# dongyangli-del/EEG_Image_decode

Measured on AMD Instinct MI355X. Metric: EEG-CLIP contrastive train samples/sec (global batch), higher is better.
Workload: dtype f32; 1 GPU; configs[1]: full ATM-S EEG encoder (63ch x 250t -> 1024-d) contrastive train step vs frozen 1024-d CLIP embeddings, 256 samples/GPU; global_batch=256, per_gpu_batch=256, parallelism=dp1, n_classes_for_accuracy=1654, optimizer=AdamW lr 3e-4 (fused)

## Files before the change

eeg_image_decode_amd/_abi.py:

```python
import ctypes as C

BIG = 1 << 62


class Dim(C.Structure):
    _fields_ = [("div", C.c_longlong), ("so", C.c_longlong), ("si", C.c_longlong)]


def dim(si, div=BIG, so=0):
    return Dim(int(div), int(so), int(si))


class GemmDesc(C.Structure):
    _fields_ = [
        ("M", C.c_int), ("N", C.c_int), ("K", C.c_int),
        ("A", C.c_void_p), ("Am", Dim), ("Ak", Dim),
        ("B", C.c_void_p), ("Bk", Dim), ("Bn", Dim),
        ("C", C.c_void_p), ("Cm", Dim), ("Cn", Dim),
        ("Cpre", C.c_void_p),
        ("bias_n", C.c_void_p), ("bias_m", C.c_void_p),
        ("R", C.c_void_p), ("Rm", Dim), ("Rn", Dim),
        ("alpha", C.c_float), ("accumulate", C.c_int), ("act", C.c_int),
        ("drop_p", C.c_float), ("seed", C.c_ulonglong), ("drop_site", C.c_uint),
        ("split_k", C.c_int),
        ("rowsum_a", C.c_void_p),
        ("precision", C.c_int),
        ("workspace", C.c_void_p), ("workspace_bytes", C.c_longlong),
    ]


class SplitItem(C.Structure):
    _fields_ = [("src", C.c_void_p), ("hi", C.c_void_p), ("lo", C.c_void_p), ("rows", C.c_int), ("cols", C.c_int), ("ld_src", C.c_longlong),
                ("ld_out", C.c_longlong), ("transpose", C.c_int), ("copy", C.c_void_p), ("ld_copy", C.c_longlong)]


class InfonceProblem(C.Structure):
    _fields_ = [("q_hi", C.c_void_p), ("q_lo", C.c_void_p), ("k_hi", C.c_void_p), ("k_lo", C.c_void_p), ("col0", C.c_int), ("weight", C.c_float),
                ("part", C.c_void_p), ("diag", C.c_void_p), ("lse", C.c_void_p), ("lse_k", C.c_void_p), ("G", C.c_void_p), ("ldg", C.c_longlong),
                ("part_k", C.c_void_p), ("diag_k", C.c_void_p), ("G_hi", C.c_void_p), ("G_lo", C.c_void_p)]


class TokenBlockDesc(C.Structure):
    _fields_ = ([("B", C.c_int), ("x", C.c_void_p), ("packed", C.c_void_p), ("bv", C.c_void_p), ("pe", C.c_void_p), ("tokens", C.c_void_p), ("ids", C.c_void_p)]
                + [(k, C.c_void_p) for k in ("bqkv", "bo", "ln1_g", "ln1_b", "b1", "b2", "ln2_g", "ln2_b", "ln3_g", "ln3_b")]
                + [(k, C.c_void_p) for k in ("h", "qkv", "r1", "mu1", "rs1", "f1", "r2", "n2", "mu2", "rs2", "n3", "mu3", "rs3")]
                + [(k, C.c_void_p) for k in ("xp", "hp", "ctxp", "n1p", "g1p")]
                + [("drop_p", C.c_float), ("eps", C.c_float), ("scale", C.c_float), ("seed", C.c_ulonglong)]
                + [(k, C.c_uint) for k in ("site_embed", "site_attn", "site_attn_out", "site_ffn_act", "site_ffn_out")]
                + [("packed_embed", C.c_void_p), ("embed_subject", C.c_void_p), ("bv_stride", C.c_longlong)]
                + [("cs_w25", C.c_void_p), ("cs_bias", C.c_void_p), ("cs_rows", C.c_void_p), ("cs_H", C.c_int)])


class TokenBlockBwdDesc(C.Structure):
    _fields_ = ([("B", C.c_int), ("packed", C.c_void_p)]
                + [(k, C.c_void_p) for k in ("dn3", "n2", "r2", "r1", "f1", "mu1", "rs1", "mu2", "rs2", "mu3", "rs3", "ln1_g", "ln2_g", "ln2_b", "ln3_g")]
                + [(k, C.c_void_p) for k in ("dr1", "dctx", "partials", "df2p", "dg1p", "da1p", "dr1p", "dqkvp")]
                + [(k, C.c_void_p) for k in ("dln3_g", "dln3_b", "dln2_g", "dln2_b", "dln1_g", "dln1_b")]
                + [("drop_p", C.c_float), ("seed", C.c_ulonglong)]
                + [(k, C.c_uint) for k in ("site_embed", "site_attn_out", "site_ffn_act", "site_ffn_out")])


class GemmPlanesDesc(C.Structure):
    _fields_ = [("a_hi", C.c_void_p), ("a_lo", C.c_void_p), ("b_hi", C.c_void_p), ("b_lo", C.c_void_p), ("lda", C.c_longlong), ("ldb", C.c_longlong),
                ("M", C.c_int), ("N", C.c_int), ("K", C.c_int), ("C", C.c_void_p), ("ldc", C.c_longlong), ("Cpre", C.c_void_p), ("ldcpre", C.c_longlong),
                ("bias", C.c_void_p), ("R", C.c_void_p), ("ldr", C.c_longlong), ("p_hi", C.c_void_p), ("p_lo", C.c_void_p), ("ldp", C.c_longlong),
                ("act", C.c_int), ("accumulate", C.c_int), ("planes_of", C.c_int)]


class HeadGemmDesc(C.Structure):
    _fields_ = [("a_hi", C.c_void_p), ("a_lo", C.c_void_p), ("b_hi", C.c_void_p), ("b_lo", C.c_void_p), ("lda", C.c_longlong), ("ldb", C.c_longlong),
                ("M", C.c_int), ("N", C.c_int), ("K", C.c_int), ("slices", C.c_int), ("slab_stride", C.c_longlong), ("bias", C.c_void_p),
                ("Cpre", C.c_void_p), ("ldcpre", C.c_longlong), ("act", C.c_int), ("aux", C.c_void_p), ("ldaux", C.c_longlong), ("R", C.c_void_p),
                ("ldr", C.c_longlong), ("C", C.c_void_p), ("ldc", C.c_longlong), ("p_hi", C.c_void_p), ("p_lo", C.c_void_p), ("ldp", C.c_longlong),
                ("b_kmajor", C.c_int)]


class Conv16Desc(C.Structure):
    _fields_ = [("in_", C.c_void_p), ("W", C.c_void_p), ("out", C.c_void_p), ("bias", C.c_void_p), ("residual", C.c_void_p),
                ("N", C.c_int), ("Hi", C.c_int), ("Wi", C.c_int), ("Cin", C.c_int), ("in_pad", C.c_int),
                ("Ho", C.c_int), ("Wo", C.c_int), ("Cout", C.c_int), ("out_pad", C.c_int),
                ("KS", C.c_int), ("stride", C.c_int), ("pad_top", C.c_int), ("pad_left", C.c_int), ("upsample", C.c_int), ("dtype", C.c_int),
                ("chan_bias", C.c_void_p)]


class WgradTokProblem(C.Structure):
    _fields_ = [("a", C.c_void_p), ("b", C.c_void_p), ("a_group_stride", C.c_longlong), ("m_groups", C.c_int), ("heads_m", C.c_int), ("heads_n", C.c_int),
                ("M", C.c_int), ("N", C.c_int), ("out", C.c_void_p), ("ldo", C.c_longlong), ("bias_out", C.c_void_p), ("bias_mfma", C.c_int),
                ("sample0", C.c_int), ("samples", C.c_int), ("sample_index", C.c_void_p)]


class CstackFwdDesc(C.Structure):
    _fields_ = [("B", C.c_int), ("H", C.c_int), ("x", C.c_void_p), ("xs_b", C.c_longlong), ("xs_h", C.c_longlong), ("w25", C.c_void_p), ("bias1", C.c_void_p),
                ("stat1", C.c_void_p), ("nstat1", C.c_int), ("count1", C.c_double), ("eps", C.c_float), ("momentum", C.c_float),
                ("gamma1", C.c_void_p), ("beta1", C.c_void_p), ("mean1", C.c_void_p), ("rstd1", C.c_void_p), ("run_mean1", C.c_void_p),
                ("run_var1", C.c_void_p), ("nbt1", C.c_void_p), ("packed", C.c_void_p), ("bias2", C.c_void_p), ("y2", C.c_void_p), ("stat2", C.c_void_p)]


class CstackBwdDesc(C.Structure):
    _fields_ = [("B", C.c_int), ("H", C.c_int), ("x", C.c_void_p), ("xs_b", C.c_longlong), ("xs_h", C.c_longlong), ("w25", C.c_void_p), ("bias1", C.c_void_p),
                ("mean1", C.c_void_p), ("rstd1", C.c_void_p), ("gamma1", C.c_void_p), ("beta1", C.c_void_p), ("packed_t", C.c_void_p), ("dy2", C.c_void_p),
                ("rows_out", C.c_void_p), ("stat", C.c_void_p), ("nstat", C.c_int), ("count", C.c_double), ("stat_local", C.c_void_p),
                ("nstat_local", C.c_int), ("dgamma", C.c_void_p), ("dbeta", C.c_void_p), ("dx", C.c_void_p), ("dw_partials", C.c_void_p), ("dw25", C.c_void_p)]


class WgradPlanesProblem(C.Structure):
    _fields_ = [("a_hi", C.c_void_p), ("a_lo", C.c_void_p), ("lda", C.c_longlong), ("b_hi", C.c_void_p), ("b_lo", C.c_void_p), ("ldb", C.c_longlong),
                ("rows", C.c_int), ("M", C.c_int), ("N", C.c_int), ("out", C.c_void_p), ("ldo", C.c_longlong), ("bias_out", C.c_void_p), ("slices", C.c_int)]


PLAN_MAX_ARGS = 28
PLAN_MEMSET, PLAN_JOIN, PLAN_SIDE, PLAN_SKIP, PLAN_SIDE2 = -2, -3, 1, 2, 4


class PlanArg(C.Union):
    _fields_ = [("p", C.c_void_p), ("i", C.c_longlong), ("u", C.c_ulonglong), ("d", C.c_double), ("f", C.c_float), ("i32", C.c_int), ("u32", C.c_uint)]


class PlanOp(C.Structure):
    _fields_ = [("fn", C.c_int), ("flags", C.c_int), ("a", PlanArg * PLAN_MAX_ARGS)]


ACT_NONE, ACT_GELU, ACT_SILU, ACT_GELU_GRAD = 0, 1, 2, 3
PREC_F32, PREC_BF16X3 = 0, 1
ABI_VERSION = 14
DT_BF16, DT_F16 = 0, 1
_P, _I, _F, _L, _U64, _U, _D = C.c_void_p, C.c_int, C.c_float, C.c_longlong, C.c_ulonglong, C.c_uint, C.c_double

PROTOTYPES = {
    "eegclip_abi_version": [],
    "eegclip_gemm_f32": [C.POINTER(GemmDesc), _P],
    "eegclip_gemm_workspace_bytes": [C.POINTER(GemmDesc)],
    "eegclip_split_rows": [C.POINTER(SplitItem), _I, _P],
    "eegclip_gemm_f32_grouped": [_P, _I, _P],
    "eegclip_layernorm_fwd": [_P, _P, _P, _P, _P, _P, _I, _I, _F, _P],
    "eegclip_residual_layernorm_fwd": [_P, _P, _P, _F, _U64, _U, _P, _P, _P, _P, _P, _P, _P, _P, _P, _P, _I, _I, _F, _P],
    "eegclip_residual_layernorm_fwd_planes": [_P, _P, _P, _F, _U64, _U, _P, _P, _P, _P, _P, _P, _P, _P, _P, _P, _I, _I, _F, _P, _P, _P],
    "eegclip_layernorm_bwd": [_P, _P, _P, _P, _P, _P, _P, _P, _I, _I, _I, _P, _F, _U64, _U, _P],
    "eegclip_layernorm_bwd_full_workspace_floats": [_I, _I],
    "eegclip_layernorm_bwd_full": [_P, _P, _P, _P, _P, _P, _P, _P, _I, _I, _I, _P, _F, _U64, _U, _P, _P],
    "eegclip_layernorm_bwd_params_workspace_floats": [_I, _I],
    "eegclip_layernorm_bwd_params": [_P, _P, _P, _P, _P, _P, _I, _I, _P, _P],
    "eegclip_layernorm_silu_fwd": [_P, _P, _P, _P, _P, _P, _P, _I, _I, _F, _F, _U64, _U, _P],
    "eegclip_silu_bwd": [_P, _P, _P, _L, _I, _F, _U64, _U, _P],
    "eegclip_timestep_embedding": [_P, _I, _I, _P, _P],
    "eegclip_ddpm_add_noise": [_P, _P, _P, _P, _P, _P, _I, _I, _P],
    "eegclip_ddpm_step": [_P, _P, _P, _F, _F, _F, _F, _F, _F, _P, _P, _P, _L, _P],
    "eegclip_prior_stage_infer": [_P, _P, _P, _P, _P, _P, _P, _I, _P, _I, _I, _F, _P],
    "eegclip_mse_loss_grad": [_P, _P, _L, _P, _P, _P],
    "eegclip_mse_loss_grad_scaled": [_P, _P, _L, _F, _P, _P, _P],
    "eegclip_bn_stats": [_P, _I, _I, _I, _P, _P],
    "eegclip_bn_finalize": [_P, _D, _F, _F, _I, _P, _P, _P, _P, _I, _P, _P],
    "eegclip_bn_finalize_rows": [_P, _I, _D, _F, _F, _I, _P, _P, _P, _P, _P, _P, _P],
    "eegclip_bn_elu_fwd": [_P, _P, _P, _P, _P, _P, _I, _I, _I, _F, _U64, _U, _P],
    "eegclip_bn_elu_bwd": [_P, _P, _P, _P, _P, _P, _P, _P, _P, _P, _I, _I, _I, _F, _U64, _U, _P],
    "eegclip_bn_elu_bwd_stats": [_P, _P, _P, _P, _P, _P, _P, _I, _I, _I, _F, _U64, _U, _P],
    "eegclip_bn_elu_bwd_apply": [_P, _P, _P, _P, _P, _P, _P, _P, _D, _P, _P, _P, _I, _I, _I, _F, _U64, _U, _P],
    "eegclip_embed_finish": [_P, _P, _P, _I, _I, _I, _F, _U64, _U, _P],
    "eegclip_embed_finish_bwd": [_P, _P, _P, _I, _I, _I, _F, _U64, _U, _P],
    "eegclip_dropout_scale": [_P, _L, _F, _U64, _U, _P],
    "eegclip_gelu_bwd": [_P, _P, _P, _L, _I, _F, _U64, _U, _P],
    "eegclip_bias_act": [_P, _P, _P, _P, _P, _I, _I, _I, _F, _U64, _U, _P],
    "eegclip_axpby": [_P, _P, _L, _F, _F, _P],
    "eegclip_reduce_mid": [_P, _I, _I, _I, _P, _P],
    "eegclip_colsum_blocks": [_P, _I, _I, _I, _I, _L, _P, _P],
    "eegclip_sumsq": [_P, _L, _P, _P],
    "eegclip_stage_eeg": [_P, _P, _L, _I, _I, _I, _P, _I, _I, _P],
    "eegclip_gather_rows": [_P, _L, _P, _L, _P, _I, _I, _I, _P],
    "eegclip_adamw_step": [_P, _P, _P, _P, _L, _F, _F, _F, _F, _F, _L, _F, _P, _P],
    "eegclip_adamw_step_zero_grad": [_P, _P, _P, _P, _L, _F, _F, _F, _F, _F, _L, _F, _P, _P],
    "eegclip_clip_scale": [_P, _F, _P, _P],
    "eegclip_attention_fwd": [_P, _P, _I, _I, _I, _I, _I, _F, _F, _U64, _U, _P],
    "eegclip_attention_bwd": [_P, _P, _P, _I, _I, _I, _I, _I, _F, _F, _U64, _U, _P],
    "eegclip_attention_bwd_x3": [_P, _P, _P, _I, _I, _I, _I, _I, _I, _F, _F, _U64, _U, _P],
    "eegclip_proj1x1_fwd": [_P, _P, _P, _P, _P, _P, _P, _P, _P, _I, _F, _U64, _U, _P],
    "eegclip_proj1x1_fwd_rows": [_P, _P, _I, _D, _F, _F, _P, _P, _P, _P, _P, _P, _P, _P, _P, _P, _P, _I, _F, _U64, _U, _P],
    "eegclip_proj1x1_bwd_workspace_floats": [_I],
    "eegclip_proj1x1_bwd": [_P, _P, _P, _P, _P, _P, _P, _P, _P, _P, _P, _P, _P, _I, _F, _U64, _U, _P],
    "eegclip_cast_bf16": [_P, _P, _L, _P],
    "eegclip_logits_bf16": [_P, _P, _P, _I, _I, _I, _L, _P, _P],
    "eegclip_tsconv_fwd_workspace_floats": [_I, _I],
    "eegclip_tsconv_fwd": [_P, _L, _L, _P, _P, _P, _I, _I, _I, _I, _P, _P, _P],
    "eegclip_tsconv_bwd_w": [_P, _L, _L, _P, _P, _P, _I, _I, _I, _I, _P],
    "eegclip_tsconv_bwd_w_workspace_floats": [_I, _I],
    "eegclip_tsconv_bwd_x": [_P, _P, _P, _L, _L, _I, _I, _I, _I, _P],
    "eegclip_cross_attn_fwd": [_P, _P, _P, _P, _P, _P, _I, _I, _I, _I, _I, _I, _F, _I, _P],
    "eegclip_self_attn_supported": [_I, _L, _L, _L, _L],
    "eegclip_self_attn_fwd": [_P, _L, _P, _L, _P, _L, _P, _L, _I, _I, _I, _I, _I, _F, _I, _P],
    "eegclip_self_attn_causal_fwd": [_P, _L, _P, _L, _P, _L, _P, _L, _I, _I, _I, _I, _I, _F, _I, _P],
    "eegclip_sconv_fwd": [_P, _P, _P, _P, _P, _P, _P, _P, _P, _I, _I, _I, _P, _P],
    "eegclip_sconv_fwd_workspace_floats": [_I],
    "eegclip_sconv_bwd_w_workspace_floats": [_I, _I],
    "eegclip_sconv_bwd_w": [_P, _P, _P, _P, _P, _P, _P, _P, _I, _I, _I, _P],
    "eegclip_sconv_bwd_x_stats_workspace_floats": [_I],
    "eegclip_sconv_bwd_x_stats": [_P, _P, _P, _P, _P, _P, _P, _P, _P, _P, _P, _I, _I, _P],
    "eegclip_sconv_bwd_x_apply": [_P, _P, _P, _P, _P, _P, _P, _P, _P, _P, _P, _D, _P, _P, _P, _I, _I, _P],
    "eegclip_lse_rows": [_P, _I, _I, _L, _P, _P, _P],
    "eegclip_lse_cols": [_P, _I, _I, _L, _P, _P, _P],
    "eegclip_infonce_grad": [_P, _I, _I, _L, _I, _I, _P, _P, _P, _F, _P, _P, _P],
    "eegclip_infonce_loss": [_P, _I, _L, _P, _P, _P, _F, _P, _P],
    "eegclip_gemm16": [_P, _L, _P, _L, _P, _L, _P, _P, _L, _I, _I, _I, _I, _I, _P],
    "eegclip_sampler_step": [_P, _P, _P, _P, _P, _P, _F, _F, _F, _F, _F, _L, _I, _P],
    "eegclip_split_bf16": [_P, _P, _P, _L, _P],
    "eegclip_infonce_fused_supported": [_I, _I, _I],
    "eegclip_infonce_fused_workspace_floats": [_I, _I],
    "eegclip_infonce_fused_fwd": [C.POINTER(InfonceProblem), _I, _I, _I, _I, _I, _I, _P, _P, _P],
    "eegclip_infonce_fused_grad": [C.POINTER(InfonceProblem), _I, _I, _I, _I, _I, _I, _P, _P, _P],
    "eegclip_infonce_fused_grad_finalize": [C.POINTER(InfonceProblem), _I, _I, _I, _I, _I, _I, _P, _P, _P, _P],
    "eegclip_token_block_packed_bytes": [],
    "eegclip_token_block_pack": [_P, _P, _P, _P, _P, _P, _P],
    "eegclip_weight_prep": [_P, _P, _P, _P, _P, _P, _P, _P, _P, _I, _P],
    "eegclip_token_block_packed_embed_bytes": [_I],
    "eegclip_token_block_pack_embed": [_P, _L, _I, _P, _P],
    "eegclip_token_block_fwd": [C.POINTER(TokenBlockDesc), _P],
    "eegclip_token_block_bwd_workspace_floats": [_I],
    "eegclip_token_block_bwd": [C.POINTER(TokenBlockBwdDesc), _I, _P],
    "eegclip_gemm_planes": [C.POINTER(GemmPlanesDesc), _P],
    "eegclip_split_transpose": [C.POINTER(SplitItem), _I, _P],
    "eegclip_infonce_small_supported": [_I, _I],
    "eegclip_infonce_small_workspace_floats": [_I, _I],
    "eegclip_infonce_small_fwd": [_P, _I, _L, _I, _I, _P, _P, _P],
    "eegclip_infonce_small_grad": [_I, _I, _P, _P, _F, _F, _F, _F, _P, _P, _L, _P, _P, _P],
    "eegclip_conv16": [C.POINTER(Conv16Desc), _P],
    "eegclip_groupnorm16": [_P, _I, _I, _I, _I, _I, _I, _P, _P, _F, _I, _P, _I, _P, _I, _P],
    "eegclip_softmax_rows16": [_P, _I, _I, _L, _F, _I, _P],
    "eegclip_vae_sample16": [_P, _P, _P, _L, _I, _I, _P],
    "eegclip_layernorm16": [_P, _L, _P, _P, _P, _L, _I, _I, _F, _I, _P],
    "eegclip_geglu16": [_P, _P, _I, _I, _I, _P],
    "eegclip_concat16": [_P, _P, _P, _I, _I, _I, _I, _I, _I, _I, _I, _P],
    "eegclip_gather_rows16": [_P, _L, _P, _I, _P, _I, _P, _I, _I, _I, _P],
    "eegclip_act16": [_P, _L, _P, _L, _I, _I, _I, _I, _P],
    "eegclip_head_gemm_slices": [_I, _I, _I],
    "eegclip_head_gemm": [C.POINTER(HeadGemmDesc), _P],
    "eegclip_head_act": [_P, _I, _L, _P, _P, _P, _P, _P, _I, _I, _P],
    "eegclip_head_act_bwd": [_P, _I, _L, _P, _P, _P, _P, _P, _L, _P],
    "eegclip_residual_layernorm_fwd_slabs": [_P, _P, _P, _F, _U64, _U, _P, _P, _P, _P, _P, _P, _P, _P, _P, _P, _I, _I, _F, _P, _P, _I, _L, _P, _P],
    "eegclip_layernorm_bwd_slabs": [_P, _I, _L, _P, _P, _P, _P, _P, _I, _I, _P, _P, _P, _P, _F, _U64, _U, _P],
    "eegclip_proj1x1_bwd_slabs": [_P, _I, _L, _P, _P, _P, _P, _P, _P, _P, _P, _P, _P, _P, _P, _I, _F, _U64, _U, _P],
    "eegclip_proj1x1_fwd_rows_planes": [_P, _P, _I, _D, _F, _F, _P, _P, _P, _P, _P, _P, _P, _P, _P, _P, _P, _I, _F, _U64, _U, _P, _P, C.POINTER(SplitItem), _I, _P],
    "eegclip_proj1x1_bwd_rows": [_P, _I, _L, _P, _P, _P, _P, _P, _P, _P, _P, _P, _P, _I, _F, _U64, _U, _P],
    "eegclip_proj1x1_bwd_reduce": [_P, _I, _P, _P, _P, _P],
    "eegclip_bn_elu_bwd_apply_rows": [_P, _P, _P, _P, _P, _P, _P, _I, _L, _I, _D, _P, _P, _P, _I, _I, _I, _F, _U64, _U, _P],
    "eegclip_prior_stage_fwd": [_P, _P, _P, _P, _P, _P, _P, _P, _P, _P, _I, _I, _F, _F, _U64, _U, _P],
    "eegclip_prior_stage_bwd": [_P, _P, _P, _P, _P, _P, _P, _P, _P, _P, _P, _I, _I, _F, _U64, _U, _P, _P],
    "eegclip_prior_stage_bwd_workspace_floats": [_I, _I],
    "eegclip_prior_stage_bwd_params": [_P, _I, _I, _P, _P, _P],
    "eegclip_silu_bwd_planes": [_P, _P, _P, _P, _L, _P],
    "eegclip_wgrad_tok_slices": [_I, _I],
    "eegclip_wgrad_tok_workspace_floats": [C.POINTER(WgradTokProblem), _I, _I, _I],
    "eegclip_wgrad_tok": [C.POINTER(WgradTokProblem), _I, _I, _I, _P, _I, _P],
    "eegclip_wgrad_tok_reduce": [C.POINTER(WgradTokProblem), _I, _I, _I, _P, _P],
    "eegclip_wgrad_tok_reduce_adamw": [C.POINTER(WgradTokProblem), _I, _I, _I, _P, _P, _P, _P, _P, _L, _F, _F, _F, _F, _F, _L, _P],
    "eegclip_wgrad_planes": [C.POINTER(WgradPlanesProblem), _I, _P],
    "eegclip_tok_planes_from_f32": [_P, _L, _I, _I, _I, _I, _P, _P],
    "eegclip_cstack_packed_bytes": [_I],
    "eegclip_cstack_pack": [_P, _P, _I, _P],
    "eegclip_cstack_stats1": [_P, _L, _L, _P, _P, _P, _I, _I, _P],
    "eegclip_cstack_fwd": [C.POINTER(CstackFwdDesc), _P],
    "eegclip_cstack_packed_t_bytes": [_I],
    "eegclip_cstack_pack_t": [_P, _P, _I, _P],
    "eegclip_cstack_pack_all": [_P, _P, _P, _I, _P],
    "eegclip_cstack_bwd_stats": [C.POINTER(CstackBwdDesc), _P],
    "eegclip_cstack_bwd_workspace_floats": [_I],
    "eegclip_cstack_bwd_apply": [C.POINTER(CstackBwdDesc), _P],
    "eegclip_cstack_bwd_taps_reduce": [_P, _I, _P, _P],
    "eegclip_cstack_bwd_w2_workspace_floats": [_I, _I],
    "eegclip_cstack_bwd_w2": [_P, _L, _L, _P, _P, _P, _P, _P, _P, _P, _P, _P, _I, _I, _P],
    "eegclip_plan_fn_id": [C.c_char_p],
    "eegclip_plan_events": [_I, C.POINTER(C.c_void_p)],
    "eegclip_plan_events_destroy": [_I, C.POINTER(C.c_void_p)],
    "eegclip_plan_run": [C.POINTER(PlanOp), _I, _I, _I, _P, _P, _P, C.POINTER(C.c_void_p), _P, _P, C.POINTER(C.c_int), C.POINTER(C.c_int)],
    "eegclip_topk_rows": [_P, _I, _I, _L, _I, _P, _P, _P],
    "eegclip_count_equal": [_P, _I, _P, _I, _P, _P],
    "eegclip_top1_count": [_P, _I, _I, _L, _P, _P, _P, _P],
    "eegclip_timing_event_create": [],
    "eegclip_timing_event_destroy": [_P],
    "eegclip_time_next_launch": [_P, _P],
    "eegclip_timing_elapsed_ms": [_P, _P],
# ... 20 lines not shown
```

eeg_image_decode_amd/atms.py:

```python
import os
import weakref
import ctypes
import math

import numpy as np
import torch
import torch.nn as nn

from . import _abi
from ._lib import EegclipError, current_stream, lib, raw_stream, require_cuda
from .loss import ClipLoss
from .plan import Plan

D = _abi.dim
ACT_GELU = _abi.ACT_GELU
ACT_GELU_GRAD = _abi.ACT_GELU_GRAD

N_CH, T_LEN, D_MODEL, N_HEADS, D_HEAD, D_FF = 63, 250, 250, 4, 62, 256
L_TOK = N_CH + 1
HE = N_HEADS * D_HEAD
C_TS, W_TS, F_TS, P_DIM = 40, 36, 1440, 1024
EPS = 1e-5
SITE_EMBED, SITE_ATTN, SITE_ATTN_OUT, SITE_FFN_ACT, SITE_FFN_OUT, SITE_CONV, SITE_PROJ = range(7)

# ... 677 lines not shown
                _p(self.buffers[_TS + "2.running_mean"]), _p(self.buffers[_TS + "2.running_var"]), int(train),
                _p(self.buffers[_TS + "2.num_batches_tracked"]))
        if "scf_ws" not in b:
            b["scf_ws"] = torch.empty(int(lib().eegclip_sconv_fwd_workspace_floats(B)), dtype=torch.float32, device=self.device)
        pl.call("eegclip_sconv_fwd", _p(b["y1"]), _p(bn[0]), _p(bn[1]), _p(P[_TS + "2.weight"]), _p(P[_TS + "2.bias"]), _p(P[_TS + "4.weight"]),
                _p(P[_TS + "4.bias"]), _p(b["y2"]), _p(sums[1]) if train else None, B, N_CH, 1, _p(b["scf_ws"]))
        if W > 1:
            pl.callback(lambda: self._allreduce(sums[1]), "allreduce_bn2")
        pl.call("eegclip_bn_finalize", _p(sums[1]), float(W * B * W_TS), EPS, 0.1, C_TS, _p(bn[2]), _p(bn[3]),
                _p(self.buffers[_TS + "5.running_mean"]), _p(self.buffers[_TS + "5.running_var"]), int(train),
                _p(self.buffers[_TS + "5.num_batches_tracked"]))

    def _build_bwd(self, B, shared, probs, want_dx, early_reduce=False, train=True):
        P, G, b = self.P, self.G, self.bufs[B]
        pe_, pc_, pp_ = probs
        pl = Plan(f"atms_bwd[B={B}]")
        R = B * L_TOK
        sums, bn = b["sums"], b["bn"]
        defer_small = os.environ.get("EEGCLIP_DEFER_SMALL", "1") != "0"
        pl.deferred = []
        wsk = int(os.environ.get("EEGCLIP_WGRAD_SK", "0"))
        attn_bwd = "eegclip_attention_bwd_x3" if pl.precision == _abi.PREC_BF16X3 else "eegclip_attention_bwd"
        sk = lambda k: (wsk if (wsk > 0 and k >= 4096) else max(1, min(64, k // 512)))

        head_side = os.environ.get("EEGCLIP_HEAD_WGRAD_SIDE", "1") != "0"

        def wgrad(name, dY, ldy, X, ldx, Nout, Nin, K, bias=None, side=head_side):
            return pl.gemm(Nout, Nin, K, dY, D(1), D(ldy), X, D(ldx), D(1), _p(G[name]), D(Nin), D(1), accumulate=1, split_k=sk(K),
                           rowsum_a=_p(G[bias]) if bias else None, side=side)

        ln_side = os.environ.get("EEGCLIP_LN_SIDE", "1") != "0"
        if "lnp_ws" not in b:
            b["lnp_ws"] = torch.empty(int(lib().eegclip_layernorm_bwd_params_workspace_floats(R, D_MODEL)), dtype=torch.float32, device=self.device)
        lnp_ws = _p(b["lnp_ws"])
        if "lnf_ws" not in b:
            b["lnf_ws"] = torch.empty(int(lib().eegclip_layernorm_bwd_full_workspace_floats(R, D_MODEL)), dtype=torch.float32, device=self.device)
        lnf_ws = _p(b["lnf_ws"])
        pl.dout_op = len(pl.ops)
        head_planes = self._head_planes_enabled(pl) and hasattr(self, "hw")
        pl.head_planes = head_planes
        dfeat_slabs = None
        if head_planes:
            if "dvp" not in b:
                b["dvp"] = torch.empty(2, B, P_DIM, dtype=torch.bfloat16, device=self.device)
                b["dup"] = torch.empty(2, B, P_DIM, dtype=torch.bfloat16, device=self.device)
                b["dout_sum"] = torch.empty(B, P_DIM, dtype=torch.float32, device=self.device)
            vp, up = (_p(b["dvp"][0]), _p(b["dvp"][1])), (_p(b["dup"][0]), _p(b["dup"][1]))
            pl.call("eegclip_layernorm_bwd_slabs", 0, 1, 0, _p(b["s"]), _p(P["proj_eeg.2.weight"]), _p(b["mu4"]), _p(b["rs4"]), _p(b["ds"]), B, P_DIM,
                    _p(b["dv"]), *vp, None, pp_, 0, SITE_PROJ, seed_at=15)
            one_fork = os.environ.get("EEGCLIP_HEAD_FORKS", "1") == "1"
            head_side_ops = []

            def later(fn):
                if one_fork:
                    head_side_ops.append(fn)
                else:
                    fn()

            def ln_params():
                pl.dout_par_op = len(pl.ops)
                pl.call("eegclip_layernorm_bwd", 0, _p(b["s"]), None, _p(b["mu4"]), _p(b["rs4"]), None,
                        _p(G["proj_eeg.2.weight"]), _p(G["proj_eeg.2.bias"]), B, P_DIM, 0, None, 0.0, 0, 0, side=ln_side)
            later(ln_params)
            wplanes = B % 32 == 0 and os.environ.get("EEGCLIP_HEAD_WGRAD_PLANES", "1") != "0"
            if not wplanes:
                later(lambda: wgrad("proj_eeg.1.fn.1.weight", _p(b["dv"]), P_DIM, _p(b["gu"]), P_DIM, P_DIM, P_DIM, B, bias="proj_eeg.1.fn.1.bias"))
            if os.environ.get("EEGCLIP_HEAD_FUSED_EPI", "0") == "1":
                pl.call_desc("eegclip_head_gemm", _abi.HeadGemmDesc(a_hi=vp[0], a_lo=vp[1], b_hi=self.hw["w2"][0], b_lo=self.hw["w2"][1], lda=P_DIM, ldb=P_DIM, M=B,
                                                                   N=P_DIM, K=P_DIM, slices=1, slab_stride=0, act=ACT_GELU_GRAD, aux=_p(b["u"]), ldaux=P_DIM,
                                                                   R=_p(b["ds"]), ldr=P_DIM, C=_p(b["ds"]), ldc=P_DIM, p_hi=up[0], p_lo=up[1], ldp=P_DIM, b_kmajor=1))
            else:
                sl = self._head_gemm(pl, b, "dgu_slabs", vp, P_DIM, self.hw["w2"], P_DIM, B, kmajor=True)
                pl.call("eegclip_head_act_bwd", *sl, _p(b["u"]), _p(b["ds"]), _p(b["ds"]), *up, B * P_DIM)
            if wplanes:
                gp_, fp_ = (_p(b["gup"][0]), _p(b["gup"][1])), (_p(b["featp"][0]), _p(b["featp"][1]))
                probs = (_abi.WgradPlanesProblem * 2)(
                    _abi.WgradPlanesProblem(a_hi=vp[0], a_lo=vp[1], lda=P_DIM, b_hi=gp_[0], b_lo=gp_[1], ldb=P_DIM, rows=B, M=P_DIM, N=P_DIM,
                                            out=_p(G["proj_eeg.1.fn.1.weight"]), ldo=P_DIM, bias_out=_p(G["proj_eeg.1.fn.1.bias"]), slices=1),
                    _abi.WgradPlanesProblem(a_hi=up[0], a_lo=up[1], lda=P_DIM, b_hi=fp_[0], b_lo=fp_[1], ldb=F_TS, rows=B, M=P_DIM, N=F_TS,
                                            out=_p(G["proj_eeg.0.weight"]), ldo=F_TS, bias_out=_p(G["proj_eeg.0.bias"]), slices=1))
                pl._keep.append(probs)
                later(lambda: pl.call("eegclip_wgrad_planes", probs, 2, side=head_side))
            else:
                later(lambda: wgrad("proj_eeg.0.weight", _p(b["ds"]), P_DIM, _p(b["feat"]), F_TS, P_DIM, F_TS, B, bias="proj_eeg.0.bias"))
            dfeat_slabs = self._head_gemm(pl, b, "dfeat_slabs", up, P_DIM, self.hw["w1"], F_TS, B, kmajor=True)
        else:
            head_side_ops = []
            self._build_bwd_head_f32(pl, b, B, pp_, ln_side, wgrad)
        W = self._world() if train else 1
        zsum = None
        if not train:
            zsum = torch.zeros(2 * C_TS, dtype=torch.float64, device=self.device)
            pl._keep.append(zsum)

            def conv_bias_grad(bias_key, gamma_key, rstd, s):
                return lambda: G[bias_key].add_((P[gamma_key] * rstd * s[:C_TS].to(torch.float32)))
        if "pj_ws" not in b:
            b["pj_ws"] = torch.empty(int(lib().eegclip_proj1x1_bwd_workspace_floats(B)) // 2, dtype=torch.float64, device=self.device)
        lean = dfeat_slabs is not None and self._lean(pl, train, W)
        pl.lean = lean
        if lean:
            if "pj_bn_rows" not in b:
                b["pj_bn_rows"] = torch.empty(B, 2 * C_TS, dtype=torch.float64, device=self.device)
            pl.call("eegclip_proj1x1_bwd_rows", *dfeat_slabs, _p(b["z2"]), _p(P["enc_eeg.0.projection.0.weight"]), _p(b["y2"]), _p(bn[2]), _p(bn[3]),
                    _p(P[_TS + "5.weight"]), _p(P[_TS + "5.bias"]), _p(b["dz2"]), _p(b["pj_ws"]), _p(b["pj_bn_rows"]), B, pc_, 0, SITE_CONV, seed_at=15)
            pl.call("eegclip_bn_elu_bwd_apply_rows", _p(b["dz2"]), _p(b["y2"]), _p(bn[2]), _p(bn[3]), _p(P[_TS + "5.weight"]), _p(P[_TS + "5.bias"]),
                    _p(b["pj_bn_rows"]), B, 2 * C_TS, 0, float(B * W_TS),
                    _p(b["dy2"]), _p(G[_TS + "5.weight"]), _p(G[_TS + "5.bias"]), B, C_TS, W_TS, pc_, 0, SITE_CONV, seed_at=18)
            for f in head_side_ops:
                f()
            pl.call("eegclip_proj1x1_bwd_reduce", _p(b["pj_ws"]), B, _p(G["enc_eeg.0.projection.0.weight"]), _p(G["enc_eeg.0.projection.0.bias"]), None, side=True)
        else:
            if dfeat_slabs is not None:
                pl.call("eegclip_proj1x1_bwd_slabs", *dfeat_slabs, _p(b["z2"]), _p(P["enc_eeg.0.projection.0.weight"]), _p(b["y2"]), _p(bn[2]), _p(bn[3]),
                        _p(P[_TS + "5.weight"]), _p(P[_TS + "5.bias"]), _p(b["dz2"]), _p(G["enc_eeg.0.projection.0.weight"]),
                        _p(G["enc_eeg.0.projection.0.bias"]), _p(sums[2]), _p(b["pj_ws"]), B, pc_, 0, SITE_CONV, seed_at=17)
            else:
                pl.call("eegclip_proj1x1_bwd", _p(b["dfeat"]), _p(b["z2"]), _p(P["enc_eeg.0.projection.0.weight"]), _p(b["y2"]), _p(bn[2]), _p(bn[3]),
                        _p(P[_TS + "5.weight"]), _p(P[_TS + "5.bias"]), _p(b["dz2"]), _p(G["enc_eeg.0.projection.0.weight"]),
                        _p(G["enc_eeg.0.projection.0.bias"]), _p(sums[2]), _p(b["pj_ws"]), B, pc_, 0, SITE_CONV, seed_at=15)
            local2 = None
            if W > 1:
                local2 = torch.zeros_like(sums[2])
                pl._keep.append(local2)

                def exchange2():
                    local2.copy_(sums[2])
                    self._allreduce(sums[2])
                pl.callback(exchange2, "allreduce_bn2_bwd")
            if not train:
                pl.callback(conv_bias_grad(_TS + "4.bias", _TS + "5.weight", bn[3], sums[2]), "conv2_bias_grad_eval")
            pl.call("eegclip_bn_elu_bwd_apply", _p(b["dz2"]), _p(b["y2"]), _p(bn[2]), _p(bn[3]), _p(P[_TS + "5.weight"]), _p(P[_TS + "5.bias"]),
                    _p(sums[2]) if train else _p(zsum), (_p(local2) if local2 is not None else None) if train else _p(sums[2]), float(W * B * W_TS), _p(b["dy2"]), _p(G[_TS + "5.weight"]), _p(G[_TS + "5.bias"]), B, C_TS,
                    W_TS, pc_, 0, SITE_CONV, seed_at=16)
            for f in head_side_ops:
                f()
        if self._cstack_bwd_enabled(pl):
            self._build_bwd_cstack(pl, b, B, train, W, zsum, conv_bias_grad if not train else None, early_reduce, defer_small)
        else:
            self._build_bwd_conv_y1(pl, b, B, train, W, zsum, conv_bias_grad if not train else None, early_reduce)
        fused = self._token_block_enabled(pl) and hasattr(self, "tb_packed")
        if fused:
            if "tb_part" not in b:
                b["tb_part"] = torch.empty(int(lib().eegclip_token_block_bwd_workspace_floats(B)), dtype=torch.float32, device=self.device)
            df2p, dg1p, da1p, dr1p, dqkvp = self._token_planes(b, B, "df2p", "dg1p", "da1p", "dr1p", "dqkvp")
            xp, hp, ctxp, n1p, g1p = self._token_planes(b, B, "xp", "hp", "ctxp", "n1p", "g1p")
            bd = _abi.TokenBlockBwdDesc(
                B=B, packed=_p(self.tb_packed), dn3=_p(b["dn3"]), n2=None, r2=_p(b["r2"]), r1=_p(b["r1"]), f1=_p(b["f1"]), mu1=_p(b["mu1"]),
                rs1=_p(b["rs1"]), mu2=_p(b["mu2"]), rs2=_p(b["rs2"]), mu3=_p(b["mu3"]), rs3=_p(b["rs3"]), ln1_g=_p(P[_LY + "norm1.weight"]),
                ln2_g=_p(P[_LY + "norm2.weight"]), ln2_b=_p(P[_LY + "norm2.bias"]), ln3_g=_p(P["encoder.encoder.norm.weight"]),
                dr1=_p(b["dr1"]), dctx=_p(b["dctx"]), partials=_p(b["tb_part"]), df2p=df2p, dg1p=dg1p, da1p=da1p, dr1p=dr1p, dqkvp=dqkvp,
                dln3_g=_p(G["encoder.encoder.norm.weight"]), dln3_b=_p(G["encoder.encoder.norm.bias"]), dln2_g=_p(G[_LY + "norm2.weight"]),
                dln2_b=_p(G[_LY + "norm2.bias"]), dln1_g=_p(G[_LY + "norm1.weight"]), dln1_b=_p(G[_LY + "norm1.bias"]),
                drop_p=pe_, seed=0, site_embed=SITE_EMBED, site_attn_out=SITE_ATTN_OUT, site_ffn_act=SITE_FFN_ACT, site_ffn_out=SITE_FFN_OUT)
            pl._keep.append(bd)
            if pe_ > 0.0:
                pl._seed_descs.append(bd)
            variant = 0

            def wgrad_tok(tag, problems, side=True, slices=None, index=None):
                arr = (_abi.WgradTokProblem * len(problems))()
                for i, (name, a, mg, x, M, N, hm, hn, bias, bm) in enumerate(problems):
                    arr[i] = _abi.WgradTokProblem(a=a, b=x, a_group_stride=B * 65536 if mg > 1 else 0, m_groups=mg, heads_m=hm, heads_n=hn, M=M, N=N,
                                                  out=_p(G[name]), ldo=N, bias_out=_p(G[bias]) if bias else None, bias_mfma=bm, sample_index=index)
                groups = sum(q[2] for q in problems)
                slices = slices or (wsk if wsk > 0 else int(lib().eegclip_wgrad_tok_slices(groups, B)))
                key = "wk:" + tag
                if key not in b:
                    b[key] = torch.empty(int(lib().eegclip_wgrad_tok_workspace_floats(arr, len(problems), B, slices)), dtype=torch.float32, device=self.device)
                pl._keep.append(arr)
                ops = (len(pl.ops), len(pl.ops) + 1)
                pl.call("eegclip_wgrad_tok", arr, len(problems), B, slices, _p(b[key]), variant, side=side)
                pl.call("eegclip_wgrad_tok_reduce", arr, len(problems), B, slices, _p(b[key]), side=side)
                return arr, ops

            merge = int(os.environ.get("EEGCLIP_WGRAD_MERGE", "2"))
            late = []
            ffn_out = [
                (_LY + "conv2.weight", df2p, 1, g1p, D_MODEL, D_FF, 0, 0, _LY + "conv2.bias", 1),
                (_LY + "conv1.weight", dg1p, 1, n1p, D_FF, D_MODEL, 0, 0, _LY + "conv1.bias", 0),
                (_LY + "attention.out_projection.weight", da1p, 1, ctxp, D_MODEL, HE, 0, 1, _LY + "attention.out_projection.bias", 0)]
            qkv_w = [(_LY + "attention.query_projection.weight", dqkvp, 3, hp, 3 * HE, D_MODEL, 1, 0, _LY + "attention.query_projection.bias", 0)]
            pl.call("eegclip_token_block_bwd", ctypes.byref(bd), 0)
            if defer_small:
                pl.deferred.append(lambda: pl.call("eegclip_token_block_bwd", ctypes.byref(bd), 2, side=True))
            else:
                pl.call("eegclip_token_block_bwd", ctypes.byref(bd), 2, side=ln_side)
            if merge >= 2:
                late += ffn_out
            else:
                wgrad_tok("ffn_out", ffn_out)
            pl.call(attn_bwd, _p(b["qkv"]), _p(b["dctx"]), dqkvp, 1, B, L_TOK, N_HEADS, D_HEAD, 3 * HE, 1.0 / math.sqrt(D_HEAD),
                    pe_, 0, SITE_ATTN, seed_at=11)
            if merge >= 1:
                late += qkv_w
            else:
                wgrad_tok("qkv", qkv_w)
            pl.call("eegclip_token_block_bwd", ctypes.byref(bd), 1)
        else:
            pl.call("eegclip_layernorm_bwd_full", _p(b["dn3"]), _p(b["n2"]), _p(P["encoder.encoder.norm.weight"]), _p(b["mu3"]), _p(b["rs3"]), _p(b["dn2"]),
                    _p(G["encoder.encoder.norm.weight"]), _p(G["encoder.encoder.norm.bias"]), R, D_MODEL, 0, None, 0.0, 0, 0, lnf_ws)
            pl.call("eegclip_layernorm_bwd_full", _p(b["dn2"]), _p(b["r2"]), _p(P[_LY + "norm2.weight"]), _p(b["mu2"]), _p(b["rs2"]), _p(b["dr2"]),
                    _p(G[_LY + "norm2.weight"]), _p(G[_LY + "norm2.bias"]), R, D_MODEL, 0, _p(b["df2"]), pe_, 0, SITE_FFN_OUT, lnf_ws, seed_at=13)
            wgrad(_LY + "conv2.weight", _p(b["df2"]), D_MODEL, _p(b["g1"]), D_FF, D_MODEL, D_FF, R, bias=_LY + "conv2.bias")
            pl.gemm(R, D_FF, D_MODEL, _p(b["df2"]), D(D_MODEL), D(1), _p(P[_LY + "conv2.weight"]), D(D_FF), D(1), _p(b["dg1"]), D(D_FF), D(1),
                    act=ACT_GELU_GRAD, R=_p(b["f1"]), Rm=D(D_FF), Rn=D(1), drop_p=pe_, drop_site=SITE_FFN_ACT)
            wgrad(_LY + "conv1.weight", _p(b["dg1"]), D_FF, _p(b["n1"]), D_MODEL, D_FF, D_MODEL, R, bias=_LY + "conv1.bias")
            pl.gemm(R, D_MODEL, D_FF, _p(b["dg1"]), D(D_FF), D(1), _p(P[_LY + "conv1.weight"]), D(D_MODEL), D(1), _p(b["dr2"]), D(D_MODEL), D(1),
                    accumulate=1)
            pl.call("eegclip_layernorm_bwd_full", _p(b["dr2"]), _p(b["r1"]), _p(P[_LY + "norm1.weight"]), _p(b["mu1"]), _p(b["rs1"]), _p(b["dr1"]),
                    _p(G[_LY + "norm1.weight"]), _p(G[_LY + "norm1.bias"]), R, D_MODEL, 0, _p(b["da1"]), pe_, 0, SITE_ATTN_OUT, lnf_ws, seed_at=13)
            wgrad(_LY + "attention.out_projection.weight", _p(b["da1"]), D_MODEL, _p(b["ctx"]), HE, D_MODEL, HE, R,
                  bias=_LY + "attention.out_projection.bias")
            pl.gemm(R, HE, D_MODEL, _p(b["da1"]), D(D_MODEL), D(1), _p(P[_LY + "attention.out_projection.weight"]), D(HE), D(1), _p(b["dctx"]), D(HE), D(1))
            if attn_bwd == "eegclip_attention_bwd_x3":
                pl.call(attn_bwd, _p(b["qkv"]), _p(b["dctx"]), _p(b["dqkv"]), 0, B, L_TOK, N_HEADS, D_HEAD, 3 * HE, 1.0 / math.sqrt(D_HEAD),
                        pe_, 0, SITE_ATTN, seed_at=11)
            else:
                pl.call(attn_bwd, _p(b["qkv"]), _p(b["dctx"]), _p(b["dqkv"]), B, L_TOK, N_HEADS, D_HEAD, 3 * HE, 1.0 / math.sqrt(D_HEAD),
                        pe_, 0, SITE_ATTN, seed_at=10)
            wgrad(_LY + "attention.query_projection.weight", _p(b["dqkv"]), 3 * HE, _p(b["h"]), D_MODEL, 3 * HE, D_MODEL, R,
                  bias=_LY + "attention.query_projection.bias")
            pl.gemm(R, D_MODEL, 3 * HE, _p(b["dqkv"]), D(3 * HE), D(1), _p(P[_LY + "attention.query_projection.weight"]), D(D_MODEL), D(1),
                    _p(b["dr1"]), D(D_MODEL), D(1), accumulate=2, drop_p=pe_, drop_site=SITE_EMBED)
        tokg = G[_TOK_SHARED] if shared else G[_TOK_TABLE]
        pl.call("eegclip_embed_finish_bwd", _p(b["dr1"]), _p(tokg), None if shared else _p(b["ids"]), B, L_TOK, D_MODEL, 0.0, 0, SITE_EMBED, side=True)
        for f in pl.deferred:
            f()
        hmap = D(D_MODEL, div=N_CH, so=L_TOK * D_MODEL)
        if want_dx:
            b["dx"] = torch.empty(B, N_CH, T_LEN, dtype=torch.float32, device=self.device)
        pl.x_gemm = None
        if fused:
            if not self.joint:
                wgrad_tok("embed" + ("+%d" % len(late) if late else ""), late + [(_E + "value_embedding.weight", dr1p, 1, xp, D_MODEL, T_LEN, 0, 0, _E + "value_embedding.bias", 0)], side=False)
            else:
                if late:
                    wgrad_tok("block", late, side=False)
                pl.j_wk_template = [(w, dr1p, 1, xp, D_MODEL, T_LEN, 0, 0, bk, 0) for w, bk in self.ve_keys]
                pl.j_wk_slices = [0] + [max(1, min(32, 2 * B // 4, (64 // n) // 8 * 8 if 64 // n >= 8 else 64 // n)) for n in range(1, self.n_subj + 1)]
                pl.j_wk_arr, pl.j_wk_ops = wgrad_tok("embed_joint", pl.j_wk_template, side=False, slices=8, index=_p(b["perm"]))
                need = max(int(lib().eegclip_wgrad_tok_workspace_floats(pl.j_wk_arr, n, B, pl.j_wk_slices[n])) for n in range(1, self.n_subj + 1))
                if b["wk:embed_joint"].numel() < need:
                    b["wk:embed_joint"] = torch.empty(need, dtype=torch.float32, device=self.device)
                    for op in pl.j_wk_ops:
                        pl.set_arg(op, 4, _p(b["wk:embed_joint"]))
                pl.j_wk_all = (_abi.WgradTokProblem * self.n_subj)(*pl.j_wk_arr)
                pl._keep.append(pl.j_wk_all)
        elif not self.joint:
            pl.x_gemm = pl.gemm(D_MODEL, T_LEN, B * N_CH, _p(b["dr1"]) + 4 * D_MODEL, D(1), hmap, 0, D(T_LEN), D(1),
                    _p(G[_E + "value_embedding.weight"]), D(T_LEN), D(1), accumulate=1, split_k=sk(B * N_CH),
                    rowsum_a=_p(G[_E + "value_embedding.bias"]))
        if not self.joint:
            if want_dx:
                pl.gemm(B * N_CH, T_LEN, D_MODEL, _p(b["dr1"]) + 4 * D_MODEL, hmap, D(1),
                        _p(P[_E + "value_embedding.weight"]), D(T_LEN), D(1), _p(b["dx"]), D(T_LEN), D(1))
        elif fused and not want_dx:
            pass
        else:
            XR = N_CH * T_LEN
            pl.j_gather = len(pl.ops)
            pl.call("eegclip_gather_rows", _p(b["hs"]) + 4 * D_MODEL, L_TOK * D_MODEL, _p(b["dr1"]) + 4 * D_MODEL, L_TOK * D_MODEL, _p(b["perm"]), B,
                    N_CH * D_MODEL, 0)
            if not fused:
                pl.j_gemm = [pl.desc(D_MODEL, T_LEN, N_CH, 0, D(1), hmap, 0, D(T_LEN), D(1), _p(G[w]), D(T_LEN), D(1), accumulate=1, split_k=1,
                                     rowsum_a=_p(G[bk])) for w, bk in self.ve_keys]
                pl.j_arr, pl.j_group = pl.gemm_grouped(self.n_subj)
            if want_dx:
                b["dxs"] = torch.empty(B, N_CH, T_LEN, dtype=torch.float32, device=self.device)
                pl.j_dx = [pl.desc(N_CH, T_LEN, D_MODEL, 0, hmap, D(1), _p(P[w]), D(T_LEN), D(1), 0, D(T_LEN), D(1)) for w, _ in self.ve_keys]
                pl.j_dx_arr, pl.j_dx_group = pl.gemm_grouped(self.n_subj)
                pl.j_scatter = len(pl.ops)
                pl.call("eegclip_gather_rows", _p(b["dx"]), XR, _p(b["dxs"]), XR, _p(b["perm"]), B, XR, 1)
        return pl

    def _build_bwd_head_f32(self, pl, b, B, pp_, ln_side, wgrad):
        P, G = self.P, self.G
        pl.call("eegclip_layernorm_bwd", 0, _p(b["s"]), _p(P["proj_eeg.2.weight"]), _p(b["mu4"]), _p(b["rs4"]), _p(b["ds"]),
                None, None, B, P_DIM, 0, _p(b["dv"]), pp_, 0, SITE_PROJ, seed_at=13)
        pl.dout_par_op = len(pl.ops)
        pl.call("eegclip_layernorm_bwd", 0, _p(b["s"]), None, _p(b["mu4"]), _p(b["rs4"]), None,
                _p(G["proj_eeg.2.weight"]), _p(G["proj_eeg.2.bias"]), B, P_DIM, 0, None, 0.0, 0, 0, side=ln_side)
        wgrad("proj_eeg.1.fn.1.weight", _p(b["dv"]), P_DIM, _p(b["gu"]), P_DIM, P_DIM, P_DIM, B, bias="proj_eeg.1.fn.1.bias")
        skh = _head_split(B)
        pl.gemm(B, P_DIM, P_DIM, _p(b["dv"]), D(P_DIM), D(1), _p(P["proj_eeg.1.fn.1.weight"]), D(P_DIM), D(1), _p(b["dgu"]), D(P_DIM), D(1),
                accumulate=int(skh > 1), split_k=skh)
        pl.call("eegclip_gelu_bwd", _p(b["dgu"]), _p(b["u"]), _p(b["ds"]), B * P_DIM, 1, 0.0, 0, 0)
        wgrad("proj_eeg.0.weight", _p(b["ds"]), P_DIM, _p(b["feat"]), F_TS, P_DIM, F_TS, B, bias="proj_eeg.0.bias")
        pl.gemm(B, F_TS, P_DIM, _p(b["ds"]), D(P_DIM), D(1), _p(P["proj_eeg.0.weight"]), D(F_TS), D(1), _p(b["dfeat"]), D(F_TS), D(1),
                accumulate=int(skh > 1), split_k=skh)

    def _build_bwd_cstack(self, pl, b, B, train, W, zsum, conv_bias_grad, early_reduce, defer_small=False):
        P, G, sums, bn = self.P, self.G, b["sums"], b["bn"]
        dev = self.device
        if "csw_ws" not in b:
            b["csw_ws"] = torch.empty(int(lib().eegclip_cstack_bwd_w2_workspace_floats(B, N_CH)), dtype=torch.float32, device=dev)
            b["csb_ws"] = torch.empty(int(lib().eegclip_cstack_bwd_workspace_floats(B)), dtype=torch.float32, device=dev)
            b["cs_rows3"] = torch.empty(B, 2 * C_TS, dtype=torch.float64, device=dev)
        xs = (_p(b["n3"]), L_TOK * D_MODEL, D_MODEL)
        bnp = (_p(bn[0]), _p(bn[1]), _p(P[_TS + "2.weight"]), _p(P[_TS + "2.bias"]))
        pl.call("eegclip_cstack_bwd_w2", *xs, _p(P[_TS + "0.weight"]), _p(P[_TS + "0.bias"]), *bnp, _p(b["dy2"]), _p(G[_TS + "4.weight"]), _p(b["csw_ws"]),
                B, N_CH, side=os.environ.get("EEGCLIP_W2_SIDE", "1") != "0")
        rows3 = b["cs_rows3"]
        count1 = float(W * B * N_CH * W_TS)
        common = dict(B=B, H=N_CH, x=xs[0], xs_b=xs[1], xs_h=xs[2], w25=_p(P[_TS + "0.weight"]), bias1=_p(P[_TS + "0.bias"]), mean1=bnp[0], rstd1=bnp[1],
                      gamma1=bnp[2], beta1=bnp[3], packed_t=_p(self.cs_packed_t), dy2=_p(b["dy2"]), rows_out=_p(rows3), count=count1,
                      dgamma=_p(G[_TS + "2.weight"]), dbeta=_p(G[_TS + "2.bias"]), dx=_p(b["dn3"]), dw_partials=_p(b["csb_ws"]), dw25=_p(G[_TS + "0.weight"]))
        pl.call_desc("eegclip_cstack_bwd_stats", _abi.CstackBwdDesc(stat=None, nstat=0, stat_local=None, nstat_local=0, **common))
        stat, nstat, local, nlocal = _p(rows3), B, None, 0
        if W > 1 or not train:
            pl.call("eegclip_bn_finalize_rows", _p(rows3), B, count1, EPS, 0.1, C_TS, None, None, None, None, None, _p(sums[3]))
            local, nlocal = _p(rows3), B
            if W > 1:
                pl.callback(lambda: self._allreduce(sums[3]), "allreduce_bn1_bwd")
            stat, nstat = (_p(sums[3]), 1) if train else (_p(zsum), 1)
            if not train:
                pl.callback(conv_bias_grad(_TS + "0.bias", _TS + "2.weight", bn[1], sums[3]), "conv1_bias_grad_eval")
        pl.call_desc("eegclip_cstack_bwd_apply", _abi.CstackBwdDesc(stat=stat, nstat=nstat, stat_local=local, nstat_local=nlocal, **dict(common, dw25=None)))
        pl.early_cut = len(pl.ops)

        def taps():
            pl.taps_op = len(pl.ops)
            pl.call("eegclip_cstack_bwd_taps_reduce", _p(b["csb_ws"]), B, _p(G[_TS + "0.weight"]), side=True)
        if early_reduce or not defer_small:
            taps()
        else:
            pl.deferred.append(taps)
        if early_reduce:
            pl.callback(self._start_early_reduce, "allreduce_early_bucket", side=True)

    def _build_bwd_conv_y1(self, pl, b, B, train, W, zsum, conv_bias_grad, early_reduce):
        P, G, sums, bn = self.P, self.G, b["sums"], b["bn"]
        if "scw_ws" not in b:
            b["scw_ws"] = torch.empty(int(lib().eegclip_sconv_bwd_w_workspace_floats(B, N_CH)), dtype=torch.float32, device=self.device)
        bnp = (_p(bn[0]), _p(bn[1]), _p(P[_TS + "2.weight"]), _p(P[_TS + "2.bias"]))
        wt = (None, None)
        if "scx_ws" not in b:
            b["scx_ws"] = torch.empty(int(lib().eegclip_sconv_bwd_x_stats_workspace_floats(B)) // 2, dtype=torch.float64, device=self.device)
        pl.call("eegclip_sconv_bwd_w", _p(b["y1"]), *bnp, _p(b["dy2"]), _p(G[_TS + "4.weight"]), _p(b["scw_ws"]), B, N_CH, pl.precision & 0xff, side=True)
        pl.call("eegclip_sconv_bwd_x_stats", _p(b["dy2"]), _p(P[_TS + "4.weight"]), *wt, _p(b["y1"]), *bnp, _p(sums[3]), _p(b["scx_ws"]), B, N_CH)
        local1 = None
        if W > 1:
            local1 = torch.zeros_like(sums[3])
            pl._keep.append(local1)

            def exchange1():
                local1.copy_(sums[3])
                self._allreduce(sums[3])
            pl.callback(exchange1, "allreduce_bn1_bwd")
        if not train:
            pl.callback(conv_bias_grad(_TS + "0.bias", _TS + "2.weight", bn[1], sums[3]), "conv1_bias_grad_eval")
# ... 216 lines not shown
```

eeg_image_decode_amd/csrc/attention_x3.hip:

```cpp
#include "eeg_common.h"

namespace eeg {

constexpr int AX_L = 64;
constexpr int AX_RS = 144;
constexpr int AX_PLANE = AX_L * AX_RS;
constexpr int AX_TENSOR = 2 * AX_PLANE;

struct ax_args {
    const float* qkv;
    const float* dctx;
    float* dqkv;
    unsigned char* dqkvp;
    int B, H, E, ld;
    float scale, drop_p;
    unsigned long long seed;
    unsigned site;
};

typedef short ax_s4 __attribute__((ext_vector_type(4)));
typedef float ax_f2 __attribute__((ext_vector_type(2)));
typedef float ax_f4u __attribute__((ext_vector_type(4), aligned(4)));

__device__ __forceinline__ ax_s4 ax_tr_read(const unsigned char* p) {
#if defined(EEG_EMU)
    const int lane = hipemu::cur->lane, g = lane >> 4, i = lane & 15;
    ax_s4 r;
    for (int j = 0; j < 4; ++j) {
        const unsigned long long src = hipemu::shfl_idx((unsigned long long)(uintptr_t)p, 16 * g + 4 * j + (i >> 2));
        r[j] = reinterpret_cast<const short*>((uintptr_t)src)[i & 3];
    }
    return r;
#else
    return __builtin_amdgcn_ds_read_tr16_b64_v4i16((__attribute__((address_space(3))) ax_s4*)(p));
#endif
}
__device__ __forceinline__ bf16x8 ax_tr_frag(const unsigned char* plane, int r0, int r1, int c0, int lane) {
    const int l = lane & 15;
    const ax_s4 a = ax_tr_read(plane + (r0 + (l >> 2)) * AX_RS + 2 * (c0 + 4 * (l & 3)));
    const ax_s4 b = ax_tr_read(plane + (r1 + (l >> 2)) * AX_RS + 2 * (c0 + 4 * (l & 3)));
    return bf16x8{a[0], a[1], a[2], a[3], b[0], b[1], b[2], b[3]};
}
__device__ __forceinline__ bf16x8 ax_frag(const unsigned char* plane, int row, int k0) {
    return *reinterpret_cast<const bf16x8*>(plane + row * AX_RS + 2 * k0);
}
__device__ __forceinline__ bf16x8 ax_pack8(u32x2_t a, u32x2_t b) {
    typedef unsigned u4 __attribute__((ext_vector_type(4)));
    const u4 v{a[0], a[1], b[0], b[1]};
    return __builtin_bit_cast(bf16x8, v);
}
__device__ __forceinline__ f32x4 ax_mfma3(bf16x8 ah, bf16x8 al, bf16x8 bh, bf16x8 bl, f32x4 c) {
    c = mfma_bf16_16x16x32(al, bh, c);
    c = mfma_bf16_16x16x32(ah, bl, c);
    return mfma_bf16_16x16x32(ah, bh, c);
}
__device__ __forceinline__ void ax_store4(float* p, int valid, f32x4 v) {
    if (valid >= 4) *reinterpret_cast<ax_f4u*>(p) = ax_f4u{v[0], v[1], v[2], v[3]};
    else if (valid >= 2) {
        *reinterpret_cast<ax_f2*>(p) = ax_f2{v[0], v[1]};
        if (valid == 3) p[2] = v[2];
    } else if (valid == 1) p[0] = v[0];
}

__device__ __forceinline__ void ax_store4_planes(unsigned char* row_base, int e0, f32x4 v) {
    u32x2_t hi, lo;
    x3_split4(v[0], v[1], v[2], v[3], hi, lo);
    *reinterpret_cast<u32x2_t*>(row_base + 2 * e0) = hi;
    *reinterpret_cast<u32x2_t*>(row_base + 32768 + 2 * e0) = lo;
}

template <bool TRAIN>
__global__ __launch_bounds__(256, 2) void attention_bwd_x3_kernel(const ax_args a) {
    EEG_LDS_BASE(float, ldsf);
    unsigned char* lds = reinterpret_cast<unsigned char*>(ldsf);
    unsigned char* Qp = lds;
    unsigned char* Kp = lds + AX_TENSOR;
    unsigned char* Vp = lds + 2 * AX_TENSOR;
    unsigned char* Op = lds + 3 * AX_TENSOR;
    const int t = threadIdx.x, lane = t & 63, w = wave_uniform(t >> 6), fr = lane & 15, g = lane >> 4;
    const int bh = blockIdx.x, b = bh / a.H, h = bh - b * a.H;
    const int E = a.E, HE = a.H * E;
    const float* qrow0 = a.qkv + (long long)b * AX_L * a.ld + h * E;
    const float* orow0 = a.dctx + (long long)b * AX_L * HE + h * E;

    {
        ax_f2 v[4][8];
#pragma unroll
        for (int j = 0; j < 8; ++j) {
            const int idx = t + 256 * j, row = idx >> 5, col = 2 * (idx & 31);
            const bool ok = col < E;
            const float* qr = qrow0 + (long long)row * a.ld + col;
            v[0][j] = ok ? *reinterpret_cast<const ax_f2*>(qr) : ax_f2{0.f, 0.f};
            v[1][j] = ok ? *reinterpret_cast<const ax_f2*>(qr + HE) : ax_f2{0.f, 0.f};
            v[2][j] = ok ? *reinterpret_cast<const ax_f2*>(qr + 2 * HE) : ax_f2{0.f, 0.f};
            v[3][j] = ok ? *reinterpret_cast<const ax_f2*>(orow0 + (long long)row * HE + col) : ax_f2{0.f, 0.f};
        }
#pragma unroll
        for (int x = 0; x < 4; ++x)
#pragma unroll
            for (int j = 0; j < 8; ++j) {
                const int idx = t + 256 * j, row = idx >> 5, col = 2 * (idx & 31);
                const unsigned hi = x3_pack2(v[x][j][0], v[x][j][1]);
                const float r0 = v[x][j][0] - __uint_as_float(hi << 16), r1 = v[x][j][1] - __uint_as_float(hi & 0xffff0000u);
                unsigned char* dst = lds + x * AX_TENSOR + row * AX_RS + 2 * col;
                *reinterpret_cast<unsigned*>(dst) = hi;
                *reinterpret_cast<unsigned*>(dst + AX_PLANE) = x3_pack2(r0, r1);
            }
    }
    __syncthreads();

    f32x4 s[4], dp[4];
#pragma unroll
    for (int kt = 0; kt < 4; ++kt) { s[kt] = f32x4{0.f, 0.f, 0.f, 0.f}; dp[kt] = f32x4{0.f, 0.f, 0.f, 0.f}; }
#pragma unroll
    for (int ks = 0; ks < 2; ++ks) {
        const int k0 = 32 * ks + 8 * g;
        const bf16x8 qh = ax_frag(Qp, 16 * w + fr, k0), ql = ax_frag(Qp + AX_PLANE, 16 * w + fr, k0);
        const bf16x8 oh = ax_frag(Op, 16 * w + fr, k0), ol = ax_frag(Op + AX_PLANE, 16 * w + fr, k0);
#pragma unroll
        for (int kt = 0; kt < 4; ++kt) {
            const bf16x8 kh = ax_frag(Kp, 16 * kt + fr, k0), kl = ax_frag(Kp + AX_PLANE, 16 * kt + fr, k0);
            const bf16x8 vh = ax_frag(Vp, 16 * kt + fr, k0), vl = ax_frag(Vp + AX_PLANE, 16 * kt + fr, k0);
            s[kt] = ax_mfma3(kh, kl, qh, ql, s[kt]);
            dp[kt] = ax_mfma3(vh, vl, oh, ol, dp[kt]);
        }
    }
    float mx = -INFINITY;
#pragma unroll
    for (int kt = 0; kt < 4; ++kt)
#pragma unroll
        for (int r = 0; r < 4; ++r) {
            s[kt][r] *= a.scale;
            mx = fmaxf(mx, s[kt][r]);
        }
    mx = fmaxf(mx, __shfl_xor(mx, 16, 64));
    mx = fmaxf(mx, __shfl_xor(mx, 32, 64));
    float sum = 0.f;
#pragma unroll
    for (int kt = 0; kt < 4; ++kt)
#pragma unroll
        for (int r = 0; r < 4; ++r) {
            s[kt][r] = expf(s[kt][r] - mx);
            sum += s[kt][r];
        }
    sum += __shfl_xor(sum, 16, 64);
    sum += __shfl_xor(sum, 32, 64);
    const float inv = 1.0f / sum;
    const bool drop = TRAIN && a.drop_p > 0.f;
    const float ksc = drop ? 1.f / (1.f - a.drop_p) : 1.f;
    f32x4 pd[4];
    float dq_sum = 0.f;
#pragma unroll
    for (int kt = 0; kt < 4; ++kt) {
        bool keep[4] = {true, true, true, true};
        if (drop) {
            const unsigned long long idx0 = ((unsigned long long)bh * AX_L + 16 * w + fr) * AX_L + 16 * kt + 4 * g;
            dropout_keep4(a.seed, a.site, idx0, a.drop_p, keep);
        }
#pragma unroll
        for (int r = 0; r < 4; ++r) {
            const float p = s[kt][r] * inv;
            const float d = keep[r] ? dp[kt][r] * ksc : 0.f;
            pd[kt][r] = keep[r] ? p * ksc : 0.f;
            s[kt][r] = p;
            dp[kt][r] = d;
            dq_sum += p * d;
        }
    }
    dq_sum += __shfl_xor(dq_sum, 16, 64);
    dq_sum += __shfl_xor(dq_sum, 32, 64);
#pragma unroll
    for (int kt = 0; kt < 4; ++kt)
#pragma unroll
        for (int r = 0; r < 4; ++r) dp[kt][r] = s[kt][r] * (dp[kt][r] - dq_sum);

    {
        f32x4 dq[4];
#pragma unroll
        for (int et = 0; et < 4; ++et) dq[et] = f32x4{0.f, 0.f, 0.f, 0.f};
#pragma unroll
        for (int m = 0; m < 2; ++m) {
            u32x2_t h0, l0, h1, l1;
            x3_split4(dp[2 * m][0], dp[2 * m][1], dp[2 * m][2], dp[2 * m][3], h0, l0);
            x3_split4(dp[2 * m + 1][0], dp[2 * m + 1][1], dp[2 * m + 1][2], dp[2 * m + 1][3], h1, l1);
            const bf16x8 bhf = ax_pack8(h0, h1), blf = ax_pack8(l0, l1);
#pragma unroll
            for (int et = 0; et < 4; ++et) {
                const bf16x8 ah = ax_tr_frag(Kp, 32 * m + 4 * g, 32 * m + 16 + 4 * g, 16 * et, lane);
                const bf16x8 al = ax_tr_frag(Kp + AX_PLANE, 32 * m + 4 * g, 32 * m + 16 + 4 * g, 16 * et, lane);
                dq[et] = ax_mfma3(ah, al, bhf, blf, dq[et]);
            }
        }
        float* out = a.dqkv + ((long long)b * AX_L + 16 * w + fr) * a.ld + h * E;
        unsigned char* outp = a.dqkvp + (long long)b * 65536 + (16 * w + fr) * 512 + 128 * h;
#pragma unroll
        for (int et = 0; et < 4; ++et) {
            const int e0 = 16 * et + 4 * g;
            f32x4 v = dq[et];
#pragma unroll
            for (int r = 0; r < 4; ++r) v[r] *= a.scale;
            if (a.dqkvp) ax_store4_planes(outp, e0, v);
            else if (e0 < E) ax_store4(out + e0, E - e0, v);
        }
    }
    __syncthreads();
#pragma unroll
    for (int kt = 0; kt < 4; ++kt) {
        u32x2_t hi, lo;
        const int off = (16 * w + fr) * AX_RS + 2 * (16 * kt + 4 * g);
        x3_split4(pd[kt][0], pd[kt][1], pd[kt][2], pd[kt][3], hi, lo);
        *reinterpret_cast<u32x2_t*>(Kp + off) = hi;
        *reinterpret_cast<u32x2_t*>(Kp + AX_PLANE + off) = lo;
        x3_split4(dp[kt][0], dp[kt][1], dp[kt][2], dp[kt][3], hi, lo);
        *reinterpret_cast<u32x2_t*>(Vp + off) = hi;
        *reinterpret_cast<u32x2_t*>(Vp + AX_PLANE + off) = lo;
    }
    __syncthreads();

    f32x4 dv[4], dk[4];
#pragma unroll
    for (int et = 0; et < 4; ++et) { dv[et] = f32x4{0.f, 0.f, 0.f, 0.f}; dk[et] = f32x4{0.f, 0.f, 0.f, 0.f}; }
#pragma unroll
    for (int ks = 0; ks < 2; ++ks) {
        const int q0 = 32 * ks + 8 * g;
        const bf16x8 ph = ax_tr_frag(Kp, q0, q0 + 4, 16 * w, lane), pl = ax_tr_frag(Kp + AX_PLANE, q0, q0 + 4, 16 * w, lane);
        const bf16x8 sh = ax_tr_frag(Vp, q0, q0 + 4, 16 * w, lane), sl = ax_tr_frag(Vp + AX_PLANE, q0, q0 + 4, 16 * w, lane);
#pragma unroll
        for (int et = 0; et < 4; ++et) {
            const bf16x8 oh = ax_tr_frag(Op, q0, q0 + 4, 16 * et, lane), ol = ax_tr_frag(Op + AX_PLANE, q0, q0 + 4, 16 * et, lane);
            const bf16x8 qh = ax_tr_frag(Qp, q0, q0 + 4, 16 * et, lane), ql = ax_tr_frag(Qp + AX_PLANE, q0, q0 + 4, 16 * et, lane);
            dv[et] = ax_mfma3(oh, ol, ph, pl, dv[et]);
            dk[et] = ax_mfma3(qh, ql, sh, sl, dk[et]);
        }
    }
    if (a.dqkvp) {
        const long long grp = (long long)a.B * 65536;
        unsigned char* outp = a.dqkvp + (long long)b * 65536 + (16 * w + fr) * 512 + 128 * h;
#pragma unroll
        for (int et = 0; et < 4; ++et) {
            const int e0 = 16 * et + 4 * g;
            f32x4 v = dk[et];
#pragma unroll
            for (int r = 0; r < 4; ++r) v[r] *= a.scale;
            ax_store4_planes(outp + grp, e0, v);
            ax_store4_planes(outp + 2 * grp, e0, dv[et]);
        }
        return;
    }
    float* outk = a.dqkv + ((long long)b * AX_L + 16 * w + fr) * a.ld + HE + h * E;
#pragma unroll
    for (int et = 0; et < 4; ++et) {
        const int e0 = 16 * et + 4 * g;
        if (e0 < E) {
            f32x4 v = dk[et];
#pragma unroll
            for (int r = 0; r < 4; ++r) v[r] *= a.scale;
            ax_store4(outk + e0, E - e0, v);
            ax_store4(outk + HE + e0, E - e0, dv[et]);
        }
    }
}

}

using namespace eeg;

extern "C" int eegclip_attention_bwd_x3(const float* qkv, const float* dctx, void* dqkv, int dqkv_planes, int B, int L, int H, int E, int ld, float scale,
                                        float drop_p, unsigned long long seed, unsigned site, void* stream) {
    if (dqkv_planes && (H > 4 || (reinterpret_cast<uintptr_t>(dqkv) & 15u))) return dqkv && H <= 4 ? EEGCLIP_EALIGN : EEGCLIP_EINVAL;
    if (!qkv || !dctx || !dqkv || B < 1 || L != AX_L || H < 1 || E < 2 || E > 64 || (E & 1) || (ld & 1) || ld < 3 * H * E || drop_p < 0.f || drop_p >= 1.f)
        return EEGCLIP_EINVAL;
    if ((reinterpret_cast<uintptr_t>(qkv) | reinterpret_cast<uintptr_t>(dctx) | reinterpret_cast<uintptr_t>(dqkv)) & 7u) return EEGCLIP_EALIGN;
    const ax_args a{qkv, dctx, dqkv_planes ? nullptr : static_cast<float*>(dqkv), dqkv_planes ? static_cast<unsigned char*>(dqkv) : nullptr, B, H, E, ld, scale,
                    drop_p, seed, site};
    const size_t lds = 4 * AX_TENSOR;
    if (drop_p > 0.f) EEG_LAUNCH(attention_bwd_x3_kernel<true>, dim3(B * H), dim3(256), lds, stream, a);
    else              EEG_LAUNCH(attention_bwd_x3_kernel<false>, dim3(B * H), dim3(256), lds, stream, a);
    return (int)hipGetLastError();
}
```

eeg_image_decode_amd/csrc/token_block.hip:

```cpp
#include "cstack_common.h"

#include <stdio.h>
#include <stdlib.h>

namespace eeg {

constexpr int TB_THREADS = 512;
constexpr int TB_L = 64, TB_D = 250, TB_T = 250, TB_NCH = 63, TB_H = 4, TB_E = 62, TB_HE = 248, TB_FF = 256;
constexpr int TB_AP_PLANE = 64 * 512;
constexpr int TB_AP_BYTES = 2 * TB_AP_PLANE;
constexpr int TB_XF_BYTES = 64 * 1024;
constexpr int TB_HQ_PLANE = 64 * 128;
constexpr int TB_HQ_BYTES = 6 * TB_HQ_PLANE;
constexpr int TB_LDS = TB_AP_BYTES + 2 * TB_HQ_BYTES;
constexpr int TB_KS = 8;
constexpr int TB_TILE = 1024;
constexpr int TB_NT_V = 16, TB_NT_QKV = 48, TB_NT_O = 16, TB_NT_1 = 16, TB_NT_2 = 16;
constexpr int TB_NMAT = 11;
constexpr long long TB_OFF_V = 0;
constexpr long long TB_OFF_QKV = TB_OFF_V + (long long)TB_NT_V * TB_KS * TB_TILE;
constexpr long long TB_OFF_O = TB_OFF_QKV + (long long)TB_NT_QKV * TB_KS * TB_TILE;
constexpr long long TB_OFF_1 = TB_OFF_O + (long long)TB_NT_O * TB_KS * TB_TILE;
constexpr long long TB_OFF_2 = TB_OFF_1 + (long long)TB_NT_1 * TB_KS * TB_TILE;
constexpr long long TB_MAT_ELEMS = 16LL * TB_KS * TB_TILE;
constexpr long long TB_OFF_2T = TB_OFF_2 + TB_MAT_ELEMS;
constexpr long long TB_OFF_1T = TB_OFF_2T + TB_MAT_ELEMS;
constexpr long long TB_OFF_OT = TB_OFF_1T + TB_MAT_ELEMS;
constexpr long long TB_OFF_QT = TB_OFF_OT + TB_MAT_ELEMS;
constexpr long long TB_PACKED_ELEMS = TB_OFF_QT + 3 * TB_MAT_ELEMS;

typedef float tb_f4u __attribute__((ext_vector_type(4), aligned(4)));
typedef float tb_f2 __attribute__((ext_vector_type(2)));
typedef unsigned tb_u4 __attribute__((ext_vector_type(4)));

__device__ __forceinline__ int ap_off(int row, int k) { return row * 512 + ((((k >> 3) ^ (row & 15))) << 4) + ((k & 7) << 1); }
__device__ __forceinline__ int xf_off(int row, int col) { return row * 1024 + ((((col >> 2) ^ (row & 15))) << 4) + ((col & 3) << 2); }
__device__ __forceinline__ int hq_off(int row, int k) { return row * 128 + ((((k >> 3) ^ ((row >> 1) & 7))) << 4) + ((k & 7) << 1); }

__device__ __forceinline__ long long tb_src_index(int mat, int n, int k) {
    switch (mat) {
        case 0: return (n < TB_D && k < TB_T) ? (long long)n * TB_T + k : -1;
        case 1: {
            const int seg = n >> 6, d = n & 63, head = seg / 3, which = seg - 3 * head;
            return (seg < 12 && d < TB_E && k < TB_D) ? (long long)(which * TB_HE + head * TB_E + d) * TB_D + k : -1;
        }
        case 2: {
            const int head = k >> 6, d = k & 63;
            return (n < TB_D && head < TB_H && d < TB_E) ? (long long)n * TB_HE + head * TB_E + d : -1;
        }
        case 3: return (n < TB_FF && k < TB_D) ? (long long)n * TB_D + k : -1;
        case 4: return (n < TB_D && k < TB_FF) ? (long long)n * TB_FF + k : -1;
        case 5: return (n < TB_FF && k < TB_D) ? (long long)k * TB_FF + n : -1;
        case 6: return (n < TB_D && k < TB_FF) ? (long long)k * TB_D + n : -1;
        case 7: {
            const int head = n >> 6, d = n & 63;
            return (head < TB_H && d < TB_E && k < TB_D) ? (long long)k * TB_HE + head * TB_E + d : -1;
        }
        default: {
            const int head = k >> 6, d = k & 63;
            return (n < TB_D && head < TB_H && d < TB_E) ? (long long)((mat - 8) * TB_HE + head * TB_E + d) * TB_D + n : -1;
        }
    }
}

struct tb_pack_args {
    const float* w[TB_NMAT];
    unsigned short* out;
    int tb_tiles;
    const float* Ws;
    unsigned char *cs_packed, *cs_packed_t;
    int H;
};

__global__ __launch_bounds__(64) void token_block_pack_kernel(const tb_pack_args a) {
    if ((int)blockIdx.x >= a.tb_tiles) {
        cs_pack_both(a.Ws, a.cs_packed, a.cs_packed_t, a.H, ((int)blockIdx.x - a.tb_tiles) * 64 + (int)(threadIdx.x & 63));
        return;
    }
    int tile = blockIdx.x;
    int mat = 0;
    while (mat < TB_NMAT - 1 && tile >= (mat == 1 ? TB_NT_QKV : 16) * TB_KS) { tile -= (mat == 1 ? TB_NT_QKV : 16) * TB_KS; ++mat; }
    const int nt = tile / TB_KS, ks = tile % TB_KS;
    const int lane = threadIdx.x & 63;
    const int n = 16 * nt + (lane & 15), k0 = 32 * ks + 8 * (lane >> 4);
    const float* src = a.w[mat];
    unsigned hb[8], lb[8];
#pragma unroll
    for (int e = 0; e < 8; ++e) {
        const long long si = tb_src_index(mat, n, k0 + e);
        const float v = si >= 0 ? src[si] : 0.f;
        const unsigned short h = f32_to_bf16_bits(v);
        hb[e] = h;
        lb[e] = f32_to_bf16_bits(v - bf16_bits_to_f32(h));
    }
    unsigned short* dst = a.out + (long long)blockIdx.x * TB_TILE + lane * 8;
    tb_u4 oh, ol;
#pragma unroll
    for (int e = 0; e < 4; ++e) {
        oh[e] = hb[2 * e] | (hb[2 * e + 1] << 16);
        ol[e] = lb[2 * e] | (lb[2 * e + 1] << 16);
    }
    *reinterpret_cast<tb_u4*>(dst) = oh;
    *reinterpret_cast<tb_u4*>(dst + 512) = ol;
}

#ifndef TB_FWD_RING
#define TB_FWD_RING false
#endif
#ifndef TB_QKV_RING
#define TB_QKV_RING false
#endif
#ifndef TB_BWD_PF
#define TB_BWD_PF 2
#endif
template <int NT, unsigned TM, int PF = 2, bool ZERO = true, bool RING = false>
__device__ __forceinline__ void tb_gemm(const unsigned char* AP, const unsigned short* wp, int lane, f32x4 (&acc)[4][NT]) {
    const int fr = lane & 15, g = lane >> 4;
    if (ZERO) {
#pragma unroll
        for (int mt = 0; mt < 4; ++mt)
#pragma unroll
            for (int j = 0; j < NT; ++j) acc[mt][j] = f32x4{0.f, 0.f, 0.f, 0.f};
    }
    bf16x8 bh[PF + 1][NT], bl[PF + 1][NT];
    auto issue = [&](int ks) {
        const int slot = ks % (PF + 1);
#pragma unroll
        for (int j = 0; j < NT; ++j) {
            const bf16x8* q = reinterpret_cast<const bf16x8*>(wp + (long long)(j * TB_KS + ks) * TB_TILE) + lane;
#if defined(EEG_EMU)
            bh[slot][j] = q[0];
            bl[slot][j] = q[64];
#else
            if constexpr (RING) {
                asm volatile("global_load_dwordx4 %0, %1, off" : "=v"(bh[slot][j]) : "v"(q) : "memory");
                asm volatile("global_load_dwordx4 %0, %1, off offset:1024" : "=v"(bl[slot][j]) : "v"(q) : "memory");
            } else {
                bh[slot][j] = q[0];
                bl[slot][j] = q[64];
            }
#endif
        }
    };
    auto landed = [&](int ks) {
#if !defined(EEG_EMU)
        if constexpr (!RING) return;
        static_assert(NT == 2 || NT == 3, "the wait statements list 2 NT fragment registers");
        const int slot = ks % (PF + 1);
        const int younger = TB_KS - 1 - ks < PF ? TB_KS - 1 - ks : PF;
#define TB_WAIT(N)                                                                                                                       \
    do {                                                                                                                                 \
        if constexpr (NT == 2)                                                                                                           \
            asm volatile("s_waitcnt vmcnt(" #N ")" : "+v"(bh[slot][0]), "+v"(bl[slot][0]), "+v"(bh[slot][1]), "+v"(bl[slot][1])::"memory"); \
// ... 480 lines not shown
                const bool wrap = col + 2 >= TB_D;
                const int row2 = wrap ? row + 1 : row, col2 = wrap ? col + 2 - TB_D : col + 2;
                const tb_f2 p0 = *reinterpret_cast<const tb_f2*>(XF + xf_off(row, col)), p1 = *reinterpret_cast<const tb_f2*>(XF + xf_off(row2, col2));
                float v[4] = {p0[0], p0[1], p1[0], p1[1]};
                if (TRAIN && p2.drop_p > 0.f) {
                    bool keep[4];
                    dropout_keep4(p2.seed, p2.site_embed, (unsigned long long)b * (TB_L * TB_D) + i0, p2.drop_p, keep);
#pragma unroll
                    for (int e = 0; e < 4; ++e) v[e] = keep[e] ? v[e] * ksc : 0.f;
                }
                if (!(p2.dbg & 1u)) *reinterpret_cast<f32x4*>(hb + i0) = f32x4{v[0], v[1], v[2], v[3]};
                tb_store_planes2(AP, TB_AP_PLANE, ap_off(row, col), v[0], v[1]);
                tb_store_planes2(AP, TB_AP_PLANE, ap_off(row2, col2), v[2], v[3]);
            }
        }
    }
    raw_barrier();

    tb_stamp(a0, b, t, 3);
    const tb_fwd_args p3 = tb_args_again(a0);
    f32x4 ctxr[2][4];
    {
        const int hip = w >> 2;
        unsigned char* const HQ = lds + TB_AP_BYTES + hip * TB_HQ_BYTES;
#pragma unroll
        for (int rd = 0; rd < 2; ++rd) {
            f32x4 cur[4][3];
            switch (w & 3) {
                case 0: tb_qkv_pass<0>(p3, AP, b, 2 * rd + hip, lane, cur); tb_qkv_to_lds<0>(HQ, lane, cur); break;
                case 1: tb_qkv_pass<1>(p3, AP, b, 2 * rd + hip, lane, cur); tb_qkv_to_lds<1>(HQ, lane, cur); break;
                case 2: tb_qkv_pass<2>(p3, AP, b, 2 * rd + hip, lane, cur); tb_qkv_to_lds<2>(HQ, lane, cur); break;
                default: tb_qkv_pass<3>(p3, AP, b, 2 * rd + hip, lane, cur); tb_qkv_to_lds<3>(HQ, lane, cur); break;
            }
            if (rd == 1 && !(p3.dbg & 1u)) tb_planes_out<0>(AP, p3.hp + (long long)b * (2 * TB_AP_PLANE), t);
            raw_barrier();
            tb_stamp(a0, b, t, 10 + 2 * rd);
            tb_attention<TRAIN>(p3, HQ, b, 2 * rd + hip, w & 3, lane, ctxr[rd]);
            raw_barrier();
            tb_stamp(a0, b, t, 11 + 2 * rd);
        }
#pragma unroll
        for (int rd = 0; rd < 2; ++rd) {
            const int head = 2 * rd + hip, m = 16 * (w & 3) + fr;
#pragma unroll
            for (int dt = 0; dt < 4; ++dt) {
                const int d0 = 16 * dt + 4 * g;
                const f32x4 c = ctxr[rd][dt];
                tb_store_planes4(AP, TB_AP_PLANE, ap_off(m, 64 * head + d0), c[0], c[1], c[2], c[3]);
            }
        }
    }
    raw_barrier();

    tb_stamp(a0, b, t, 4);
    const tb_fwd_args p4 = tb_args_again(a0);
    {
        f32x4 acc[4][2];
        tb_gemm<2, 3u, 2, true, TB_FWD_RING>(AP, p4.packed + TB_OFF_O + (long long)(2 * w) * TB_KS * TB_TILE, lane, acc);
        tb_for_tiles(w, lane, TB_D, acc, [&](int m, int n0, int valid, f32x4& v) {
            const f32x4 bias = tb_ld4(p4.bo + n0, valid);
            f32x4 o;
#pragma unroll
            for (int i = 0; i < 4; ++i) o[i] = i < valid ? v[i] + bias[i] : 0.f;
            *reinterpret_cast<f32x4*>(XF + xf_off(m, n0)) = o;
        });
        if (!(p4.dbg & 1u)) tb_planes_out<0>(AP, p4.ctxp + (long long)b * (2 * TB_AP_PLANE), t);
    }
    __syncthreads();
    tb_stamp(a0, b, t, 5);
    const tb_fwd_args p5 = tb_args_again(a0);
    tb_ln_rows<TRAIN, false>(p5, b, w, lane, XF, nullptr, p5.h, p5.site_attn_out, p5.r1, p5.ln1_g, p5.ln1_b, nullptr, p5.mu1, p5.rs1, nullptr, nullptr, nullptr, nullptr,
                             nullptr, XF, AP);
    raw_barrier();

    tb_stamp(a0, b, t, 6);
    const tb_fwd_args p6 = tb_args_again(a0);
    {
        f32x4 acc[4][2];
        tb_gemm<2, 3u, 2, true, TB_FWD_RING>(AP, p6.packed + TB_OFF_1 + (long long)(2 * w) * TB_KS * TB_TILE, lane, acc);
        f32x4 bias1[2];
#pragma unroll
        for (int j = 0; j < 2; ++j) bias1[j] = *reinterpret_cast<const f32x4*>(p6.b1 + 32 * w + 16 * j + 4 * g);
        tb_for_tiles(w, lane, TB_FF, acc, [&](int m, int n0, int valid, f32x4& v) {
            const f32x4 bias = bias1[(n0 >> 4) & 1];
            const long long ob = (long long)b * (TB_L * TB_FF);
            const unsigned ol = (unsigned)(m * TB_FF + n0);
            f32x4 f, gq;
#pragma unroll
            for (int i = 0; i < 4; ++i) f[i] = v[i] + bias[i];
            if (!(p6.dbg & 1u)) *reinterpret_cast<f32x4*>(p6.f1 + ob + ol) = f;
            bool keep[4] = {true, true, true, true};
            if (TRAIN && p6.drop_p > 0.f) dropout_keep4(p6.seed, p6.site_ffn_act, (unsigned long long)ob + ol, p6.drop_p, keep);
#pragma unroll
            for (int i = 0; i < 4; ++i) {
                const float ge = gelu_erf(f[i]);
                gq[i] = (TRAIN && p6.drop_p > 0.f) ? (keep[i] ? ge * ksc : 0.f) : ge;
            }
            v = gq;
        });
        if (!(p6.dbg & 1u)) tb_planes_out<0>(AP, p6.n1p + (long long)b * (2 * TB_AP_PLANE), t);
        raw_barrier();
        tb_for_tiles(w, lane, TB_FF, acc, [&](int m, int n0, int valid, f32x4& v) {
            tb_store_planes4(AP, TB_AP_PLANE, ap_off(m, n0), v[0], v[1], v[2], v[3]);
        });
    }
    raw_barrier();

    tb_stamp(a0, b, t, 7);
    const tb_fwd_args p7 = tb_args_again(a0);
    {
        f32x4 acc[4][2];
        tb_gemm<2, 3u, 2, true, TB_FWD_RING>(AP, p7.packed + TB_OFF_2 + (long long)(2 * w) * TB_KS * TB_TILE, lane, acc);
        f32x4 bias2[2];
#pragma unroll
        for (int j = 0; j < 2; ++j) {
            const int n0 = 32 * w + 16 * j + 4 * g;
            bias2[j] = n0 < TB_D ? tb_ld4(p7.b2 + n0, TB_D - n0 >= 4 ? 4 : 2) : f32x4{0.f, 0.f, 0.f, 0.f};
        }
        if (!(p7.dbg & 1u)) tb_planes_out<64>(AP, p7.g1p + (long long)b * (2 * TB_AP_PLANE), t);
        raw_barrier();
#pragma unroll
        for (int j = 0; j < 2; ++j) {
            const int n0 = 32 * w + 16 * j + 4 * g;
            if (n0 >= TB_D) continue;
            const int valid = TB_D - n0 >= 4 ? 4 : TB_D - n0;
#pragma unroll
            for (int mt = 0; mt < 4; ++mt) {
                f32x4 o;
#pragma unroll
                for (int i = 0; i < 4; ++i) o[i] = i < valid ? acc[mt][j][i] + bias2[j][i] : 0.f;
                *reinterpret_cast<f32x4*>(AP + xf_off(16 * mt + fr, n0)) = o;
            }
        }
    }
    raw_barrier();
    tb_stamp(a0, b, t, 8);
    const tb_fwd_args p8 = tb_args_again(a0);
    tb_ln_rows<TRAIN, true>(p8, b, w, lane, AP, XF, nullptr, p8.site_ffn_out, p8.r2, p8.ln2_g, p8.ln2_b, p8.n2, p8.mu2, p8.rs2, p8.ln3_g, p8.ln3_b, p8.n3, p8.mu3, p8.rs3,
                            nullptr, nullptr);
    tb_stamp(a0, b, t, 9);
    if (a0.cs_rows) {
        __syncthreads();
        const tb_fwd_args p9 = tb_args_again(a0);
        cs_stats1_sample(lds, p9.n3, (long long)(TB_L * TB_D), (long long)TB_D, p9.cs_w25, p9.cs_bias, p9.cs_rows, b, p9.cs_H, 1);
    }
}


struct tb_bwd_args {
    const unsigned short* packed;
    const float *dn3, *n2, *r2, *r1, *f1, *mu1, *rs1, *mu2, *rs2, *mu3, *rs3, *ln1_g, *ln2_g, *ln2_b, *ln3_g;
    float *dr1, *dctx, *partials;
    unsigned char *df2p, *dg1p, *da1p, *dr1p;
    const unsigned char* dqkvp;
    float drop_p;
    unsigned long long seed;
    unsigned site_embed, site_attn_out, site_ffn_act, site_ffn_out;
};

__device__ __forceinline__ void tb_ln_bwd_row(const float (&dy)[4], const float (&x)[4], const float (&gam)[4], const bool (&ok)[2], float mu, float rs,
                                              float (&dx)[4], float (&pg)[4], float (&pb)[4]) {
    float xh[4], gq[4];
    float s1 = 0.f, s2 = 0.f;
#pragma unroll
    for (int e = 0; e < 4; ++e) {
        xh[e] = ok[e >> 1] ? (x[e] - mu) * rs : 0.f;
        gq[e] = dy[e] * gam[e];
        s1 += gq[e];
        s2 += gq[e] * xh[e];
        pg[e] += dy[e] * xh[e];
        pb[e] += dy[e];
    }
    const float c1 = wave_sum(s1) * (1.0f / (float)TB_D), c2 = wave_sum(s2) * (1.0f / (float)TB_D);
#pragma unroll
    for (int e = 0; e < 4; ++e) dx[e] = ok[e >> 1] ? rs * (gq[e] - c1 - xh[e] * c2) : 0.f;
}

template <int NV>
__device__ __forceinline__ void tb_reduce_partials(float* slab, int w, int lane, int t, const float (&pe)[NV][4], const float (&po)[NV][4], float* out) {
    float* mine = slab + w * (NV * 256);
#pragma unroll
    for (int v = 0; v < NV; ++v) *reinterpret_cast<f32x4*>(mine + v * 256 + 4 * lane) = f32x4{pe[v][0], pe[v][1], pe[v][2], pe[v][3]};
    wave_sync();
#pragma unroll
    for (int v = 0; v < NV; ++v)
#pragma unroll
        for (int e = 0; e < 4; ++e) {
            const int c = 4 * lane - 2 + e;
            if (c >= 0) mine[v * 256 + c] += po[v][e];
        }
    raw_barrier();
    for (int i = t; i < NV * 256; i += TB_THREADS) {
        float sum = 0.f;
#pragma unroll
        for (int ww = 0; ww < 8; ++ww) sum += slab[ww * (NV * 256) + i];
        out[i] = sum;
    }
}

template <bool TRAIN>
__global__ __launch_bounds__(TB_THREADS, 2) void token_block_bwd_a_kernel(const tb_bwd_args a0) {
    EEG_LDS_BASE(unsigned char, lds);
    unsigned char* const AP = lds;
    unsigned char* const XF = lds + TB_AP_BYTES;
    float* const SC = reinterpret_cast<float*>(lds + TB_AP_BYTES + TB_XF_BYTES);
    const int t = threadIdx.x, lane = t & 63, w = wave_uniform(t >> 6);
    const int b = blockIdx.x;
    const float ksc = (TRAIN && a0.drop_p > 0.f) ? 1.f / (1.f - a0.drop_p) : 1.f;
    float* const part = a0.partials + (long long)b * (6 * 256);

    const tb_bwd_args q1 = tb_args_again(a0);
    {
        float pe[4][4], po[4][4];
#pragma unroll
        for (int v = 0; v < 4; ++v)
#pragma unroll
            for (int e = 0; e < 4; ++e) { pe[v][e] = 0.f; po[v][e] = 0.f; }
        tb_f2 pg3[2][2], pg2[2][2], pb2[2][2];
#pragma unroll
        for (int par = 0; par < 2; ++par)
#pragma unroll
            for (int p = 0; p < 2; ++p) {
                const int cp = 4 * lane - 2 * par + 2 * p;
                const bool okc = cp >= 0 && cp < TB_D;
                pg3[par][p] = okc ? *reinterpret_cast<const tb_f2*>(q1.ln3_g + cp) : tb_f2{0.f, 0.f};
                pg2[par][p] = okc ? *reinterpret_cast<const tb_f2*>(q1.ln2_g + cp) : tb_f2{0.f, 0.f};
                pb2[par][p] = (okc && !q1.n2) ? *reinterpret_cast<const tb_f2*>(q1.ln2_b + cp) : tb_f2{0.f, 0.f};
            }
        tb_f2 in_dy[8][2], in_r2[8][2], in_n2[8][2];
#pragma unroll
        for (int rr = 0; rr < 8; ++rr)
#pragma unroll
            for (int p = 0; p < 2; ++p) {
                const int cp = 4 * lane - ((rr & 1) ? 2 : 0) + 2 * p;
                const long long sb = (long long)b * (TB_L * TB_D);
                const unsigned o = (unsigned)((8 * w + rr) * TB_D + cp);
                const bool okc = cp >= 0 && cp < TB_D;
                in_dy[rr][p] = okc ? *reinterpret_cast<const tb_f2*>(q1.dn3 + sb + o) : tb_f2{0.f, 0.f};
                in_r2[rr][p] = okc ? *reinterpret_cast<const tb_f2*>(q1.r2 + sb + o) : tb_f2{0.f, 0.f};
                in_n2[rr][p] = (okc && q1.n2) ? *reinterpret_cast<const tb_f2*>(q1.n2 + sb + o) : tb_f2{0.f, 0.f};
            }
#pragma unroll
        for (int rr = 0; rr < 8; ++rr) {
            const int r = 8 * w + rr, c0 = 4 * lane - ((rr & 1) ? 2 : 0);
            const long long row = (long long)b * TB_L + r, rbase = row * TB_D;
            float dy[4], x3[4], x2[4], g3[4], g2[4];
            bool ok[2];
#pragma unroll
            for (int p = 0; p < 2; ++p) {
                const int cp = c0 + 2 * p;
                ok[p] = cp >= 0 && cp < TB_D;
                const tb_f2 v0 = in_dy[rr][p], v2 = in_r2[rr][p], v3 = pg3[rr & 1][p], v4 = pg2[rr & 1][p];
                tb_f2 v1 = in_n2[rr][p];
                if (ok[p] && !q1.n2) {
                    const tb_f2 bb = pb2[rr & 1][p];
                    const float mu = q1.mu2[row], rs = q1.rs2[row];
                    v1 = tb_f2{(v2[0] - mu) * rs * v4[0] + bb[0], (v2[1] - mu) * rs * v4[1] + bb[1]};
                }
#pragma unroll
                for (int e = 0; e < 2; ++e) { dy[2 * p + e] = v0[e]; x3[2 * p + e] = v1[e]; x2[2 * p + e] = v2[e]; g3[2 * p + e] = v3[e]; g2[2 * p + e] = v4[e]; }
            }
            float dn2[4], dr2[4];
            if (rr & 1) {
                tb_ln_bwd_row(dy, x3, g3, ok, q1.mu3[row], q1.rs3[row], dn2, po[0], po[1]);
                tb_ln_bwd_row(dn2, x2, g2, ok, q1.mu2[row], q1.rs2[row], dr2, po[2], po[3]);
            } else {
                tb_ln_bwd_row(dy, x3, g3, ok, q1.mu3[row], q1.rs3[row], dn2, pe[0], pe[1]);
                tb_ln_bwd_row(dn2, x2, g2, ok, q1.mu2[row], q1.rs2[row], dr2, pe[2], pe[3]);
            }
            bool keep[4] = {true, true, true, true};
            if (TRAIN && q1.drop_p > 0.f && c0 < TB_D) dropout_keep4(q1.seed, q1.site_ffn_out, (unsigned long long)(rbase + c0), q1.drop_p, keep);
#pragma unroll
            for (int p = 0; p < 2; ++p) {
                const int cp = c0 + 2 * p;
                const float d0 = (TRAIN && q1.drop_p > 0.f) ? (keep[2 * p] ? dr2[2 * p] * ksc : 0.f) : dr2[2 * p];
                const float d1 = (TRAIN && q1.drop_p > 0.f) ? (keep[2 * p + 1] ? dr2[2 * p + 1] * ksc : 0.f) : dr2[2 * p + 1];
                if (ok[p]) *reinterpret_cast<tb_f2*>(XF + xf_off(r, cp)) = tb_f2{dr2[2 * p], dr2[2 * p + 1]};
                if (cp >= 0 && cp < 256) tb_store_planes2(AP, TB_AP_PLANE, ap_off(r, cp), ok[p] ? d0 : 0.f, ok[p] ? d1 : 0.f);
            }
            if ((rr & 1) && lane == 63) tb_store_planes2(AP, TB_AP_PLANE, ap_off(r, 254), 0.f, 0.f);
        }
        tb_reduce_partials<4>(SC, w, lane, t, pe, po, part);
    }
    raw_barrier();

    const tb_bwd_args q2 = tb_args_again(a0);
    {
        f32x4 acc[4][2];
        tb_gemm<2, 3u, TB_BWD_PF, true, true>(AP, q2.packed + TB_OFF_2T + (long long)(2 * w) * TB_KS * TB_TILE, lane, acc);
        f32x4 fpre[4][2];
#pragma unroll
        for (int mt = 0; mt < 4; ++mt)
#pragma unroll
            for (int j = 0; j < 2; ++j)
                fpre[mt][j] = *reinterpret_cast<const f32x4*>(q2.f1 + (long long)b * (TB_L * TB_FF) + (unsigned)((16 * mt + (lane & 15)) * TB_FF + 32 * w + 16 * j + 4 * (lane >> 4)));
        tb_planes_out<64>(AP, q2.df2p + (long long)b * (2 * TB_AP_PLANE), t);
        tb_for_tiles(w, lane, TB_FF, acc, [&](int m, int n0, int valid, f32x4& v) {
            const long long ob = (long long)b * (TB_L * TB_FF);
            const unsigned ol = (unsigned)(m * TB_FF + n0);
            const f32x4 f = fpre[m >> 4][(n0 >> 4) & 1];
            bool keep[4] = {true, true, true, true};
            if (TRAIN && q2.drop_p > 0.f) dropout_keep4(q2.seed, q2.site_ffn_act, (unsigned long long)ob + ol, q2.drop_p, keep);
#pragma unroll
            for (int i = 0; i < 4; ++i) {
                const float d = (TRAIN && q2.drop_p > 0.f) ? (keep[i] ? v[i] * ksc : 0.f) : v[i];
                v[i] = d * gelu_erf_grad(f[i]);
            }
        });
        raw_barrier();
        tb_for_tiles(w, lane, TB_FF, acc, [&](int m, int n0, int valid, f32x4& v) {
            tb_store_planes4(AP, TB_AP_PLANE, ap_off(m, n0), v[0], v[1], v[2], v[3]);
        });
    }
    raw_barrier();

    const tb_bwd_args q3 = tb_args_again(a0);
    {
        f32x4 acc[4][2];
        tb_gemm<2, 3u, TB_BWD_PF, true, true>(AP, q3.packed + TB_OFF_1T + (long long)(2 * w) * TB_KS * TB_TILE, lane, acc);
        tb_for_tiles(w, lane, TB_D, acc, [&](int m, int n0, int valid, f32x4& v) {
            f32x4* p = reinterpret_cast<f32x4*>(XF + xf_off(m, n0));
            f32x4 o = *p;
#pragma unroll
            for (int i = 0; i < 4; ++i) o[i] = i < valid ? o[i] + v[i] : 0.f;
            *p = o;
        });
        tb_planes_out<64>(AP, q3.dg1p + (long long)b * (2 * TB_AP_PLANE), t);
    }
    raw_barrier();

    const tb_bwd_args q4 = tb_args_again(a0);
    {
        float pe[2][4], po[2][4];
#pragma unroll
        for (int v = 0; v < 2; ++v)
#pragma unroll
            for (int e = 0; e < 4; ++e) { pe[v][e] = 0.f; po[v][e] = 0.f; }
        tb_f2 pg1[2][2], in_r1[8][2];
#pragma unroll
        for (int par = 0; par < 2; ++par)
#pragma unroll
            for (int p = 0; p < 2; ++p) {
                const int cp = 4 * lane - 2 * par + 2 * p;
                pg1[par][p] = (cp >= 0 && cp < TB_D) ? *reinterpret_cast<const tb_f2*>(q4.ln1_g + cp) : tb_f2{0.f, 0.f};
            }
#pragma unroll
        for (int rr = 0; rr < 8; ++rr)
#pragma unroll
            for (int p = 0; p < 2; ++p) {
                const int cp = 4 * lane - ((rr & 1) ? 2 : 0) + 2 * p;
                in_r1[rr][p] = (cp >= 0 && cp < TB_D) ? *reinterpret_cast<const tb_f2*>(q4.r1 + (long long)b * (TB_L * TB_D) + (unsigned)((8 * w + rr) * TB_D + cp)) : tb_f2{0.f, 0.f};
            }
#pragma unroll
        for (int rr = 0; rr < 8; ++rr) {
            const int r = 8 * w + rr, c0 = 4 * lane - ((rr & 1) ? 2 : 0);
            const long long row = (long long)b * TB_L + r, rbase = row * TB_D;
            float dy[4], x1[4], g1[4];
            bool ok[2];
#pragma unroll
            for (int p = 0; p < 2; ++p) {
                const int cp = c0 + 2 * p;
                ok[p] = cp >= 0 && cp < TB_D;
                tb_f2 v0 = tb_f2{0.f, 0.f};
                const tb_f2 v1 = in_r1[rr][p], v2 = pg1[rr & 1][p];
                if (ok[p]) v0 = *reinterpret_cast<const tb_f2*>(XF + xf_off(r, cp));
#pragma unroll
                for (int e = 0; e < 2; ++e) { dy[2 * p + e] = v0[e]; x1[2 * p + e] = v1[e]; g1[2 * p + e] = v2[e]; }
            }
            float dr1[4];
            if (rr & 1) tb_ln_bwd_row(dy, x1, g1, ok, q4.mu1[row], q4.rs1[row], dr1, po[0], po[1]);
            else tb_ln_bwd_row(dy, x1, g1, ok, q4.mu1[row], q4.rs1[row], dr1, pe[0], pe[1]);
            bool keep[4] = {true, true, true, true};
            if (TRAIN && q4.drop_p > 0.f && c0 < TB_D) dropout_keep4(q4.seed, q4.site_attn_out, (unsigned long long)(rbase + c0), q4.drop_p, keep);
#pragma unroll
            for (int p = 0; p < 2; ++p) {
                const int cp = c0 + 2 * p;
                const float d0 = (TRAIN && q4.drop_p > 0.f) ? (keep[2 * p] ? dr1[2 * p] * ksc : 0.f) : dr1[2 * p];
                const float d1 = (TRAIN && q4.drop_p > 0.f) ? (keep[2 * p + 1] ? dr1[2 * p + 1] * ksc : 0.f) : dr1[2 * p + 1];
                if (ok[p]) {
                    *reinterpret_cast<tb_f2*>(q4.dr1 + rbase + (unsigned)cp) = tb_f2{dr1[2 * p], dr1[2 * p + 1]};
                }
                if (cp >= 0 && cp < 256) tb_store_planes2(AP, TB_AP_PLANE, ap_off(r, cp), ok[p] ? d0 : 0.f, ok[p] ? d1 : 0.f);
            }
            if ((rr & 1) && lane == 63) tb_store_planes2(AP, TB_AP_PLANE, ap_off(r, 254), 0.f, 0.f);
        }
        raw_barrier();
        tb_reduce_partials<2>(SC, w, lane, t, pe, po, part + 4 * 256);
    }
    raw_barrier();

    const tb_bwd_args q5 = tb_args_again(a0);
    {
        f32x4 acc[4][2];
        tb_gemm<2, 3u, TB_BWD_PF, true, true>(AP, q5.packed + TB_OFF_OT + (long long)(2 * w) * TB_KS * TB_TILE, lane, acc);
        tb_for_tiles(w, lane, 256, acc, [&](int m, int n0, int valid, f32x4& v) {
            const int head = n0 >> 6, d0 = n0 & 63;
            if (d0 < TB_E) tb_st4(q5.dctx + (long long)b * (TB_L * TB_HE) + (unsigned)(m * TB_HE + head * TB_E + d0), TB_E - d0 >= 4 ? 4 : 2, v);
        });
        tb_planes_out<64>(AP, q5.da1p + (long long)b * (2 * TB_AP_PLANE), t);
    }
}

template <bool TRAIN>
__global__ __launch_bounds__(TB_THREADS, 2) void token_block_bwd_b_kernel(const tb_bwd_args a) {
    EEG_LDS_BASE(unsigned char, lds);
    unsigned char* const AP = lds;
    unsigned char* const XF = lds + TB_AP_BYTES;
    const int t = threadIdx.x, lane = t & 63, w = wave_uniform(t >> 6);
    const int b = blockIdx.x;
    const float ksc = (TRAIN && a.drop_p > 0.f) ? 1.f / (1.f - a.drop_p) : 1.f;
    f32x4 acc[4][2];
    auto dma_planes = [&](int which, unsigned char* dst) {
        const unsigned char* src = a.dqkvp + ((long long)which * gridDim.x + b) * (2 * TB_AP_PLANE);
#pragma unroll
        for (int i = 0; i < 8; ++i) {
            const int plane = i >> 2, row = 8 * w + 2 * (i & 3) + (lane >> 5), c = lane & 31;
            lds_dma16(dst + plane * TB_AP_PLANE + (8 * w + 2 * (i & 3)) * 512, src + plane * TB_AP_PLANE + row * 512 + ((c ^ (row & 15)) << 4));
        }
    };
    dma_planes(0, AP);
    dma_planes(1, XF);
    wait_vmcnt<8>();
    raw_barrier();
    tb_gemm<2, 3u, TB_BWD_PF, true, true>(AP, a.packed + TB_OFF_QT + (long long)(2 * w) * TB_KS * TB_TILE, lane, acc);
    raw_barrier();
    dma_planes(2, AP);
    wait_vmcnt<8>();
    raw_barrier();
    tb_gemm<2, 3u, TB_BWD_PF, false, true>(XF, a.packed + TB_OFF_QT + TB_MAT_ELEMS + (long long)(2 * w) * TB_KS * TB_TILE, lane, acc);
    wait_vmcnt<0>();
    raw_barrier();
    tb_gemm<2, 3u, TB_BWD_PF, false, true>(AP, a.packed + TB_OFF_QT + 2 * TB_MAT_ELEMS + (long long)(2 * w) * TB_KS * TB_TILE, lane, acc);
    raw_barrier();
    tb_for_tiles(w, lane, TB_D, acc, [&](int m, int n0, int valid, f32x4& v) {
        const f32x4 r = tb_ld4(a.dr1 + (long long)b * (TB_L * TB_D) + (unsigned)(m * TB_D + n0), valid);
        f32x4 o;
#pragma unroll
        for (int i = 0; i < 4; ++i) o[i] = i < valid ? r[i] + v[i] : 0.f;
        *reinterpret_cast<f32x4*>(XF + xf_off(m, n0)) = o;
    });
    __syncthreads();
    float* ob = a.dr1 + (long long)b * (TB_L * TB_D);
#pragma unroll
    for (int j = 0; j < 8; ++j) {
        const int q = t + TB_THREADS * j;
        if (q < TB_L * TB_D / 4) {
            const int i0 = 4 * q, row = i0 / TB_D, col = i0 - TB_D * row;
            const bool wrap = col + 2 >= TB_D;
            const int row2 = wrap ? row + 1 : row, col2 = wrap ? col + 2 - TB_D : col + 2;
            const tb_f2 p0 = *reinterpret_cast<const tb_f2*>(XF + xf_off(row, col)), p1 = *reinterpret_cast<const tb_f2*>(XF + xf_off(row2, col2));
            float v[4] = {p0[0], p0[1], p1[0], p1[1]};
            if (TRAIN && a.drop_p > 0.f) {
                bool keep[4];
                dropout_keep4(a.seed, a.site_embed, (unsigned long long)b * (TB_L * TB_D) + i0, a.drop_p, keep);
#pragma unroll
                for (int e = 0; e < 4; ++e) v[e] = keep[e] ? v[e] * ksc : 0.f;
            }
            *reinterpret_cast<f32x4*>(ob + i0) = f32x4{v[0], v[1], v[2], v[3]};
            if (a.dr1p) {
                tb_store_planes2(AP, TB_AP_PLANE, ap_off(row, col), v[0], v[1]);
                tb_store_planes2(AP, TB_AP_PLANE, ap_off(row2, col2), v[2], v[3]);
            }
        }
    }
    if (a.dr1p) {
        if (t < 128) {
            const int row = t & 63, plane = t >> 6;
#pragma unroll
            for (int k = 250; k < 256; k += 2) *reinterpret_cast<unsigned*>(AP + plane * TB_AP_PLANE + ap_off(row, k)) = 0u;
        }
        raw_barrier();
        tb_planes_out<64>(AP, a.dr1p + (long long)b * (2 * TB_AP_PLANE), t);
    }
}

struct tb_param_args {
    const float* partials;
    float* out[6];
    int B;
};
__global__ __launch_bounds__(256) void token_block_param_reduce_kernel(const tb_param_args a) {
    EEG_LDS_BASE(float, red);
    const int v = blockIdx.y, lane = threadIdx.x & 63, g = threadIdx.x >> 6;
    const int c = blockIdx.x * 64 + lane;
    const int per = (a.B + (int)gridDim.z - 1) / (int)gridDim.z, b0 = (int)blockIdx.z * per, b1 = b0 + per < a.B ? b0 + per : a.B;
    float s = 0.f;
#pragma unroll 4
    for (int b = b0 + g; b < b1; b += 4) s += a.partials[((long long)b * 6 + v) * 256 + c];
    red[g * 64 + lane] = s;
    __syncthreads();
    if (g == 0 && c < TB_D) atomicAdd(a.out[v] + c, (red[lane] + red[64 + lane]) + (red[128 + lane] + red[192 + lane]));
}

}

using namespace eeg;

extern "C" long long eegclip_token_block_packed_bytes(void) { return TB_PACKED_ELEMS * 2; }

extern "C" int eegclip_token_block_pack(const float* wv, const float* wqkv, const float* wo, const float* w1, const float* w2, void* packed, void* stream) {
    if (!wv || !wqkv || !wo || !w1 || !w2 || !packed) return EEGCLIP_EINVAL;
    if (reinterpret_cast<uintptr_t>(packed) & 15u) return EEGCLIP_EALIGN;
    const int tiles = (int)(TB_PACKED_ELEMS / TB_TILE);
    tb_pack_args a{{wv, wqkv, wo, w1, w2, w2, w1, wo, wqkv, wqkv, wqkv}, static_cast<unsigned short*>(packed), tiles, nullptr, nullptr, nullptr, 0};
    EEG_LAUNCH(token_block_pack_kernel, dim3(tiles), dim3(64), 0, stream, a);
    return (int)hipGetLastError();
}

extern "C" int eegclip_weight_prep(const float* wv, const float* wqkv, const float* wo, const float* w1, const float* w2, void* packed, const float* Ws,
                                   void* cs_packed, void* cs_packed_t, int H, void* stream) {
    if (!wv || !wqkv || !wo || !w1 || !w2 || !packed || !Ws || !cs_packed || H < 1 || H > CS_MAXH) return EEGCLIP_EINVAL;
    if ((reinterpret_cast<uintptr_t>(packed) | reinterpret_cast<uintptr_t>(cs_packed) | reinterpret_cast<uintptr_t>(cs_packed_t)) & 15u) return EEGCLIP_EALIGN;
    const int tiles = (int)(TB_PACKED_ELEMS / TB_TILE);
    tb_pack_args a{{wv, wqkv, wo, w1, w2, w2, w1, wo, wqkv, wqkv, wqkv}, static_cast<unsigned short*>(packed), tiles, Ws, static_cast<unsigned char*>(cs_packed),
                   static_cast<unsigned char*>(cs_packed_t), H};
    const int extra = (cs_pack_items(H, cs_packed_t != nullptr) + 63) / 64;
    EEG_LAUNCH(token_block_pack_kernel, dim3(tiles + extra), dim3(64), 0, stream, a);
    return (int)hipGetLastError();
}

namespace eeg {
__global__ __launch_bounds__(64) void token_block_pack_embed_kernel(const float* __restrict__ w0, long long w_stride, unsigned short* __restrict__ out) {
    const int tile = blockIdx.x, s = blockIdx.y;
    const int nt = tile / TB_KS, ks = tile % TB_KS;
    const int lane = threadIdx.x & 63;
    const int n = 16 * nt + (lane & 15), k0 = 32 * ks + 8 * (lane >> 4);
    const float* src = w0 + (long long)s * w_stride;
    unsigned hb[8], lb[8];
#pragma unroll
    for (int e = 0; e < 8; ++e) {
        const long long si = tb_src_index(0, n, k0 + e);
        const float v = si >= 0 ? src[si] : 0.f;
        const unsigned short h = f32_to_bf16_bits(v);
        hb[e] = h;
        lb[e] = f32_to_bf16_bits(v - bf16_bits_to_f32(h));
    }
    unsigned short* dst = out + (long long)s * TB_MAT_ELEMS + (long long)tile * TB_TILE + lane * 8;
    tb_u4 oh, ol;
#pragma unroll
    for (int e = 0; e < 4; ++e) {
        oh[e] = hb[2 * e] | (hb[2 * e + 1] << 16);
        ol[e] = lb[2 * e] | (lb[2 * e + 1] << 16);
    }
    *reinterpret_cast<tb_u4*>(dst) = oh;
    *reinterpret_cast<tb_u4*>(dst + 512) = ol;
}
}

extern "C" long long eegclip_token_block_packed_embed_bytes(int n_subjects) { return n_subjects < 1 ? 0 : (long long)n_subjects * TB_MAT_ELEMS * 2; }

extern "C" int eegclip_token_block_pack_embed(const float* w0, long long w_stride, int n_subjects, void* out, void* stream) {
    if (!w0 || !out || n_subjects < 1 || n_subjects > 65535 || w_stride < (long long)TB_D * TB_T) return EEGCLIP_EINVAL;
    if (reinterpret_cast<uintptr_t>(out) & 15u) return EEGCLIP_EALIGN;
    EEG_LAUNCH(token_block_pack_embed_kernel, dim3(16 * TB_KS, (unsigned)n_subjects), dim3(64), 0, stream, w0, w_stride, static_cast<unsigned short*>(out));
    return (int)hipGetLastError();
}

extern "C" int eegclip_token_block_fwd(const eegclip_token_block_desc* d, void* stream) {
    if (!d || d->B < 1 || !d->x || !d->packed || !d->bv || !d->pe || !d->tokens || !d->bqkv || !d->bo || !d->ln1_g || !d->ln1_b || !d->b1 || !d->b2 ||
        !d->ln2_g || !d->ln2_b || !d->ln3_g || !d->ln3_b || !d->h || !d->qkv || !d->ctxp || !d->r1 || !d->n1p || !d->mu1 || !d->rs1 || !d->f1 || !d->g1p ||
        !d->hp || !d->r2 || !d->mu2 || !d->rs2 || !d->n3 || !d->mu3 || !d->rs3 || d->drop_p < 0.f || d->drop_p >= 1.f)
        return EEGCLIP_EINVAL;
    const uintptr_t al16 = reinterpret_cast<uintptr_t>(d->packed) | reinterpret_cast<uintptr_t>(d->h) | reinterpret_cast<uintptr_t>(d->f1) |
                           reinterpret_cast<uintptr_t>(d->b1) | reinterpret_cast<uintptr_t>(d->xp) | reinterpret_cast<uintptr_t>(d->hp) |
                           reinterpret_cast<uintptr_t>(d->ctxp) | reinterpret_cast<uintptr_t>(d->n1p) | reinterpret_cast<uintptr_t>(d->g1p);
    const uintptr_t al8 = reinterpret_cast<uintptr_t>(d->x) | reinterpret_cast<uintptr_t>(d->qkv) |
                          reinterpret_cast<uintptr_t>(d->r1) | reinterpret_cast<uintptr_t>(d->r2) |
                          reinterpret_cast<uintptr_t>(d->n2) | reinterpret_cast<uintptr_t>(d->n3) | reinterpret_cast<uintptr_t>(d->bv) |
                          reinterpret_cast<uintptr_t>(d->pe) | reinterpret_cast<uintptr_t>(d->tokens) | reinterpret_cast<uintptr_t>(d->bqkv) |
                          reinterpret_cast<uintptr_t>(d->bo) | reinterpret_cast<uintptr_t>(d->b2) | reinterpret_cast<uintptr_t>(d->ln1_g) |
                          reinterpret_cast<uintptr_t>(d->ln1_b) | reinterpret_cast<uintptr_t>(d->ln2_g) | reinterpret_cast<uintptr_t>(d->ln2_b) |
                          reinterpret_cast<uintptr_t>(d->ln3_g) | reinterpret_cast<uintptr_t>(d->ln3_b);
    if ((al16 & 15u) || (al8 & 7u)) return EEGCLIP_EALIGN;
    tb_fwd_args a{d->x, static_cast<const unsigned short*>(d->packed), d->bv, d->pe, d->tokens, d->ids, d->bqkv, d->bo, d->ln1_g, d->ln1_b, d->b1, d->b2,
                  d->ln2_g, d->ln2_b, d->ln3_g, d->ln3_b, d->h, d->qkv, d->r1, d->mu1, d->rs1, d->f1, d->r2, d->n2, d->mu2, d->rs2,
                  d->n3, d->mu3, d->rs3, static_cast<unsigned char*>(d->xp), static_cast<unsigned char*>(d->hp), static_cast<unsigned char*>(d->ctxp),
                  static_cast<unsigned char*>(d->n1p), static_cast<unsigned char*>(d->g1p), d->drop_p, d->eps, d->scale, d->seed, d->site_embed, d->site_attn,
                  d->site_attn_out, d->site_ffn_act, d->site_ffn_out, 0u, nullptr, static_cast<const unsigned short*>(d->packed_embed), d->embed_subject,
                  d->embed_subject ? d->bv_stride : 0, d->cs_w25, d->cs_bias, d->cs_rows, d->cs_H};
    if (d->cs_rows && (!d->cs_w25 || !d->cs_bias || d->cs_H < 1 || d->cs_H > CS_MAXH || (reinterpret_cast<uintptr_t>(d->cs_rows) & 7u))) return EEGCLIP_EINVAL;
    static_assert(CS_LDS_S + CS_LDS_PS <= TB_LDS && CS_NT == TB_THREADS, "the conv stack's statistics pass runs in the block kernel's workgroup");
    if (d->embed_subject && (!d->packed_embed || (reinterpret_cast<uintptr_t>(d->packed_embed) & 15u) || d->bv_stride < 0 || (d->bv_stride & 1))) return EEGCLIP_EINVAL;
    static const unsigned dbg = getenv("EEGCLIP_TB_DEBUG") ? (unsigned)atoi(getenv("EEGCLIP_TB_DEBUG")) : 0u;
    if ((dbg & 1u) && (d->xp || d->hp || d->ctxp || d->n1p || d->g1p)) return EEGCLIP_EINVAL;
    a.dbg = dbg;
    a.tstamp = nullptr;
#if !defined(EEG_EMU)
    static unsigned long long* stamps = nullptr;
    static int calls = 0;
    if ((dbg & 2u) && d->B <= 4096) {
        if (!stamps && hipMalloc(&stamps, 4096 * 16 * sizeof(unsigned long long)) != hipSuccess) stamps = nullptr;
        a.tstamp = stamps;
    }
#endif
    if (d->drop_p > 0.f) EEG_LAUNCH(token_block_fwd_kernel<true>, dim3(d->B), dim3(TB_THREADS), TB_LDS, stream, a);
    else EEG_LAUNCH(token_block_fwd_kernel<false>, dim3(d->B), dim3(TB_THREADS), TB_LDS, stream, a);
#if !defined(EEG_EMU)
    if (a.tstamp && ++calls % 20 == 0) {
        hipStreamSynchronize((hipStream_t)stream);
        static unsigned long long host[4096 * 16];
        hipMemcpy(host, stamps, (size_t)d->B * 16 * sizeof(unsigned long long), hipMemcpyDeviceToHost);
        double ph[9] = {0};
        for (int b = 0; b < d->B; ++b)
            for (int k = 0; k < 9; ++k) ph[k] += (double)(host[b * 16 + k + 1] - host[b * 16 + k]);
        fprintf(stderr, "token_block_fwd phases (s_memtime ticks, mean of %d workgroups): x->planes %.0f | embed GEMM %.0f | dropout+h %.0f | qkv+attention %.0f | out-proj %.0f | "
                        "LN1 %.0f | FFN1 %.0f | FFN2 %.0f | LN2+LN3 %.0f\n", d->B, ph[0] / d->B, ph[1] / d->B, ph[2] / d->B, ph[3] / d->B, ph[4] / d->B, ph[5] / d->B,
                ph[6] / d->B, ph[7] / d->B, ph[8] / d->B);
        double q[4] = {0};
        for (int b = 0; b < d->B; ++b) {
            const unsigned long long* h = host + b * 16;
            q[0] += (double)(h[10] - h[3]); q[1] += (double)(h[11] - h[10]); q[2] += (double)(h[12] - h[11]); q[3] += (double)(h[13] - h[12]);
        }
        fprintf(stderr, "  qkv+attention: qkv(heads 0,1) %.0f | attention %.0f | qkv(heads 2,3) + h planes out %.0f | attention %.0f\n", q[0] / d->B, q[1] / d->B, q[2] / d->B,
                q[3] / d->B);
    }
#endif
    return (int)hipGetLastError();
}

extern "C" long long eegclip_token_block_bwd_workspace_floats(int B) { return B < 1 ? 0 : (long long)B * 6 * 256; }

extern "C" int eegclip_token_block_bwd(const eegclip_token_block_bwd_desc* d, int part, void* stream) {
    if (!d || d->B < 1 || !d->packed || d->drop_p < 0.f || d->drop_p >= 1.f || part < 0 || part > 2) return EEGCLIP_EINVAL;
    tb_bwd_args a{static_cast<const unsigned short*>(d->packed), d->dn3, d->n2, d->r2, d->r1, d->f1, d->mu1, d->rs1, d->mu2, d->rs2, d->mu3, d->rs3,
                  d->ln1_g, d->ln2_g, d->ln2_b, d->ln3_g, d->dr1, d->dctx, d->partials, static_cast<unsigned char*>(d->df2p), static_cast<unsigned char*>(d->dg1p),
                  static_cast<unsigned char*>(d->da1p), static_cast<unsigned char*>(d->dr1p), static_cast<const unsigned char*>(d->dqkvp), d->drop_p, d->seed,
                  d->site_embed, d->site_attn_out, d->site_ffn_act, d->site_ffn_out};
    if (part == 0) {
        if (!d->dn3 || (!d->n2 && !d->ln2_b) || !d->r2 || !d->r1 || !d->f1 || !d->mu1 || !d->rs1 || !d->mu2 || !d->rs2 || !d->mu3 || !d->rs3 || !d->ln1_g || !d->ln2_g ||
            !d->ln3_g || !d->df2p || !d->dg1p || !d->da1p || !d->dr1 || !d->dctx || !d->partials)
            return EEGCLIP_EINVAL;
        const uintptr_t al16 = reinterpret_cast<uintptr_t>(d->packed) | reinterpret_cast<uintptr_t>(d->f1) | reinterpret_cast<uintptr_t>(d->df2p) |
                               reinterpret_cast<uintptr_t>(d->dg1p) | reinterpret_cast<uintptr_t>(d->da1p);
        const uintptr_t al8 = reinterpret_cast<uintptr_t>(d->dn3) | reinterpret_cast<uintptr_t>(d->n2) | reinterpret_cast<uintptr_t>(d->r2) |
                              reinterpret_cast<uintptr_t>(d->r1) | reinterpret_cast<uintptr_t>(d->ln1_g) | reinterpret_cast<uintptr_t>(d->ln2_g) |
                              reinterpret_cast<uintptr_t>(d->ln3_g) | reinterpret_cast<uintptr_t>(d->dr1) | reinterpret_cast<uintptr_t>(d->dctx);
        if ((al16 & 15u) || (al8 & 7u)) return EEGCLIP_EALIGN;
        if (d->drop_p > 0.f) EEG_LAUNCH(token_block_bwd_a_kernel<true>, dim3(d->B), dim3(TB_THREADS), TB_LDS, stream, a);
        else EEG_LAUNCH(token_block_bwd_a_kernel<false>, dim3(d->B), dim3(TB_THREADS), TB_LDS, stream, a);
    } else if (part == 1) {
        if (!d->dqkvp || !d->dr1) return EEGCLIP_EINVAL;
        if ((reinterpret_cast<uintptr_t>(d->packed) | reinterpret_cast<uintptr_t>(d->dr1) | reinterpret_cast<uintptr_t>(d->dqkvp) | reinterpret_cast<uintptr_t>(d->dr1p)) & 15u)
            return EEGCLIP_EALIGN;
        if (d->drop_p > 0.f) EEG_LAUNCH(token_block_bwd_b_kernel<true>, dim3(d->B), dim3(TB_THREADS), TB_AP_BYTES + TB_XF_BYTES, stream, a);
        else EEG_LAUNCH(token_block_bwd_b_kernel<false>, dim3(d->B), dim3(TB_THREADS), TB_AP_BYTES + TB_XF_BYTES, stream, a);
    } else {
        if (!d->partials || !d->dln3_g || !d->dln3_b || !d->dln2_g || !d->dln2_b || !d->dln1_g || !d->dln1_b) return EEGCLIP_EINVAL;
        tb_param_args pa{d->partials, {d->dln3_g, d->dln3_b, d->dln2_g, d->dln2_b, d->dln1_g, d->dln1_b}, d->B};
        EEG_LAUNCH(token_block_param_reduce_kernel, dim3(4, 6, d->B < 16 ? d->B : 16), dim3(256), 256 * sizeof(float), stream, pa);
    }
    return (int)hipGetLastError();
}
```

include/eegclip.h:

```cpp
#ifndef EEGCLIP_H
#define EEGCLIP_H

#ifdef __cplusplus
extern "C" {
#endif

#define EEGCLIP_ABI_VERSION 14
#define EEGCLIP_EINVAL (-1)
#define EEGCLIP_EALIGN (-2)

int eegclip_abi_version(void);

typedef struct {
    long long div, so, si;
} eegclip_dim;

#define EEGCLIP_ACT_NONE 0
#define EEGCLIP_ACT_GELU 1
#define EEGCLIP_ACT_SILU 2
#define EEGCLIP_ACT_GELU_GRAD 3

#define EEGCLIP_PREC_F32 0
#define EEGCLIP_PREC_BF16X3 1

typedef struct {
    int M, N, K;
    const float* A;
    eegclip_dim Am, Ak;
    const float* B;
    eegclip_dim Bk, Bn;
    float* C;
    eegclip_dim Cm, Cn;
    float* Cpre;
    const float* bias_n;
    const float* bias_m;
    const float* R;
    eegclip_dim Rm, Rn;
    float alpha;
    int accumulate;
    int act;
    float drop_p;
    unsigned long long seed;
    unsigned int drop_site;
    int split_k;
    float* rowsum_a;
    int precision;
    float* workspace;
    long long workspace_bytes;
} eegclip_gemm_desc;

typedef struct {
    const float* src;
    void* hi;
    void* lo;
    int rows, cols;
    long long ld_src, ld_out;
    int transpose;
    float* copy;
    long long ld_copy;
} eegclip_split_item;
int eegclip_split_rows(const eegclip_split_item* items, int n, void* stream);
int eegclip_gemm_f32(const eegclip_gemm_desc* d, void* stream);
long long eegclip_gemm_workspace_bytes(const eegclip_gemm_desc* d);
int eegclip_gemm_f32_grouped(const eegclip_gemm_desc* descs, int n, void* stream);

int eegclip_layernorm_fwd(const float* x, const float* gamma, const float* beta, float* y, float* mean, float* rstd,
                          int rows, int cols, float eps, void* stream);
int eegclip_residual_layernorm_fwd(const float* x, const float* resid, float* x_out, float drop_p, unsigned long long seed, unsigned int site,
                                   const float* gamma, const float* beta, float* y, float* mean, float* rstd, const float* gamma2,
                                   const float* beta2, float* y2, float* mean2, float* rstd2, int rows, int cols, float eps, void* stream);
int eegclip_residual_layernorm_fwd_planes(const float* x, const float* resid, float* x_out, float drop_p, unsigned long long seed, unsigned int site,
                                          const float* gamma, const float* beta, float* y, float* mean, float* rstd, const float* gamma2,
                                          const float* beta2, float* y2, float* mean2, float* rstd2, int rows, int cols, float eps, void* y_hi, void* y_lo,
                                          void* stream);
int eegclip_layernorm_bwd(const float* dy, const float* x, const float* gamma, const float* mean, const float* rstd,
                          float* dx, float* dgamma, float* dbeta, int rows, int cols, int accumulate_dx, float* dx_drop, float drop_p,
                          unsigned long long seed, unsigned int site, void* stream);
long long eegclip_layernorm_bwd_full_workspace_floats(int rows, int cols);
int eegclip_layernorm_bwd_full(const float* dy, const float* x, const float* gamma, const float* mean, const float* rstd, float* dx, float* dgamma,
                               float* dbeta, int rows, int cols, int accumulate_dx, float* dx_drop, float drop_p, unsigned long long seed,
                               unsigned int site, float* workspace, void* stream);
long long eegclip_layernorm_bwd_params_workspace_floats(int rows, int cols);
int eegclip_layernorm_bwd_params(const float* dy, const float* x, const float* mean, const float* rstd, float* dgamma, float* dbeta,
                                 int rows, int cols, float* workspace, void* stream);

int eegclip_layernorm_silu_fwd(const float* x, const float* gamma, const float* beta, float* y_ln, float* y_act, float* mean, float* rstd,
                               int rows, int cols, float eps, float drop_p, unsigned long long seed, unsigned int site, void* stream);
int eegclip_silu_bwd(const float* dy, const float* pre, float* dx, long long n, int accumulate, float drop_p, unsigned long long seed,
                     unsigned int site, void* stream);

int eegclip_bn_stats(const float* x, int outer, int C, int inner, double* sums, void* stream);
int eegclip_bn_finalize(const double* sums, double count, float eps, float momentum, int C, float* mean, float* rstd,
                        float* running_mean, float* running_var, int train, long long* num_batches_tracked, void* stream);
int eegclip_bn_finalize_rows(const double* rows, int nrows, double count, float eps, float momentum, int C, float* mean, float* rstd,
                             float* running_mean, float* running_var, long long* num_batches_tracked, double* sums_out, void* stream);
int eegclip_bn_elu_fwd(const float* x, const float* mean, const float* rstd, const float* gamma, const float* beta, float* y,
                       int outer, int C, int inner, float drop_p, unsigned long long seed, unsigned int site, void* stream);
int eegclip_bn_elu_bwd(const float* dz, const float* x, const float* mean, const float* rstd, const float* gamma, const float* beta,
                       double* sums, float* dx, float* dgamma, float* dbeta, int outer, int C, int inner, float drop_p,
                       unsigned long long seed, unsigned int site, void* stream);

int eegclip_bn_elu_bwd_stats(const float* dz, const float* x, const float* mean, const float* rstd, const float* gamma, const float* beta,
                             double* sums, int outer, int C, int inner, float drop_p, unsigned long long seed, unsigned int site, void* stream);
int eegclip_bn_elu_bwd_apply(const float* dz, const float* x, const float* mean, const float* rstd, const float* gamma, const float* beta,
                             const double* sums, const double* sums_local, double count, float* dx, float* dgamma, float* dbeta, int outer, int C, int inner, float drop_p,
                             unsigned long long seed, unsigned int site, void* stream);

int eegclip_embed_finish(float* h, const float* tokens, const long long* ids, int B, int L, int D, float drop_p,
                         unsigned long long seed, unsigned int site, void* stream);
int eegclip_embed_finish_bwd(float* dh, float* dtokens, const long long* ids, int B, int L, int D, float drop_p,
                             unsigned long long seed, unsigned int site, void* stream);

int eegclip_dropout_scale(float* x, long long n, float drop_p, unsigned long long seed, unsigned int site, void* stream);
int eegclip_gelu_bwd(const float* dy, const float* pre, float* dx, long long n, int accumulate, float drop_p,
                     unsigned long long seed, unsigned int site, void* stream);
int eegclip_bias_act(const float* acc, const float* bias_n, float* pre, const float* resid, float* out, int M, int N, int act, float drop_p,
                     unsigned long long seed, unsigned int site, void* stream);
int eegclip_axpby(const float* x, float* y, long long n, float a, float b, void* stream);
int eegclip_reduce_mid(const float* x, int outer, int mid, int inner, float* out, void* stream);
int eegclip_colsum_blocks(const float* x, int nblk, int blk_rows, int row0, int cols, long long blk_stride, float* out, void* stream);
int eegclip_sumsq(const float* x, long long n, double* out, void* stream);
int eegclip_stage_eeg(const double* src, float* dst, long long n_items, int reps, int channels, int T, const int* tidx, int Tw, int mean_reps,
                      void* stream);
int eegclip_gather_rows(float* dst, long long dst_stride, const float* src, long long src_stride, const int* idx, int n, int row_floats,
                        int scatter, void* stream);

int eegclip_adamw_step(float* p, const float* g, float* m, float* v, long long n, float lr, float beta1, float beta2, float eps,
                       float weight_decay, long long step, float grad_scale, const float* grad_scale_dev, void* stream);
int eegclip_adamw_step_zero_grad(float* p, float* g, float* m, float* v, long long n, float lr, float beta1, float beta2, float eps,
                                 float weight_decay, long long step, float grad_scale, const float* grad_scale_dev, void* stream);
int eegclip_clip_scale(const double* sumsq, float max_norm, float* scale_out, void* stream);

int eegclip_timestep_embedding(const float* t, int n, int dim, float* out, void* stream);
int eegclip_ddpm_add_noise(const float* h, const float* noise, const long long* t, const float* sqrt_acp, const float* sqrt_1macp,
                           float* out, int n, int d, void* stream);
int eegclip_ddpm_step(const float* x, const float* eps_c, const float* eps_u, float guidance, float sa, float sb, float c0, float ct,
                      float sigma, const float* noise, float* out, float* out_dup, long long n, void* stream);
int eegclip_prior_stage_infer(const float* x, const float* gamma, const float* beta, const float* skip, float* act_out, const float* te,
                              const float* ce, int ce_rows, float* xin_out, int rows, int cols, float eps, void* stream);
int eegclip_mse_loss_grad(const float* pred, const float* target, long long n, float* loss, float* dpred, void* stream);
int eegclip_mse_loss_grad_scaled(const float* pred, const float* target, long long n, float weight, float* loss, float* dpred, void* stream);

int eegclip_attention_fwd(const float* qkv, float* ctx, int B, int L, int H, int E, int ld, float scale, float drop_p,
                          unsigned long long seed, unsigned int site, void* stream);
int eegclip_attention_bwd(const float* qkv, const float* dctx, float* dqkv, int B, int L, int H, int E, int ld, float scale,
                          float drop_p, unsigned long long seed, unsigned int site, void* stream);
int eegclip_attention_bwd_x3(const float* qkv, const float* dctx, void* dqkv, int dqkv_planes, int B, int L, int H, int E, int ld, float scale,
                          float drop_p, unsigned long long seed, unsigned int site, void* stream);

long long eegclip_tsconv_fwd_workspace_floats(int B, int H);
int eegclip_tsconv_fwd(const float* x, long long xs_b, long long xs_h, const float* w25, const float* bias, float* y, int B, int H,
                       int T, int C, double* sums, float* workspace, void* stream);
long long eegclip_tsconv_bwd_w_workspace_floats(int B, int H);
int eegclip_tsconv_bwd_w(const float* x, long long xs_b, long long xs_h, const float* dy, float* dw25, float* workspace, int B, int H,
                         int T, int C, void* stream);
int eegclip_tsconv_bwd_x(const float* dy, const float* w25, float* dx, long long xs_b, long long xs_h, int B, int H, int T, int C,
                         void* stream);

int eegclip_sconv_fwd(const float* y1, const float* mean, const float* rstd, const float* gamma, const float* beta, const float* Ws,
                      const float* bs, float* y2, double* sums2, int B, int H, int y2_is_zero, float* workspace, void* stream);
long long eegclip_sconv_fwd_workspace_floats(int B);
long long eegclip_sconv_bwd_w_workspace_floats(int B, int H);
int eegclip_sconv_bwd_w(const float* y1, const float* mean, const float* rstd, const float* gamma, const float* beta, const float* dy2,
                        float* dWs, float* workspace, int B, int H, int precision, void* stream);
long long eegclip_sconv_bwd_x_stats_workspace_floats(int B);
int eegclip_sconv_bwd_x_stats(const float* dy2, const float* Ws, const void* WsT_hi, const void* WsT_lo, const float* y1, const float* mean,
                              const float* rstd, const float* gamma, const float* beta, double* sums, float* workspace, int B, int H, void* stream);
int eegclip_sconv_bwd_x_apply(const float* dy2, const float* Ws, const void* WsT_hi, const void* WsT_lo, const float* y1, const float* mean,
                              const float* rstd, const float* gamma, const float* beta, const double* sums, const double* sums_local,
                              double count, float* dy1, float* dgamma, float* dbeta, int B, int H, void* stream);

int eegclip_lse_rows(const float* X, int rows, int cols, long long ld, const float* scale, float* lse, void* stream);
int eegclip_lse_cols(const float* X, int rows, int cols, long long ld, const float* scale, float* lse, void* stream);
int eegclip_infonce_grad(float* X, int rows, int cols, long long ld, int col0, int n_total, const float* scale, const float* lse_r,
                         const float* lse_c, float weight, float* loss, float* dscale, void* stream);
int eegclip_infonce_loss(const float* X, int n, long long ld, const float* scale, const float* lse_r, const float* lse_c, float weight,
                         float* loss, void* stream);

#define EEGCLIP_DT_BF16 0
#define EEGCLIP_DT_F16 1

int eegclip_gemm16(const void* A, long long lda, const void* W, long long ldw, void* C, long long ldc, const void* bias, const void* R, long long ldr,
                   int r_div, int M, int N, int K, int dtype, void* stream);
int eegclip_sampler_step(const void* x, const void* eps_u, const void* eps_c, const void* noise, void* out, void* scaled, float guidance, float cx,
                         float ce, float cn, float in_scale, long long n, int dtype, void* stream);

typedef struct {
    const void* q_hi;
    const void* q_lo;
    const void* k_hi;
    const void* k_lo;
    int col0;
    float weight;
    float* part;
    float* diag;
    float* lse;
    const float* lse_k;
    float* G;
    long long ldg;
    const float* part_k;
    const float* diag_k;
    void *G_hi, *G_lo;
} eegclip_infonce_problem;
int eegclip_split_bf16(const float* x, void* hi, void* lo, long long n, void* stream);
int eegclip_infonce_fused_supported(int n, int N, int D);
long long eegclip_infonce_fused_workspace_floats(int n, int N);
int eegclip_infonce_fused_fwd(const eegclip_infonce_problem* blocks, int n_blocks, int n, int N, int D, int planes, int n_total,
                              const float* scale, float* loss, void* stream);
int eegclip_infonce_fused_grad(const eegclip_infonce_problem* blocks, int n_blocks, int n, int N, int D, int planes, int n_total,
                               const float* scale, float* dscale, void* stream);
int eegclip_infonce_fused_grad_finalize(const eegclip_infonce_problem* blocks, int n_blocks, int n, int N, int D, int planes, int n_total,
                                        const float* scale, float* loss, float* dscale, void* stream);

int eegclip_proj1x1_fwd(const float* y2, const float* mean, const float* rstd, const float* gamma, const float* beta, const float* W,
                        const float* bias, float* z2, float* feat, int B, float drop_p, unsigned long long seed, unsigned int site, void* stream);
int eegclip_proj1x1_fwd_rows(const float* y2, const double* rows, int nrows, double count, float eps, float momentum, float* mean, float* rstd,
                             float* running_mean, float* running_var, long long* num_batches_tracked, const float* gamma, const float* beta, const float* W,
                             const float* bias, float* z2, float* feat, int B, float drop_p, unsigned long long seed, unsigned int site, void* stream);
long long eegclip_proj1x1_bwd_workspace_floats(int B);
int eegclip_proj1x1_bwd(const float* dfeat, const float* z2, const float* W, const float* y2, const float* mean, const float* rstd,
                        const float* gamma, const float* beta, float* dz2, float* dW, float* dbias, double* sums, float* workspace, int B,
                        float drop_p, unsigned long long seed, unsigned int site, void* stream);

int eegclip_cast_bf16(const float* x, void* y_bf16, long long n, void* stream);
int eegclip_logits_bf16(const void* a_bf16, const void* b_bf16, float* c, int M, int N, int K, long long ldc, const float* scale, void* stream);

int eegclip_cross_attn_fwd(const void* q, const void* k, const void* v, const void* k_ip, const void* v_ip, void* out, int B, int HW, int heads,
                           int head_dim, int S, int S_ip, float ip_scale, int dtype, void* stream);

int eegclip_self_attn_supported(int head_dim, long long ldq, long long ldk, long long ldv, long long ldo);
int eegclip_self_attn_fwd(const void* q, long long ldq, const void* k, long long ldk, const void* v, long long ldv, void* out, long long ldo, int B,
                          int Tq, int Tk, int heads, int head_dim, float scale, int dtype, void* stream);
int eegclip_self_attn_causal_fwd(const void* q, long long ldq, const void* k, long long ldk, const void* v, long long ldv, void* out, long long ldo, int B,
                                 int Tq, int Tk, int heads, int head_dim, float scale, int dtype, void* stream);

int eegclip_topk_rows(const float* X, int rows, int cols, long long ld, int k, const float* scale ,
                      long long* out_idx, void* stream);
int eegclip_count_equal(const long long* pred, int stride, const long long* labels, int n, int* count, void* stream);
int eegclip_top1_count(const float* X, int rows, int cols, long long ld, const float* scale, const long long* labels, int* count, void* stream);

typedef union {
    void* p;
    long long i;
    unsigned long long u;
    double d;
    float f;
    int i32;
    unsigned int u32;
} eegclip_plan_arg;
#define EEGCLIP_PLAN_MAX_ARGS 28
typedef struct {
    int fn;
    int flags;
    eegclip_plan_arg a[EEGCLIP_PLAN_MAX_ARGS];
} eegclip_plan_op;
#define EEGCLIP_PLAN_MEMSET (-2)
#define EEGCLIP_PLAN_JOIN (-3)
#define EEGCLIP_PLAN_SIDE 1
#define EEGCLIP_PLAN_SKIP 2
#define EEGCLIP_PLAN_SIDE2 4
int eegclip_plan_fn_id(const char* name);
int eegclip_plan_events(int n, void** out);
int eegclip_plan_events_destroy(int n, void* const* events);
int eegclip_plan_run(const eegclip_plan_op* ops, int begin, int end, int n_total, void* main_stream, void* side_stream, void* side_stream2,
                     void* const* events, void* join_event, void* join_event2, int* dirty, int* failed);

typedef struct {
    int B;
    const float* x;
    const void* packed;
    const float *bv, *pe, *tokens;
    const long long* ids;
    const float *bqkv, *bo, *ln1_g, *ln1_b, *b1, *b2, *ln2_g, *ln2_b, *ln3_g, *ln3_b;
    float *h, *qkv, *r1, *mu1, *rs1, *f1, *r2, *n2, *mu2, *rs2, *n3, *mu3, *rs3;
    void *xp, *hp, *ctxp, *n1p, *g1p;
    float drop_p, eps, scale;
    unsigned long long seed;
    unsigned int site_embed, site_attn, site_attn_out, site_ffn_act, site_ffn_out;
    const void* packed_embed;
    const int* embed_subject;
    long long bv_stride;
    const float *cs_w25, *cs_bias;
    double* cs_rows;
    int cs_H;
} eegclip_token_block_desc;
long long eegclip_token_block_packed_bytes(void);
int eegclip_token_block_pack(const float* wv, const float* wqkv, const float* wo, const float* w1, const float* w2, void* packed, void* stream);
int eegclip_weight_prep(const float* wv, const float* wqkv, const float* wo, const float* w1, const float* w2, void* packed, const float* Ws, void* cs_packed,
                        void* cs_packed_t, int H, void* stream);
long long eegclip_token_block_packed_embed_bytes(int n_subjects);
int eegclip_token_block_pack_embed(const float* w0, long long w_stride, int n_subjects, void* out, void* stream);
int eegclip_token_block_fwd(const eegclip_token_block_desc* d, void* stream);

typedef struct {
    int B;
    const void* packed;
    const float *dn3, *n2, *r2, *r1, *f1, *mu1, *rs1, *mu2, *rs2, *mu3, *rs3, *ln1_g, *ln2_g, *ln2_b, *ln3_g;
    float *dr1, *dctx, *partials;
    void *df2p, *dg1p, *da1p, *dr1p;
    const void* dqkvp;
    float *dln3_g, *dln3_b, *dln2_g, *dln2_b, *dln1_g, *dln1_b;
    float drop_p;
    unsigned long long seed;
    unsigned int site_embed, site_attn_out, site_ffn_act, site_ffn_out;
} eegclip_token_block_bwd_desc;
long long eegclip_token_block_bwd_workspace_floats(int B);
int eegclip_token_block_bwd(const eegclip_token_block_bwd_desc* d, int part, void* stream);

typedef struct {
    const void *a_hi, *a_lo, *b_hi, *b_lo;
    long long lda, ldb;
    int M, N, K;
    float* C;
    long long ldc;
    float* Cpre;
    long long ldcpre;
    const float* bias;
    const float* R;
    long long ldr;
    void *p_hi, *p_lo;
    long long ldp;
    int act, accumulate, planes_of;
} eegclip_gemm_planes_desc;
int eegclip_gemm_planes(const eegclip_gemm_planes_desc* d, void* stream);

int eegclip_split_transpose(const eegclip_split_item* items, int n, void* stream);

int eegclip_infonce_small_supported(int n, int T);
long long eegclip_infonce_small_workspace_floats(int n, int T);
int eegclip_infonce_small_fwd(const float* slabs, int nslabs, long long slab_stride, int n, int T, const float* scale, float* workspace, void* stream);
int eegclip_infonce_small_grad(int n, int T, const float* scale, const float* workspace, float w0, float w1, float w2, float w3, void* g_hi, void* g_lo,
                               long long ldg, float* loss, float* dscale, void* stream);

typedef struct {
    const void* in;
    const void* W;
    void* out;
    const void* bias;
    const void* residual;
    int N, Hi, Wi, Cin, in_pad;
    int Ho, Wo, Cout, out_pad;
    int KS, stride, pad_top, pad_left, upsample, dtype;
    const void* chan_bias;
} eegclip_conv16_desc;
int eegclip_conv16(const eegclip_conv16_desc* d, void* stream);
int eegclip_groupnorm16(const void* x, int N, int H, int W, int C, int pad, int groups, const void* gamma, const void* beta, float eps, int silu, void* y,
                        int out_pad, double* sums, int dtype, void* stream);
int eegclip_softmax_rows16(void* s, int rows, int cols, long long ld, float scale, int dtype, void* stream);
int eegclip_vae_sample16(const void* moments, const void* noise, void* z, long long pixels, int latent_channels, int dtype, void* stream);

int eegclip_layernorm16(const void* x, long long ldx, const void* gamma, const void* beta, void* y, long long ldy, int rows, int C, float eps, int dtype,
                        void* stream);
int eegclip_geglu16(const void* x, void* y, int M, int D, int dtype, void* stream);
int eegclip_concat16(const void* a, const void* b, void* out, int N, int H, int W, int pad, int Ca, int Cb, int out_pad, int dtype, void* stream);

int eegclip_gather_rows16(const void* table, long long table_rows, const void* idx, int idx64, const void* add, int add_rows, void* out, int rows, int C,
                          int dtype, void* stream);
int eegclip_act16(const void* x, long long ldx, void* y, long long ldy, int M, int D, int kind, int dtype, void* stream);

typedef struct {
    const void *a_hi, *a_lo, *b_hi, *b_lo;
    long long lda, ldb;
    int M, N, K, slices;
    long long slab_stride;
    const float* bias;
    float* Cpre;
    long long ldcpre;
    int act;
    const float* aux;
    long long ldaux;
    const float* R;
    long long ldr;
    float* C;
    long long ldc;
    void *p_hi, *p_lo;
    long long ldp;
    int b_kmajor;
} eegclip_head_gemm_desc;
int eegclip_head_gemm_slices(int M, int N, int K);
int eegclip_head_gemm(const eegclip_head_gemm_desc* d, void* stream);
int eegclip_head_act(const float* slabs, int nslabs, long long slab_stride, const float* bias, float* pre, float* out, void* out_hi, void* out_lo, int M, int N,
                     void* stream);
int eegclip_head_act_bwd(const float* slabs, int nslabs, long long slab_stride, const float* pre, const float* base, float* dx, void* dx_hi, void* dx_lo,
                         long long n, void* stream);
int eegclip_residual_layernorm_fwd_slabs(const float* x, const float* resid, float* x_out, float drop_p, unsigned long long seed, unsigned int site,
                                         const float* gamma, const float* beta, float* y, float* mean, float* rstd, const float* gamma2, const float* beta2,
                                         float* y2, float* mean2, float* rstd2, int rows, int cols, float eps, void* y_hi, void* y_lo, int nslabs,
                                         long long slab_stride, const float* x_bias, void* stream);
int eegclip_layernorm_bwd_slabs(const float* dy, int nslabs, long long slab_stride, const float* x, const float* gamma, const float* mean, const float* rstd,
                                float* dx, int rows, int cols, float* dx_drop, void* dd_hi, void* dd_lo, float* dy_sum, float drop_p, unsigned long long seed,
                                unsigned int site, void* stream);
int eegclip_proj1x1_bwd_slabs(const float* dfeat, int nslabs, long long slab_stride, const float* z2, const float* W, const float* y2, const float* mean,
                              const float* rstd, const float* gamma, const float* beta, float* dz2, float* dW, float* dbias, double* sums, float* workspace,
                              int B, float drop_p, unsigned long long seed, unsigned int site, void* stream);
int eegclip_proj1x1_fwd_rows_planes(const float* y2, const double* rows, int nrows, double count, float eps, float momentum, float* mean, float* rstd,
                                    float* running_mean, float* running_var, long long* num_batches_tracked, const float* gamma, const float* beta,
                                    const float* W, const float* bias, float* z2, float* feat, int B, float drop_p, unsigned long long seed,
                                    unsigned int site, void* feat_hi, void* feat_lo, const eegclip_split_item* riders, int n_riders, void* stream);
int eegclip_proj1x1_bwd_rows(const float* dfeat, int nslabs, long long slab_stride, const float* z2, const float* W, const float* y2, const float* mean,
                             const float* rstd, const float* gamma, const float* beta, float* dz2, float* workspace, double* bn_rows, int B, float drop_p,
                             unsigned long long seed, unsigned int site, void* stream);
int eegclip_proj1x1_bwd_reduce(const float* workspace, int B, float* dW, float* dbias, double* sums, void* stream);
int eegclip_bn_elu_bwd_apply_rows(const float* dz, const float* x, const float* mean, const float* rstd, const float* gamma, const float* beta,
                                  const double* rows, int nrows, long long ld, int col0, double count, float* dx, float* dgamma, float* dbeta, int outer, int C,
                                  int inner, float drop_p, unsigned long long seed, unsigned int site, void* stream);
int eegclip_prior_stage_fwd(const float* x, const float* gamma, const float* beta, const float* skip, float* y_ln, float* y_act, float* mean, float* rstd,
                            void* act_hi, void* act_lo, int rows, int cols, float eps, float drop_p, unsigned long long seed, unsigned int site, void* stream);
int eegclip_prior_stage_bwd(const float* dact, const float* y_ln, const float* x, const float* gamma, const float* mean, const float* rstd, float* dx,
                            void* dx_hi, void* dx_lo, float* dgamma, float* dbeta, int rows, int cols, float drop_p, unsigned long long seed,
                            unsigned int site, float* workspace, void* stream);
long long eegclip_prior_stage_bwd_workspace_floats(int rows, int cols);
int eegclip_prior_stage_bwd_params(const float* workspace, int rows, int cols, float* dgamma, float* dbeta, void* stream);
int eegclip_silu_bwd_planes(const float* dy, const float* pre, void* dx_hi, void* dx_lo, long long n, void* stream);

typedef struct {
    const void* a;
    const void* b;
    long long a_group_stride;
    int m_groups, heads_m, heads_n;
    int M, N;
    float* out;
    long long ldo;
    float* bias_out;
    int bias_mfma;
    int sample0, samples;
    const int* sample_index;
} eegclip_wgrad_tok_problem;
int eegclip_wgrad_tok_slices(int total_m_groups, int B);
long long eegclip_wgrad_tok_workspace_floats(const eegclip_wgrad_tok_problem* p, int n_prob, int B, int slices);
int eegclip_wgrad_tok(const eegclip_wgrad_tok_problem* p, int n_prob, int B, int slices, float* workspace, int variant, void* stream);
int eegclip_wgrad_tok_reduce(const eegclip_wgrad_tok_problem* p, int n_prob, int B, int slices, float* workspace, void* stream);
int eegclip_wgrad_tok_reduce_adamw(const eegclip_wgrad_tok_problem* p, int n_prob, int B, int slices, float* workspace, float* P, float* G, float* M, float* V,
                                   long long n, float lr, float beta1, float beta2, float eps, float weight_decay, long long step, void* stream);
typedef struct {
    const void *a_hi, *a_lo;
    long long lda;
    const void *b_hi, *b_lo;
    long long ldb;
    int rows, M, N;
    float* out;
    long long ldo;
    float* bias_out;
    int slices;
} eegclip_wgrad_planes_problem;
int eegclip_wgrad_planes(const eegclip_wgrad_planes_problem* p, int n_prob, void* stream);
int eegclip_tok_planes_from_f32(const float* src, long long ld, int rows, int cols, int heads, int ones, void* dst, void* stream);

typedef struct {
    int B, H;
    const float* x;
    long long xs_b, xs_h;
    const float *w25, *bias1;
    const double* stat1;
    int nstat1;
    double count1;
    float eps, momentum;
    const float *gamma1, *beta1;
// ... 53 lines not shown
```

Before: 396,100 samples/s.

## Fuse attention backward into token-block backward part B kernel

Moves the per-head attention backward body into a shared header and adds a fused token-block backward kernel. The new kernel computes dQ/dK/dV for all heads in LDS, writes the dqkv planes, and immediately runs the QKV input-gradient GEMM and the rest of the old part-B work. This replaces two launches with one and avoids a global round trip of dqkv before the dr1 computation. In exchange the kernel needs more LDS, which may reduce occupancy, and the attention work now runs with only one block per sample instead of one per (sample, head). The old EEGCLIP_WGRAD_MERGE option is removed, so weight-gradient merging is always late.

```diff
diff --git a/eeg_image_decode_amd/_abi.py b/eeg_image_decode_amd/_abi.py
--- a/eeg_image_decode_amd/_abi.py
+++ b/eeg_image_decode_amd/_abi.py
@@ -57,7 +57,8 @@
                 + [(k, C.c_void_p) for k in ("dr1", "dctx", "partials", "df2p", "dg1p", "da1p", "dr1p", "dqkvp")]
                 + [(k, C.c_void_p) for k in ("dln3_g", "dln3_b", "dln2_g", "dln2_b", "dln1_g", "dln1_b")]
                 + [("drop_p", C.c_float), ("seed", C.c_ulonglong)]
-                + [(k, C.c_uint) for k in ("site_embed", "site_attn_out", "site_ffn_act", "site_ffn_out")])
+                + [(k, C.c_uint) for k in ("site_embed", "site_attn_out", "site_ffn_act", "site_ffn_out")]
+                + [("qkv", C.c_void_p), ("scale", C.c_float), ("site_attn", C.c_uint)])
 
 
 class GemmPlanesDesc(C.Structure):
@@ -122,7 +123,7 @@
 
 ACT_NONE, ACT_GELU, ACT_SILU, ACT_GELU_GRAD = 0, 1, 2, 3
 PREC_F32, PREC_BF16X3 = 0, 1
-ABI_VERSION = 14
+ABI_VERSION = 15
 DT_BF16, DT_F16 = 0, 1
 _P, _I, _F, _L, _U64, _U, _D = C.c_void_p, C.c_int, C.c_float, C.c_longlong, C.c_ulonglong, C.c_uint, C.c_double
 
diff --git a/eeg_image_decode_amd/atms.py b/eeg_image_decode_amd/atms.py
--- a/eeg_image_decode_amd/atms.py
+++ b/eeg_image_decode_amd/atms.py
@@ -853,7 +853,8 @@
                 dr1=_p(b["dr1"]), dctx=_p(b["dctx"]), partials=_p(b["tb_part"]), df2p=df2p, dg1p=dg1p, da1p=da1p, dr1p=dr1p, dqkvp=dqkvp,
                 dln3_g=_p(G["encoder.encoder.norm.weight"]), dln3_b=_p(G["encoder.encoder.norm.bias"]), dln2_g=_p(G[_LY + "norm2.weight"]),
                 dln2_b=_p(G[_LY + "norm2.bias"]), dln1_g=_p(G[_LY + "norm1.weight"]), dln1_b=_p(G[_LY + "norm1.bias"]),
-                drop_p=pe_, seed=0, site_embed=SITE_EMBED, site_attn_out=SITE_ATTN_OUT, site_ffn_act=SITE_FFN_ACT, site_ffn_out=SITE_FFN_OUT)
+                drop_p=pe_, seed=0, site_embed=SITE_EMBED, site_attn_out=SITE_ATTN_OUT, site_ffn_act=SITE_FFN_ACT, site_ffn_out=SITE_FFN_OUT,
+                qkv=_p(b["qkv"]), scale=1.0 / math.sqrt(D_HEAD), site_attn=SITE_ATTN)
             pl._keep.append(bd)
             if pe_ > 0.0:
                 pl._seed_descs.append(bd)
@@ -875,8 +876,6 @@
                 pl.call("eegclip_wgrad_tok_reduce", arr, len(problems), B, slices, _p(b[key]), side=side)
                 return arr, ops
 
-            merge = int(os.environ.get("EEGCLIP_WGRAD_MERGE", "2"))
-            late = []
             ffn_out = [
                 (_LY + "conv2.weight", df2p, 1, g1p, D_MODEL, D_FF, 0, 0, _LY + "conv2.bias", 1),
                 (_LY + "conv1.weight", dg1p, 1, n1p, D_FF, D_MODEL, 0, 0, _LY + "conv1.bias", 0),
@@ -887,17 +886,8 @@
                 pl.deferred.append(lambda: pl.call("eegclip_token_block_bwd", ctypes.byref(bd), 2, side=True))
             else:
                 pl.call("eegclip_token_block_bwd", ctypes.byref(bd), 2, side=ln_side)
-            if merge >= 2:
-                late += ffn_out
-            else:
-                wgrad_tok("ffn_out", ffn_out)
-            pl.call(attn_bwd, _p(b["qkv"]), _p(b["dctx"]), dqkvp, 1, B, L_TOK, N_HEADS, D_HEAD, 3 * HE, 1.0 / math.sqrt(D_HEAD),
-                    pe_, 0, SITE_ATTN, seed_at=11)
-            if merge >= 1:
-                late += qkv_w
-            else:
-                wgrad_tok("qkv", qkv_w)
-            pl.call("eegclip_token_block_bwd", ctypes.byref(bd), 1)
+            late = ffn_out + qkv_w
+            pl.call("eegclip_token_block_bwd", ctypes.byref(bd), 3)
         else:
             pl.call("eegclip_layernorm_bwd_full", _p(b["dn3"]), _p(b["n2"]), _p(P["encoder.encoder.norm.weight"]), _p(b["mu3"]), _p(b["rs3"]), _p(b["dn2"]),
                     _p(G["encoder.encoder.norm.weight"]), _p(G["encoder.encoder.norm.bias"]), R, D_MODEL, 0, None, 0.0, 0, 0, lnf_ws)
diff --git a/eeg_image_decode_amd/csrc/attention_x3.hip b/eeg_image_decode_amd/csrc/attention_x3.hip
--- a/eeg_image_decode_amd/csrc/attention_x3.hip
+++ b/eeg_image_decode_amd/csrc/attention_x3.hip
@@ -1,11 +1,6 @@
-#include "eeg_common.h"
+#include "attention_x3_body.h"
 
 namespace eeg {
-
-constexpr int AX_L = 64;
-constexpr int AX_RS = 144;
-constexpr int AX_PLANE = AX_L * AX_RS;
-constexpr int AX_TENSOR = 2 * AX_PLANE;
 
 struct ax_args {
     const float* qkv;
@@ -18,42 +13,6 @@
     unsigned site;
 };
 
-typedef short ax_s4 __attribute__((ext_vector_type(4)));
-typedef float ax_f2 __attribute__((ext_vector_type(2)));
-typedef float ax_f4u __attribute__((ext_vector_type(4), aligned(4)));
-
-__device__ __forceinline__ ax_s4 ax_tr_read(const unsigned char* p) {
-#if defined(EEG_EMU)
-    const int lane = hipemu::cur->lane, g = lane >> 4, i = lane & 15;
-    ax_s4 r;
-    for (int j = 0; j < 4; ++j) {
-        const unsigned long long src = hipemu::shfl_idx((unsigned long long)(uintptr_t)p, 16 * g + 4 * j + (i >> 2));
-        r[j] = reinterpret_cast<const short*>((uintptr_t)src)[i & 3];
-    }
-    return r;
-#else
-    return __builtin_amdgcn_ds_read_tr16_b64_v4i16((__attribute__((address_space(3))) ax_s4*)(p));
-#endif
-}
-__device__ __forceinline__ bf16x8 ax_tr_frag(const unsigned char* plane, int r0, int r1, int c0, int lane) {
-    const int l = lane & 15;
-    const ax_s4 a = ax_tr_read(plane + (r0 + (l >> 2)) * AX_RS + 2 * (c0 + 4 * (l & 3)));
-    const ax_s4 b = ax_tr_read(plane + (r1 + (l >> 2)) * AX_RS + 2 * (c0 + 4 * (l & 3)));
-    return bf16x8{a[0], a[1], a[2], a[3], b[0], b[1], b[2], b[3]};
-}
-__device__ __forceinline__ bf16x8 ax_frag(const unsigned char* plane, int row, int k0) {
-    return *reinterpret_cast<const bf16x8*>(plane + row * AX_RS + 2 * k0);
-}
-__device__ __forceinline__ bf16x8 ax_pack8(u32x2_t a, u32x2_t b) {
-    typedef unsigned u4 __attribute__((ext_vector_type(4)));
-    const u4 v{a[0], a[1], b[0], b[1]};
-    return __builtin_bit_cast(bf16x8, v);
-}
-__device__ __forceinline__ f32x4 ax_mfma3(bf16x8 ah, bf16x8 al, bf16x8 bh, bf16x8 bl, f32x4 c) {
-    c = mfma_bf16_16x16x32(al, bh, c);
-    c = mfma_bf16_16x16x32(ah, bl, c);
-    return mfma_bf16_16x16x32(ah, bh, c);
-}
 __device__ __forceinline__ void ax_store4(float* p, int valid, f32x4 v) {
     if (valid >= 4) *reinterpret_cast<ax_f4u*>(p) = ax_f4u{v[0], v[1], v[2], v[3]};
     else if (valid >= 2) {
@@ -73,166 +32,35 @@
 __global__ __launch_bounds__(256, 2) void attention_bwd_x3_kernel(const ax_args a) {
     EEG_LDS_BASE(float, ldsf);
     unsigned char* lds = reinterpret_cast<unsigned char*>(ldsf);
-    unsigned char* Qp = lds;
-    unsigned char* Kp = lds + AX_TENSOR;
-    unsigned char* Vp = lds + 2 * AX_TENSOR;
-    unsigned char* Op = lds + 3 * AX_TENSOR;
     const int t = threadIdx.x, lane = t & 63, w = wave_uniform(t >> 6), fr = lane & 15, g = lane >> 4;
     const int bh = blockIdx.x, b = bh / a.H, h = bh - b * a.H;
     const int E = a.E, HE = a.H * E;
-    const float* qrow0 = a.qkv + (long long)b * AX_L * a.ld + h * E;
-    const float* orow0 = a.dctx + (long long)b * AX_L * HE + h * E;
 
     {
         ax_f2 v[4][8];
-#pragma unroll
-        for (int j = 0; j < 8; ++j) {
-            const int idx = t + 256 * j, row = idx >> 5, col = 2 * (idx & 31);
-            const bool ok = col < E;
-            const float* qr = qrow0 + (long long)row * a.ld + col;
-            v[0][j] = ok ? *reinterpret_cast<const ax_f2*>(qr) : ax_f2{0.f, 0.f};
-            v[1][j] = ok ? *reinterpret_cast<const ax_f2*>(qr + HE) : ax_f2{0.f, 0.f};
-            v[2][j] = ok ? *reinterpret_cast<const ax_f2*>(qr + 2 * HE) : ax_f2{0.f, 0.f};
-            v[3][j] = ok ? *reinterpret_cast<const ax_f2*>(orow0 + (long long)row * HE + col) : ax_f2{0.f, 0.f};
-        }
-#pragma unroll
-        for (int x = 0; x < 4; ++x)
-#pragma unroll
-            for (int j = 0; j < 8; ++j) {
-                const int idx = t + 256 * j, row = idx >> 5, col = 2 * (idx & 31);
-                const unsigned hi = x3_pack2(v[x][j][0], v[x][j][1]);
-                const float r0 = v[x][j][0] - __uint_as_float(hi << 16), r1 = v[x][j][1] - __uint_as_float(hi & 0xffff0000u);
-                unsigned char* dst = lds + x * AX_TENSOR + row * AX_RS + 2 * col;
-                *reinterpret_cast<unsigned*>(dst) = hi;
-                *reinterpret_cast<unsigned*>(dst + AX_PLANE) = x3_pack2(r0, r1);
-            }
+        ax_stage_load(v, a.qkv + (long long)b * AX_L * a.ld + h * E, a.dctx + (long long)b * AX_L * HE + h * E, t, a.ld, HE, E);
+        ax_stage_store(v, lds, t);
     }
     __syncthreads();
 
-    f32x4 s[4], dp[4];
-#pragma unroll
-    for (int kt = 0; kt < 4; ++kt) { s[kt] = f32x4{0.f, 0.f, 0.f, 0.f}; dp[kt] = f32x4{0.f, 0.f, 0.f, 0.f}; }
-#pragma unroll
-    for (int ks = 0; ks < 2; ++ks) {
-        const int k0 = 32 * ks + 8 * g;
-        const bf16x8 qh = ax_frag(Qp, 16 * w + fr, k0), ql = ax_frag(Qp + AX_PLANE, 16 * w + fr, k0);
-        const bf16x8 oh = ax_frag(Op, 16 * w + fr, k0), ol = ax_frag(Op + AX_PLANE, 16 * w + fr, k0);
-#pragma unroll
-        for (int kt = 0; kt < 4; ++kt) {
-            const bf16x8 kh = ax_frag(Kp, 16 * kt + fr, k0), kl = ax_frag(Kp + AX_PLANE, 16 * kt + fr, k0);
-            const bf16x8 vh = ax_frag(Vp, 16 * kt + fr, k0), vl = ax_frag(Vp + AX_PLANE, 16 * kt + fr, k0);
-            s[kt] = ax_mfma3(kh, kl, qh, ql, s[kt]);
-            dp[kt] = ax_mfma3(vh, vl, oh, ol, dp[kt]);
-        }
-    }
-    float mx = -INFINITY;
-#pragma unroll
-    for (int kt = 0; kt < 4; ++kt)
-#pragma unroll
-        for (int r = 0; r < 4; ++r) {
-            s[kt][r] *= a.scale;
-            mx = fmaxf(mx, s[kt][r]);
-        }
-    mx = fmaxf(mx, __shfl_xor(mx, 16, 64));
-    mx = fmaxf(mx, __shfl_xor(mx, 32, 64));
-    float sum = 0.f;
-#pragma unroll
-    for (int kt = 0; kt < 4; ++kt)
-#pragma unroll
-        for (int r = 0; r < 4; ++r) {
-            s[kt][r] = expf(s[kt][r] - mx);
-            sum += s[kt][r];
-        }
-    sum += __shfl_xor(sum, 16, 64);
-    sum += __shfl_xor(sum, 32, 64);
-    const float inv = 1.0f / sum;
-    const bool drop = TRAIN && a.drop_p > 0.f;
-    const float ksc = drop ? 1.f / (1.f - a.drop_p) : 1.f;
-    f32x4 pd[4];
-    float dq_sum = 0.f;
-#pragma unroll
-    for (int kt = 0; kt < 4; ++kt) {
-        bool keep[4] = {true, true, true, true};
-        if (drop) {
-            const unsigned long long idx0 = ((unsigned long long)bh * AX_L + 16 * w + fr) * AX_L + 16 * kt + 4 * g;
-            dropout_keep4(a.seed, a.site, idx0, a.drop_p, keep);
-        }
-#pragma unroll
-        for (int r = 0; r < 4; ++r) {
-            const float p = s[kt][r] * inv;
-            const float d = keep[r] ? dp[kt][r] * ksc : 0.f;
-            pd[kt][r] = keep[r] ? p * ksc : 0.f;
-            s[kt][r] = p;
-            dp[kt][r] = d;
-            dq_sum += p * d;
-        }
-    }
-    dq_sum += __shfl_xor(dq_sum, 16, 64);
-    dq_sum += __shfl_xor(dq_sum, 32, 64);
-#pragma unroll
-    for (int kt = 0; kt < 4; ++kt)
-#pragma unroll
-        for (int r = 0; r < 4; ++r) dp[kt][r] = s[kt][r] * (dp[kt][r] - dq_sum);
-
-    {
-        f32x4 dq[4];
-#pragma unroll
-        for (int et = 0; et < 4; ++et) dq[et] = f32x4{0.f, 0.f, 0.f, 0.f};
-#pragma unroll
-        for (int m = 0; m < 2; ++m) {
-            u32x2_t h0, l0, h1, l1;
-            x3_split4(dp[2 * m][0], dp[2 * m][1], dp[2 * m][2], dp[2 * m][3], h0, l0);
-            x3_split4(dp[2 * m + 1][0], dp[2 * m + 1][1], dp[2 * m + 1][2], dp[2 * m + 1][3], h1, l1);
-            const bf16x8 bhf = ax_pack8(h0, h1), blf = ax_pack8(l0, l1);
+    f32x4 dk[4], dv[4];
+    ax_head_bwd<TRAIN>(
+        lds, w, lane, bh, a.scale, a.drop_p, a.seed, a.site, [] { __syncthreads(); },
+        [&](f32x4(&dq)[4]) {
+            float* out = a.dqkv + ((long long)b * AX_L + 16 * w + fr) * a.ld + h * E;
+            unsigned char* outp = a.dqkvp + (long long)b * 65536 + (16 * w + fr) * 512 + 128 * h;
 #pragma unroll
             for (int et = 0; et < 4; ++et) {
-                const bf16x8 ah = ax_tr_frag(Kp, 32 * m + 4 * g, 32 * m + 16 + 4 * g, 16 * et, lane);
-                const bf16x8 al = ax_tr_frag(Kp + AX_PLANE, 32 * m + 4 * g, 32 * m + 16 + 4 * g, 16 * et, lane);
-                dq[et] = ax_mfma3(ah, al, bhf, blf, dq[et]);
+                const int e0 = 16 * et + 4 * g;
+                f32x4 v = dq[et];
+#pragma unroll
+                for (int r = 0; r < 4; ++r) v[r] *= a.scale;
+                if (a.dqkvp) ax_store4_planes(outp, e0, v);
+                else if (e0 < E) ax_store4(out + e0, E - e0, v);
             }
-        }
-        float* out = a.dqkv + ((long long)b * AX_L + 16 * w + fr) * a.ld + h * E;
-        unsigned char* outp = a.dqkvp + (long long)b * 65536 + (16 * w + fr) * 512 + 128 * h;
-#pragma unroll
-        for (int et = 0; et < 4; ++et) {
-            const int e0 = 16 * et + 4 * g;
-            f32x4 v = dq[et];
-#pragma unroll
-            for (int r = 0; r < 4; ++r) v[r] *= a.scale;
-            if (a.dqkvp) ax_store4_planes(outp, e0, v);
-            else if (e0 < E) ax_store4(out + e0, E - e0, v);
-        }
-    }
-    __syncthreads();
-#pragma unroll
-    for (int kt = 0; kt < 4; ++kt) {
-        u32x2_t hi, lo;
-        const int off = (16 * w + fr) * AX_RS + 2 * (16 * kt + 4 * g);
-        x3_split4(pd[kt][0], pd[kt][1], pd[kt][2], pd[kt][3], hi, lo);
-        *reinterpret_cast<u32x2_t*>(Kp + off) = hi;
-        *reinterpret_cast<u32x2_t*>(Kp + AX_PLANE + off) = lo;
-        x3_split4(dp[kt][0], dp[kt][1], dp[kt][2], dp[kt][3], hi, lo);
-        *reinterpret_cast<u32x2_t*>(Vp + off) = hi;
-        *reinterpret_cast<u32x2_t*>(Vp + AX_PLANE + off) = lo;
-    }
-    __syncthreads();
+        },
+        dk, dv);
 
-    f32x4 dv[4], dk[4];
-#pragma unroll
-    for (int et = 0; et < 4; ++et) { dv[et] = f32x4{0.f, 0.f, 0.f, 0.f}; dk[et] = f32x4{0.f, 0.f, 0.f, 0.f}; }
-#pragma unroll
-    for (int ks = 0; ks < 2; ++ks) {
-        const int q0 = 32 * ks + 8 * g;
-        const bf16x8 ph = ax_tr_frag(Kp, q0, q0 + 4, 16 * w, lane), pl = ax_tr_frag(Kp + AX_PLANE, q0, q0 + 4, 16 * w, lane);
-        const bf16x8 sh = ax_tr_frag(Vp, q0, q0 + 4, 16 * w, lane), sl = ax_tr_frag(Vp + AX_PLANE, q0, q0 + 4, 16 * w, lane);
-#pragma unroll
-        for (int et = 0; et < 4; ++et) {
-            const bf16x8 oh = ax_tr_frag(Op, q0, q0 + 4, 16 * et, lane), ol = ax_tr_frag(Op + AX_PLANE, q0, q0 + 4, 16 * et, lane);
-            const bf16x8 qh = ax_tr_frag(Qp, q0, q0 + 4, 16 * et, lane), ql = ax_tr_frag(Qp + AX_PLANE, q0, q0 + 4, 16 * et, lane);
-            dv[et] = ax_mfma3(oh, ol, ph, pl, dv[et]);
-            dk[et] = ax_mfma3(qh, ql, sh, sl, dk[et]);
-        }
-    }
     if (a.dqkvp) {
         const long long grp = (long long)a.B * 65536;
         unsigned char* outp = a.dqkvp + (long long)b * 65536 + (16 * w + fr) * 512 + 128 * h;
diff --git a/eeg_image_decode_amd/csrc/attention_x3_body.h b/eeg_image_decode_amd/csrc/attention_x3_body.h
--- /dev/null
+++ b/eeg_image_decode_amd/csrc/attention_x3_body.h
@@ -0,0 +1,198 @@
+#pragma once
+#include "eeg_common.h"
+
+namespace eeg {
+
+constexpr int AX_L = 64;
+constexpr int AX_RS = 144;
+constexpr int AX_PLANE = AX_L * AX_RS;
+constexpr int AX_TENSOR = 2 * AX_PLANE;
+
+typedef short ax_s4 __attribute__((ext_vector_type(4)));
+typedef float ax_f2 __attribute__((ext_vector_type(2)));
+typedef float ax_f4u __attribute__((ext_vector_type(4), aligned(4)));
+
+__device__ __forceinline__ ax_s4 ax_tr_read(const unsigned char* p) {
+#if defined(EEG_EMU)
+    const int lane = hipemu::cur->lane, g = lane >> 4, i = lane & 15;
+    ax_s4 r;
+    for (int j = 0; j < 4; ++j) {
+        const unsigned long long src = hipemu::shfl_idx((unsigned long long)(uintptr_t)p, 16 * g + 4 * j + (i >> 2));
+        r[j] = reinterpret_cast<const short*>((uintptr_t)src)[i & 3];
+    }
+    return r;
+#else
+    return __builtin_amdgcn_ds_read_tr16_b64_v4i16((__attribute__((address_space(3))) ax_s4*)(p));
+#endif
+}
+__device__ __forceinline__ bf16x8 ax_tr_frag(const unsigned char* plane, int r0, int r1, int c0, int lane) {
+    const int l = lane & 15;
+    const ax_s4 a = ax_tr_read(plane + (r0 + (l >> 2)) * AX_RS + 2 * (c0 + 4 * (l & 3)));
+    const ax_s4 b = ax_tr_read(plane + (r1 + (l >> 2)) * AX_RS + 2 * (c0 + 4 * (l & 3)));
+    return bf16x8{a[0], a[1], a[2], a[3], b[0], b[1], b[2], b[3]};
+}
+__device__ __forceinline__ bf16x8 ax_frag(const unsigned char* plane, int row, int k0) {
+    return *reinterpret_cast<const bf16x8*>(plane + row * AX_RS + 2 * k0);
+}
+__device__ __forceinline__ bf16x8 ax_pack8(u32x2_t a, u32x2_t b) {
+    typedef unsigned u4 __attribute__((ext_vector_type(4)));
+    const u4 v{a[0], a[1], b[0], b[1]};
+    return __builtin_bit_cast(bf16x8, v);
+}
+__device__ __forceinline__ f32x4 ax_mfma3(bf16x8 ah, bf16x8 al, bf16x8 bh, bf16x8 bl, f32x4 c) {
+    c = mfma_bf16_16x16x32(al, bh, c);
+    c = mfma_bf16_16x16x32(ah, bl, c);
+    return mfma_bf16_16x16x32(ah, bh, c);
+}
+
+__device__ __forceinline__ void ax_stage_load(ax_f2 (&v)[4][8], const float* qrow0, const float* orow0, int th, int ld, int HE, int E) {
+#pragma unroll
+    for (int j = 0; j < 8; ++j) {
+        const int idx = th + 256 * j, row = idx >> 5, col = 2 * (idx & 31);
+        const bool ok = col < E;
+        const float* qr = qrow0 + (long long)row * ld + col;
+        v[0][j] = ok ? *reinterpret_cast<const ax_f2*>(qr) : ax_f2{0.f, 0.f};
+        v[1][j] = ok ? *reinterpret_cast<const ax_f2*>(qr + HE) : ax_f2{0.f, 0.f};
+        v[2][j] = ok ? *reinterpret_cast<const ax_f2*>(qr + 2 * HE) : ax_f2{0.f, 0.f};
+        v[3][j] = ok ? *reinterpret_cast<const ax_f2*>(orow0 + (long long)row * HE + col) : ax_f2{0.f, 0.f};
+    }
+}
+__device__ __forceinline__ void ax_stage_store(const ax_f2 (&v)[4][8], unsigned char* lds, int th) {
+#pragma unroll
+    for (int x = 0; x < 4; ++x)
+#pragma unroll
+        for (int j = 0; j < 8; ++j) {
+            const int idx = th + 256 * j, row = idx >> 5, col = 2 * (idx & 31);
+            const unsigned hi = x3_pack2(v[x][j][0], v[x][j][1]);
+            const float r0 = v[x][j][0] - __uint_as_float(hi << 16), r1 = v[x][j][1] - __uint_as_float(hi & 0xffff0000u);
+            unsigned char* dst = lds + x * AX_TENSOR + row * AX_RS + 2 * col;
+            *reinterpret_cast<unsigned*>(dst) = hi;
+            *reinterpret_cast<unsigned*>(dst + AX_PLANE) = x3_pack2(r0, r1);
+        }
+}
+
+template <bool TRAIN, class BARRIER, class DQ_READY>
+__device__ __forceinline__ void ax_head_bwd(unsigned char* lds, int w, int lane, int bh, float scale, float drop_p, unsigned long long seed, unsigned site,
+                                            BARRIER&& barrier, DQ_READY&& dq_ready, f32x4 (&dk)[4], f32x4 (&dv)[4]) {
+    unsigned char* Qp = lds;
+    unsigned char* Kp = lds + AX_TENSOR;
+    unsigned char* Vp = lds + 2 * AX_TENSOR;
+    unsigned char* Op = lds + 3 * AX_TENSOR;
+    const int fr = lane & 15, g = lane >> 4;
+
+    f32x4 s[4], dp[4];
+#pragma unroll
+    for (int kt = 0; kt < 4; ++kt) { s[kt] = f32x4{0.f, 0.f, 0.f, 0.f}; dp[kt] = f32x4{0.f, 0.f, 0.f, 0.f}; }
+#pragma unroll
+    for (int ks = 0; ks < 2; ++ks) {
+        const int k0 = 32 * ks + 8 * g;
+        const bf16x8 qh = ax_frag(Qp, 16 * w + fr, k0), ql = ax_frag(Qp + AX_PLANE, 16 * w + fr, k0);
+        const bf16x8 oh = ax_frag(Op, 16 * w + fr, k0), ol = ax_frag(Op + AX_PLANE, 16 * w + fr, k0);
+#pragma unroll
+        for (int kt = 0; kt < 4; ++kt) {
+            const bf16x8 kh = ax_frag(Kp, 16 * kt + fr, k0), kl = ax_frag(Kp + AX_PLANE, 16 * kt + fr, k0);
+            const bf16x8 vh = ax_frag(Vp, 16 * kt + fr, k0), vl = ax_frag(Vp + AX_PLANE, 16 * kt + fr, k0);
+            s[kt] = ax_mfma3(kh, kl, qh, ql, s[kt]);
+            dp[kt] = ax_mfma3(vh, vl, oh, ol, dp[kt]);
+        }
+    }
+    float mx = -INFINITY;
+#pragma unroll
+    for (int kt = 0; kt < 4; ++kt)
+#pragma unroll
+        for (int r = 0; r < 4; ++r) {
+            s[kt][r] *= scale;
+            mx = fmaxf(mx, s[kt][r]);
+        }
+    mx = fmaxf(mx, __shfl_xor(mx, 16, 64));
+    mx = fmaxf(mx, __shfl_xor(mx, 32, 64));
+    float sum = 0.f;
+#pragma unroll
+    for (int kt = 0; kt < 4; ++kt)
+#pragma unroll
+        for (int r = 0; r < 4; ++r) {
+            s[kt][r] = expf(s[kt][r] - mx);
+            sum += s[kt][r];
+        }
+    sum += __shfl_xor(sum, 16, 64);
+    sum += __shfl_xor(sum, 32, 64);
+    const float inv = 1.0f / sum;
+    const bool drop = TRAIN && drop_p > 0.f;
+    const float ksc = drop ? 1.f / (1.f - drop_p) : 1.f;
+    f32x4 pd[4];
+    float dq_sum = 0.f;
+#pragma unroll
+    for (int kt = 0; kt < 4; ++kt) {
+        bool keep[4] = {true, true, true, true};
+        if (drop) {
+            const unsigned long long idx0 = ((unsigned long long)bh * AX_L + 16 * w + fr) * AX_L + 16 * kt + 4 * g;
+            dropout_keep4(seed, site, idx0, drop_p, keep);
+        }
+#pragma unroll
+        for (int r = 0; r < 4; ++r) {
+            const float p = s[kt][r] * inv;
+            const float d = keep[r] ? dp[kt][r] * ksc : 0.f;
+            pd[kt][r] = keep[r] ? p * ksc : 0.f;
+            s[kt][r] = p;
+            dp[kt][r] = d;
+            dq_sum += p * d;
+        }
+    }
+    dq_sum += __shfl_xor(dq_sum, 16, 64);
+    dq_sum += __shfl_xor(dq_sum, 32, 64);
+#pragma unroll
+    for (int kt = 0; kt < 4; ++kt)
+#pragma unroll
+        for (int r = 0; r < 4; ++r) dp[kt][r] = s[kt][r] * (dp[kt][r] - dq_sum);
+
+    {
+        f32x4 dq[4];
+#pragma unroll
+        for (int et = 0; et < 4; ++et) dq[et] = f32x4{0.f, 0.f, 0.f, 0.f};
+#pragma unroll
+        for (int m = 0; m < 2; ++m) {
+            u32x2_t h0, l0, h1, l1;
+            x3_split4(dp[2 * m][0], dp[2 * m][1], dp[2 * m][2], dp[2 * m][3], h0, l0);
+            x3_split4(dp[2 * m + 1][0], dp[2 * m + 1][1], dp[2 * m + 1][2], dp[2 * m + 1][3], h1, l1);
+            const bf16x8 bhf = ax_pack8(h0, h1), blf = ax_pack8(l0, l1);
+#pragma unroll
+            for (int et = 0; et < 4; ++et) {
+                const bf16x8 ah = ax_tr_frag(Kp, 32 * m + 4 * g, 32 * m + 16 + 4 * g, 16 * et, lane);
+                const bf16x8 al = ax_tr_frag(Kp + AX_PLANE, 32 * m + 4 * g, 32 * m + 16 + 4 * g, 16 * et, lane);
+                dq[et] = ax_mfma3(ah, al, bhf, blf, dq[et]);
+            }
+        }
+        dq_ready(dq);
+    }
+    barrier();
+#pragma unroll
+    for (int kt = 0; kt < 4; ++kt) {
+        u32x2_t hi, lo;
+        const int off = (16 * w + fr) * AX_RS + 2 * (16 * kt + 4 * g);
+        x3_split4(pd[kt][0], pd[kt][1], pd[kt][2], pd[kt][3], hi, lo);
+        *reinterpret_cast<u32x2_t*>(Kp + off) = hi;
+        *reinterpret_cast<u32x2_t*>(Kp + AX_PLANE + off) = lo;
+        x3_split4(dp[kt][0], dp[kt][1], dp[kt][2], dp[kt][3], hi, lo);
+        *reinterpret_cast<u32x2_t*>(Vp + off) = hi;
+        *reinterpret_cast<u32x2_t*>(Vp + AX_PLANE + off) = lo;
+    }
+    barrier();
+
+#pragma unroll
+    for (int et = 0; et < 4; ++et) { dv[et] = f32x4{0.f, 0.f, 0.f, 0.f}; dk[et] = f32x4{0.f, 0.f, 0.f, 0.f}; }
+#pragma unroll
+    for (int ks = 0; ks < 2; ++ks) {
+        const int q0 = 32 * ks + 8 * g;
+        const bf16x8 ph = ax_tr_frag(Kp, q0, q0 + 4, 16 * w, lane), pl = ax_tr_frag(Kp + AX_PLANE, q0, q0 + 4, 16 * w, lane);
+        const bf16x8 sh = ax_tr_frag(Vp, q0, q0 + 4, 16 * w, lane), sl = ax_tr_frag(Vp + AX_PLANE, q0, q0 + 4, 16 * w, lane);
+#pragma unroll
+        for (int et = 0; et < 4; ++et) {
+            const bf16x8 oh = ax_tr_frag(Op, q0, q0 + 4, 16 * et, lane), ol = ax_tr_frag(Op + AX_PLANE, q0, q0 + 4, 16 * et, lane);
+            const bf16x8 qh = ax_tr_frag(Qp, q0, q0 + 4, 16 * et, lane), ql = ax_tr_frag(Qp + AX_PLANE, q0, q0 + 4, 16 * et, lane);
+            dv[et] = ax_mfma3(oh, ol, ph, pl, dv[et]);
+            dk[et] = ax_mfma3(qh, ql, sh, sl, dk[et]);
+        }
+    }
+}
+
+}
diff --git a/eeg_image_decode_amd/csrc/token_block.hip b/eeg_image_decode_amd/csrc/token_block.hip
--- a/eeg_image_decode_amd/csrc/token_block.hip
+++ b/eeg_image_decode_amd/csrc/token_block.hip
@@ -1,4 +1,5 @@
 #include "cstack_common.h"
+#include "attention_x3_body.h"
 
 #include <stdio.h>
 #include <stdlib.h>
@@ -785,10 +786,13 @@
     const float *dn3, *n2, *r2, *r1, *f1, *mu1, *rs1, *mu2, *rs2, *mu3, *rs3, *ln1_g, *ln2_g, *ln2_b, *ln3_g;
     float *dr1, *dctx, *partials;
     unsigned char *df2p, *dg1p, *da1p, *dr1p;
-    const unsigned char* dqkvp;
+    unsigned char* dqkvp;
     float drop_p;
     unsigned long long seed;
     unsigned site_embed, site_attn_out, site_ffn_act, site_ffn_out;
+    const float* qkv;
+    float scale;
+    unsigned site_attn;
 };
 
 __device__ __forceinline__ void tb_ln_bwd_row(const float (&dy)[4], const float (&x)[4], const float (&gam)[4], const bool (&ok)[2], float mu, float rs,
@@ -1031,6 +1035,42 @@
             if (d0 < TB_E) tb_st4(q5.dctx + (long long)b * (TB_L * TB_HE) + (unsigned)(m * TB_HE + head * TB_E + d0), TB_E - d0 >= 4 ? 4 : 2, v);
         });
         tb_planes_out<64>(AP, q5.da1p + (long long)b * (2 * TB_AP_PLANE), t);
+    }
+}
+
+template <bool TRAIN>
+__device__ __forceinline__ void tb_bwd_b_finish(const tb_bwd_args& a, unsigned char* AP, const unsigned char* XF, int b, int t, float ksc) {
+    float* ob = a.dr1 + (long long)b * (TB_L * TB_D);
+#pragma unroll
+    for (int j = 0; j < 8; ++j) {
+        const int q = t + TB_THREADS * j;
+        if (q < TB_L * TB_D / 4) {
+            const int i0 = 4 * q, row = i0 / TB_D, col = i0 - TB_D * row;
+            const bool wrap = col + 2 >= TB_D;
+            const int row2 = wrap ? row + 1 : row, col2 = wrap ? col + 2 - TB_D : col + 2;
+            const tb_f2 p0 = *reinterpret_cast<const tb_f2*>(XF + xf_off(row, col)), p1 = *reinterpret_cast<const tb_f2*>(XF + xf_off(row2, col2));
+            float v[4] = {p0[0], p0[1], p1[0], p1[1]};
+            if (TRAIN && a.drop_p > 0.f) {
+                bool keep[4];
+                dropout_keep4(a.seed, a.site_embed, (unsigned long long)b * (TB_L * TB_D) + i0, a.drop_p, keep);
+#pragma unroll
+                for (int e = 0; e < 4; ++e) v[e] = keep[e] ? v[e] * ksc : 0.f;
+            }
+            *reinterpret_cast<f32x4*>(ob + i0) = f32x4{v[0], v[1], v[2], v[3]};
+            if (a.dr1p) {
+                tb_store_planes2(AP, TB_AP_PLANE, ap_off(row, col), v[0], v[1]);
+                tb_store_planes2(AP, TB_AP_PLANE, ap_off(row2, col2), v[2], v[3]);
+            }
+        }
+    }
+    if (a.dr1p) {
+        if (t < 128) {
+            const int row = t & 63, plane = t >> 6;
+#pragma unroll
+            for (int k = 250; k < 256; k += 2) *reinterpret_cast<unsigned*>(AP + plane * TB_AP_PLANE + ap_off(row, k)) = 0u;
+        }
+        raw_barrier();
+        tb_planes_out<64>(AP, a.dr1p + (long long)b * (2 * TB_AP_PLANE), t);
     }
 }
 
@@ -1073,38 +1113,155 @@
         *reinterpret_cast<f32x4*>(XF + xf_off(m, n0)) = o;
     });
     __syncthreads();
-    float* ob = a.dr1 + (long long)b * (TB_L * TB_D);
-#pragma unroll
-    for (int j = 0; j < 8; ++j) {
-        const int q = t + TB_THREADS * j;
-        if (q < TB_L * TB_D / 4) {
-            const int i0 = 4 * q, row = i0 / TB_D, col = i0 - TB_D * row;
-            const bool wrap = col + 2 >= TB_D;
-            const int row2 = wrap ? row + 1 : row, col2 = wrap ? col + 2 - TB_D : col + 2;
-            const tb_f2 p0 = *reinterpret_cast<const tb_f2*>(XF + xf_off(row, col)), p1 = *reinterpret_cast<const tb_f2*>(XF + xf_off(row2, col2));
-            float v[4] = {p0[0], p0[1], p1[0], p1[1]};
-            if (TRAIN && a.drop_p > 0.f) {
-                bool keep[4];
-                dropout_keep4(a.seed, a.site_embed, (unsigned long long)b * (TB_L * TB_D) + i0, a.drop_p, keep);
-#pragma unroll
-                for (int e = 0; e < 4; ++e) v[e] = keep[e] ? v[e] * ksc : 0.f;
-            }
-            *reinterpret_cast<f32x4*>(ob + i0) = f32x4{v[0], v[1], v[2], v[3]};
-            if (a.dr1p) {
-                tb_store_planes2(AP, TB_AP_PLANE, ap_off(row, col), v[0], v[1]);
-                tb_store_planes2(AP, TB_AP_PLANE, ap_off(row2, col2), v[2], v[3]);
-            }
-        }
-    }
-    if (a.dr1p) {
-        if (t < 128) {
-            const int row = t & 63, plane = t >> 6;
-#pragma unroll
-            for (int k = 250; k < 256; k += 2) *reinterpret_cast<unsigned*>(AP + plane * TB_AP_PLANE + ap_off(row, k)) = 0u;
-        }
+    tb_bwd_b_finish<TRAIN>(a, AP, XF, b, t, ksc);
+}
+
+constexpr int TB_HO_PLANE = 64 * 256;
+constexpr int TB_HO_TENSOR = 2 * TB_HO_PLANE;
+constexpr int TB_FUSED_LDS = 2 * 4 * AX_TENSOR;
+static_assert(3 * TB_HO_TENSOR <= TB_FUSED_LDS && TB_AP_BYTES + TB_XF_BYTES <= TB_FUSED_LDS && TB_FUSED_LDS <= 160 * 1024, "LDS map of the fused backward");
+
+__device__ __forceinline__ int ho_off(int row, int col) { return row * 256 + ((((col >> 3) ^ (row & 15))) << 4) + ((col & 7) << 1); }
+
+__device__ __forceinline__ void tb_gemm_heads(const unsigned char* HO, const unsigned short* wp, int pair, int lane, f32x4 (&acc)[4][2]) {
+    constexpr int NT = 2, PF = 2, NS = 12;
+    const int fr = lane & 15, g = lane >> 4;
+    bf16x8 bh[PF + 1][NT], bl[PF + 1][NT];
+    auto issue = [&](int s) {
+        const int slot = s % (PF + 1), which = s >> 2, ks = 4 * pair + (s & 3);
+#pragma unroll
+        for (int j = 0; j < NT; ++j) {
+            const bf16x8* q = reinterpret_cast<const bf16x8*>(wp + which * TB_MAT_ELEMS + (long long)(j * TB_KS + ks) * TB_TILE) + lane;
+#if defined(EEG_EMU)
+            bh[slot][j] = q[0];
+            bl[slot][j] = q[64];
+#else
+            asm volatile("global_load_dwordx4 %0, %1, off" : "=v"(bh[slot][j]) : "v"(q) : "memory");
+            asm volatile("global_load_dwordx4 %0, %1, off offset:1024" : "=v"(bl[slot][j]) : "v"(q) : "memory");
+#endif
+        }
+    };
+    auto landed = [&](int s) {
+#if !defined(EEG_EMU)
+        const int slot = s % (PF + 1);
+        const int younger = NS - 1 - s < PF ? NS - 1 - s : PF;
+#define TB_WAIT(N) asm volatile("s_waitcnt vmcnt(" #N ")" : "+v"(bh[slot][0]), "+v"(bl[slot][0]), "+v"(bh[slot][1]), "+v"(bl[slot][1])::"memory")
+        if (younger == 2) TB_WAIT(8);
+        else if (younger == 1) TB_WAIT(4);
+        else TB_WAIT(0);
+#undef TB_WAIT
+#endif
+    };
+#pragma unroll
+    for (int p = 0; p < PF; ++p) issue(p);
+#pragma unroll
+    for (int s = 0; s < NS; ++s) {
+        const int cur = s % (PF + 1);
+        if (s + PF < NS) issue(s + PF);
+        landed(s);
+        const unsigned char* A = HO + (s >> 2) * TB_HO_TENSOR;
+        bf16x8 ah[4], al[4];
+#pragma unroll
+        for (int mt = 0; mt < 4; ++mt) {
+            const int off = (16 * mt + fr) * 256 + (((4 * (s & 3) + g) ^ fr) << 4);
+            ah[mt] = *reinterpret_cast<const bf16x8*>(A + off);
+            al[mt] = *reinterpret_cast<const bf16x8*>(A + TB_HO_PLANE + off);
+        }
+#pragma unroll
+        for (int pr = 0; pr < 3; ++pr)
+#pragma unroll
+            for (int j = 0; j < NT; ++j)
+#pragma unroll
+                for (int mt = 0; mt < 4; ++mt) {
+                    const bf16x8 bw = pr == 0 ? bl[cur][j] : bh[cur][j];
+                    const bf16x8 aw = pr == 1 ? al[mt] : ah[mt];
+                    acc[mt][j] = mfma_bf16_16x16x32(bw, aw, acc[mt][j]);
+                }
+    }
+}
+
+template <bool TRAIN>
+__global__ __launch_bounds__(TB_THREADS, 2) void token_block_bwd_fused_kernel(const tb_bwd_args a0) {
+    EEG_LDS_BASE(unsigned char, lds);
+    const int t = threadIdx.x, lane = t & 63, w = wave_uniform(t >> 6), fr = lane & 15, g = lane >> 4;
+    const int hf = w >> 2, wl = w & 3, th = t & 255;
+    const int b = blockIdx.x, B = gridDim.x;
+    const float ksc = (TRAIN && a0.drop_p > 0.f) ? 1.f / (1.f - a0.drop_p) : 1.f;
+    unsigned char* const AX = lds + hf * (4 * AX_TENSOR);
+    f32x4 acc[4][2], resid[4][2];
+#pragma unroll
+    for (int mt = 0; mt < 4; ++mt)
+#pragma unroll
+        for (int j = 0; j < 2; ++j) acc[mt][j] = f32x4{0.f, 0.f, 0.f, 0.f};
+    ax_f2 stage[4][8];
+    auto stage_load = [&](const tb_bwd_args& q, int head) {
+        ax_stage_load(stage, q.qkv + (long long)b * (TB_L * 3 * TB_HE) + head * TB_E, q.dctx + (long long)b * (TB_L * TB_HE) + head * TB_E, th, 3 * TB_HE, TB_HE, TB_E);
+    };
+    stage_load(tb_args_again(a0), hf);
+#pragma unroll
+    for (int pair = 0; pair < 2; ++pair) {
+        const tb_bwd_args q = tb_args_again(a0);
+        const int head = 2 * pair + hf;
+        ax_stage_store(stage, AX, th);
         raw_barrier();
-        tb_planes_out<64>(AP, a.dr1p + (long long)b * (2 * TB_AP_PLANE), t);
-    }
+        f32x4 dq[4], dk[4], dv[4];
+        ax_head_bwd<TRAIN>(
+            AX, wl, lane, b * TB_H + head, q.scale, q.drop_p, q.seed, q.site_attn, [] { raw_barrier(); },
+            [&](f32x4(&d)[4]) {
+#pragma unroll
+                for (int et = 0; et < 4; ++et)
+#pragma unroll
+                    for (int r = 0; r < 4; ++r) dq[et][r] = d[et][r] * q.scale;
+            },
+            dk, dv);
+        raw_barrier();
+        if (pair == 0) stage_load(q, 2 + hf);
+#pragma unroll
+        for (int et = 0; et < 4; ++et) {
+            const int off = ho_off(16 * wl + fr, 64 * hf + 16 * et + 4 * g);
+            f32x4 k = dk[et];
+#pragma unroll
+            for (int r = 0; r < 4; ++r) k[r] *= q.scale;
+            tb_store_planes4(lds, TB_HO_PLANE, off, dq[et][0], dq[et][1], dq[et][2], dq[et][3]);
+            tb_store_planes4(lds + TB_HO_TENSOR, TB_HO_PLANE, off, k[0], k[1], k[2], k[3]);
+            tb_store_planes4(lds + 2 * TB_HO_TENSOR, TB_HO_PLANE, off, dv[et][0], dv[et][1], dv[et][2], dv[et][3]);
+        }
+        raw_barrier();
+        tb_gemm_heads(lds, q.packed + TB_OFF_QT + (long long)(2 * w) * TB_KS * TB_TILE, pair, lane, acc);
+        if (pair == 1)
+            tb_for_tiles(w, lane, TB_D, acc, [&](int m, int n0, int valid, f32x4& v) {
+                resid[m >> 4][(n0 >> 4) & 1] = tb_ld4(q.dr1 + (long long)b * (TB_L * TB_D) + (unsigned)(m * TB_D + n0), valid);
+            });
+        {
+            const unsigned lds_off = (unsigned)((t >> 4) * 256 + (((t & 15) ^ ((t >> 4) & 15)) << 4)), g_off = (unsigned)((t >> 4) * 512 + 256 * pair + (t & 15) * 16);
+#pragma unroll
+            for (int which = 0; which < 3; ++which) {
+                tb_u4 v[2][2];
+#pragma unroll
+                for (int plane = 0; plane < 2; ++plane)
+#pragma unroll
+                    for (int j = 0; j < 2; ++j) v[plane][j] = *reinterpret_cast<const tb_u4*>(lds + which * TB_HO_TENSOR + plane * TB_HO_PLANE + j * 8192 + lds_off);
+                unsigned char* dst = q.dqkvp + ((long long)which * B + b) * (2 * TB_AP_PLANE);
+#pragma unroll
+                for (int plane = 0; plane < 2; ++plane)
+#pragma unroll
+                    for (int j = 0; j < 2; ++j) *reinterpret_cast<tb_u4*>(dst + plane * TB_AP_PLANE + j * 16384 + g_off) = v[plane][j];
+            }
+        }
+        raw_barrier();
+    }
+    const tb_bwd_args q = tb_args_again(a0);
+    unsigned char* const AP = lds;
+    unsigned char* const XF = lds + TB_AP_BYTES;
+    tb_for_tiles(w, lane, TB_D, acc, [&](int m, int n0, int valid, f32x4& v) {
+        const f32x4 r = resid[m >> 4][(n0 >> 4) & 1];
+        f32x4 o;
+#pragma unroll
+        for (int i = 0; i < 4; ++i) o[i] = i < valid ? r[i] + v[i] : 0.f;
+        *reinterpret_cast<f32x4*>(XF + xf_off(m, n0)) = o;
+    });
+    __syncthreads();
+    tb_bwd_b_finish<TRAIN>(q, AP, XF, b, t, ksc);
 }
 
 struct tb_param_args {
@@ -1254,11 +1411,11 @@
 extern "C" long long eegclip_token_block_bwd_workspace_floats(int B) { return B < 1 ? 0 : (long long)B * 6 * 256; }
 
 extern "C" int eegclip_token_block_bwd(const eegclip_token_block_bwd_desc* d, int part, void* stream) {
-    if (!d || d->B < 1 || !d->packed || d->drop_p < 0.f || d->drop_p >= 1.f || part < 0 || part > 2) return EEGCLIP_EINVAL;
+    if (!d || d->B < 1 || !d->packed || d->drop_p < 0.f || d->drop_p >= 1.f || part < 0 || part > 3) return EEGCLIP_EINVAL;
     tb_bwd_args a{static_cast<const unsigned short*>(d->packed), d->dn3, d->n2, d->r2, d->r1, d->f1, d->mu1, d->rs1, d->mu2, d->rs2, d->mu3, d->rs3,
                   d->ln1_g, d->ln2_g, d->ln2_b, d->ln3_g, d->dr1, d->dctx, d->partials, static_cast<unsigned char*>(d->df2p), static_cast<unsigned char*>(d->dg1p),
-                  static_cast<unsigned char*>(d->da1p), static_cast<unsigned char*>(d->dr1p), static_cast<const unsigned char*>(d->dqkvp), d->drop_p, d->seed,
-                  d->site_embed, d->site_attn_out, d->site_ffn_act, d->site_ffn_out};
+                  static_cast<unsigned char*>(d->da1p), static_cast<unsigned char*>(d->dr1p), static_cast<unsigned char*>(d->dqkvp), d->drop_p, d->seed,
+                  d->site_embed, d->site_attn_out, d->site_ffn_act, d->site_ffn_out, d->qkv, d->scale, d->site_attn};
     if (part == 0) {
         if (!d->dn3 || (!d->n2 && !d->ln2_b) || !d->r2 || !d->r1 || !d->f1 || !d->mu1 || !d->rs1 || !d->mu2 || !d->rs2 || !d->mu3 || !d->rs3 || !d->ln1_g || !d->ln2_g ||
             !d->ln3_g || !d->df2p || !d->dg1p || !d->da1p || !d->dr1 || !d->dctx || !d->partials)
@@ -1277,6 +1434,13 @@
             return EEGCLIP_EALIGN;
         if (d->drop_p > 0.f) EEG_LAUNCH(token_block_bwd_b_kernel<true>, dim3(d->B), dim3(TB_THREADS), TB_AP_BYTES + TB_XF_BYTES, stream, a);
         else EEG_LAUNCH(token_block_bwd_b_kernel<false>, dim3(d->B), dim3(TB_THREADS), TB_AP_BYTES + TB_XF_BYTES, stream, a);
+    } else if (part == 3) {
+        if (!d->qkv || !d->dctx || !d->dqkvp || !d->dr1) return EEGCLIP_EINVAL;
+        if ((reinterpret_cast<uintptr_t>(d->packed) | reinterpret_cast<uintptr_t>(d->dr1) | reinterpret_cast<uintptr_t>(d->dqkvp) | reinterpret_cast<uintptr_t>(d->dr1p)) & 15u)
+            return EEGCLIP_EALIGN;
+        if ((reinterpret_cast<uintptr_t>(d->qkv) | reinterpret_cast<uintptr_t>(d->dctx)) & 7u) return EEGCLIP_EALIGN;
+        if (d->drop_p > 0.f) EEG_LAUNCH(token_block_bwd_fused_kernel<true>, dim3(d->B), dim3(TB_THREADS), TB_FUSED_LDS, stream, a);
+        else EEG_LAUNCH(token_block_bwd_fused_kernel<false>, dim3(d->B), dim3(TB_THREADS), TB_FUSED_LDS, stream, a);
     } else {
         if (!d->partials || !d->dln3_g || !d->dln3_b || !d->dln2_g || !d->dln2_b || !d->dln1_g || !d->dln1_b) return EEGCLIP_EINVAL;
         tb_param_args pa{d->partials, {d->dln3_g, d->dln3_b, d->dln2_g, d->dln2_b, d->dln1_g, d->dln1_b}, d->B};
diff --git a/include/eegclip.h b/include/eegclip.h
--- a/include/eegclip.h
+++ b/include/eegclip.h
@@ -5,7 +5,7 @@
 extern "C" {
 #endif
 
-#define EEGCLIP_ABI_VERSION 14
+#define EEGCLIP_ABI_VERSION 15
 #define EEGCLIP_EINVAL (-1)
 #define EEGCLIP_EALIGN (-2)
 
@@ -298,11 +298,14 @@
     const float *dn3, *n2, *r2, *r1, *f1, *mu1, *rs1, *mu2, *rs2, *mu3, *rs3, *ln1_g, *ln2_g, *ln2_b, *ln3_g;
     float *dr1, *dctx, *partials;
     void *df2p, *dg1p, *da1p, *dr1p;
-    const void* dqkvp;
+    void* dqkvp;
     float *dln3_g, *dln3_b, *dln2_g, *dln2_b, *dln1_g, *dln1_b;
     float drop_p;
     unsigned long long seed;
     unsigned int site_embed, site_attn_out, site_ffn_act, site_ffn_out;
+    const float* qkv;
+    float scale;
+    unsigned int site_attn;
 } eegclip_token_block_bwd_desc;
 long long eegclip_token_block_bwd_workspace_floats(int B);
 int eegclip_token_block_bwd(const eegclip_token_block_bwd_desc* d, int part, void* stream);
```

Result: no change. 394,000 samples/s (-0.5%).
